# yanglei18/SGV3D

Hardware: AMD Instinct MI355X
Metric: camera frames/sec at 864x1536->BEV (higher is better)
Workload: dtype f32

## Files before the change

### include/sgv3d_hip.h

```cpp
#ifndef SGV3D_HIP_H
#define SGV3D_HIP_H

#include <stddef.h>
#include <stdint.h>

#ifdef __cplusplus
extern "C" {
#endif

#define SGV3D_OK 0
#define SGV3D_EINVAL (-1)
#define SGV3D_ELAUNCH (-2)
#define SGV3D_ENOSPACE (-3)

const char *sgv3d_last_error(void);
int sgv3d_abi_version(void);


int sgv3d_voxel_pooling_forward(int batch_size, int num_points, int num_channels,
                                int num_voxel_x, int num_voxel_y, int num_voxel_z,
                                const int32_t *geom_xyz, const float *input_features,
                                float *output_features, int32_t *pos_memo, void *stream);
int sgv3d_voxel_pooling_forward_fresh(int batch_size, int num_points, int num_channels,
                                      int num_voxel_x, int num_voxel_y, int num_voxel_z,
// ... 57 lines not shown
                              const float *prob,
                              const float *context,
                              const float *grad_output,
                              long long sb, long long sy, long long sx,
                              float *grad_prob,
                              float *grad_context,
                              void *workspace, size_t workspace_bytes, void *stream);


int sgv3d_calib_prep(int num_cams, const float *sensor2ego, const float *sensor2virtual,
                     const float *intrin, const float *ida, float *prep, void *stream);

int sgv3d_geometry_voxel_index(int num_cams, int cams_per_batch, int num_depth, int feat_h, int feat_w,
                               const float *frustum, const float *prep, const float *ref_h,
                               const float *bda, const float *voxel_coord ,
                               const float *voxel_size , int32_t *geom_xyz, float *geom_f,
                               void *stream);

int sgv3d_calib_changed(int n, const void *const *tensors , const int32_t *nbytes ,
                        void *copy, int force, int32_t *changed, void *stream);
int sgv3d_calib_prep_gated(int num_cams, const float *sensor2ego, const float *sensor2virtual, const float *intrin,
                           const float *ida, float *prep, const int32_t *run, void *stream);
int sgv3d_geometry_voxel_index_gated(int num_cams, int cams_per_batch, int num_depth, int feat_h, int feat_w,
                                     const float *frustum, const float *prep, const float *ref_h, const float *bda,
                                     const float *voxel_coord , const float *voxel_size , int32_t *geom_xyz,
                                     float *geom_f, const int32_t *run, void *stream);


int sgv3d_lift(int batch_size, int num_pixels, int num_depth, int num_channels,
               const float *height_context, float *prob, float *lifted, void *stream);
int sgv3d_lift_bf16(int batch_size, int num_pixels, int num_depth, int num_channels, const float *height_context,
                    float *prob, void *lifted_bf16, void *stream);


typedef struct sgv3d_conv_desc {
    int batch, in_h, in_w, cin;
    int out_h, out_w, cout;
    int kh, kw, stride, pad, dil;
    int x_ld, x_coff;
    int y_ld, y_coff;
    int res_ld;
    int relu;
    int mode;
    int deconv_ks;
    int k_pad, cout_pad;
    int tile;
    int x_nchw;
    int k_order;
    int split_k;
} sgv3d_conv_desc;

#define SGV3D_CONV_NORMAL 0
#define SGV3D_CONV_DECONV 1
#define SGV3D_CONV_NCHW_OUT 2
#define SGV3D_CONV_GROUP_PLANES 3

#define SGV3D_TILE_128x128 1
#define SGV3D_TILE_128x64 2
#define SGV3D_TILE_64x128 3
#define SGV3D_TILE_64x64 4
#define SGV3D_TILE_32x128 9
#define SGV3D_TILE_48x64 10
#define SGV3D_TILE_X3 64
#define SGV3D_TILE_MFIRST 16
#define SGV3D_TILE_OCC5 32
#define SGV3D_WINOGRAD_RESIDENT 6
#define SGV3D_WINOGRAD_HALF 8

int sgv3d_conv_winograd4_pack_weight(const float *w_src , int cout, int cin, int k_pad, int cout_pad,
                                     float *u_packed , void *stream);
int sgv3d_conv_winograd4_pack_weight_x3(const float *w_src, int cout, int cin, int cin_pad, int cout_pad, void *u3_packed,
                                        void *stream);

int sgv3d_conv_pack_weight_x3(const float *w_src, int cout, int cin, int kh, int kw, int cin_pad, int cout_pad, void *u3_packed,
                              void *stream);
int sgv3d_conv2d_x3_forward(const sgv3d_conv_desc *desc, const float *x, const void *u3_packed, const float *scale,
                            const float *bias, const float *residual, float *y, void *workspace, size_t workspace_bytes,
                            void *stream);
int sgv3d_conv2d_x3_shortcut_forward(const sgv3d_conv_desc *desc_a, const float *xa, const void *u3a, const float *scale_a,
                                     const float *bias_a, const sgv3d_conv_desc *desc_b, const float *xb, const void *u3b,
                                     const float *scale_b, const float *bias_b, float *y, void *stream);
int sgv3d_stem_pool_x3_forward(int batch, int h, int w, const float *x_nchw, const void *w_x3, size_t w_bytes, const float *scale,
                               const float *shift, float *y_nhwc, int y_ld, int variant, void *stream);
size_t sgv3d_conv2d_winograd4_workspace_bytes(const sgv3d_conv_desc *desc );
int sgv3d_conv2d_winograd4_forward(const sgv3d_conv_desc *desc , const float *x, const float *u_packed,
                                   const float *scale, const float *bias, const float *residual, float *y,
                                   void *workspace, size_t workspace_bytes, void *stream);

void sgv3d_conv_pack_geometry(int k, int n, int *k_pad, int *n_pad);

int sgv3d_conv_pack_weight(const float *w_src, int cout, int cin, int kh, int kw, int cin_pad,
                           int transposed, int k_order, float *w_packed, int k_pad, int cout_pad,
                           void *stream);

size_t sgv3d_conv2d_workspace_bytes(const sgv3d_conv_desc *desc );
int sgv3d_conv2d_forward(const sgv3d_conv_desc *desc , const float *x, const float *w_packed,
                         const float *scale, const float *bias, const float *residual,
                         const float *gate, float *y, void *workspace, size_t workspace_bytes,
                         void *stream);

int sgv3d_conv2d_forward_bf16(const sgv3d_conv_desc *desc , const float *x, const float *w_packed,
                              const float *scale, const float *bias, const float *residual,
                              const float *gate, float *y, void *workspace, size_t workspace_bytes,
                              void *stream);

int sgv3d_conv_weight_to_bf16(const float *w_packed, int k_pad, int cout_pad, void *w_packed_bf16, void *stream);
int sgv3d_conv2d_forward_bf16io(const sgv3d_conv_desc *desc , const void *x, const void *w_packed,
                                const float *scale, const float *bias, const void *residual, const float *gate,
                                void *y, void *workspace, size_t workspace_bytes, void *stream, int io_flags);

int sgv3d_conv2d_forward_f32x3(const sgv3d_conv_desc *desc , const float *x, const float *w_packed,
                               const float *scale, const float *bias, const float *residual,
                               const float *gate, float *y, void *workspace, size_t workspace_bytes,
                               void *stream);

size_t sgv3d_conv_winograd_weight_floats(int cout, int cin_pad);
int sgv3d_conv_winograd_pack_weight(const float *w_src, int cout, int cin, int cin_pad, float *w_packed,
                                    void *stream);
int sgv3d_conv2d_winograd_forward(const sgv3d_conv_desc *desc , const float *x, const float *w_wino,
                                  const float *scale, const float *bias, const float *residual,
                                  const float *gate, float *y, void *workspace, size_t workspace_bytes,
                                  void *stream);


int sgv3d_maxpool3x3s2(int batch, int in_h, int in_w, int channels, const float *x, float *y,
                       void *stream);

int sgv3d_maxpool3x3s2_bf16(int batch, int in_h, int in_w, int channels, const void *x, void *y, void *stream);
int sgv3d_nchw_to_nhwc(int batch, int channels, int h, int w, int c_pad, const float *x, float *y,
                       void *stream);
int sgv3d_nhwc_to_nchw(int batch, int channels, int h, int w, int ld, int coff, const float *x,
                       float *y, void *stream);

size_t sgv3d_global_avgpool_workspace_bytes(int batch, int channels);
int sgv3d_global_avgpool(int batch, int pixels, int channels, int x_ld, const float *x, float *y,
                         void *workspace, size_t workspace_bytes, void *stream);

int sgv3d_dense(int batch, int k, int n, const float *x, const float *w, const float *scale,
                const float *bias, int act, float *y, void *stream);
int sgv3d_dense_gated(int batch, int k, int n, const float *x, const float *w, const float *scale,
                      const float *bias, int act, float *y, const int32_t *run, void *stream);

int sgv3d_broadcast_channels(int batch, int pixels, int channels, int y_ld, int y_coff,
                             const float *v, float *y, void *stream);

int sgv3d_scale_channels(int batch, int pixels, int channels, const float *x, const float *gate,
                         float *y, void *stream);

int sgv3d_copy_channels(int batch, int pixels, int channels, int x_ld, int x_coff, const float *x,
                        float *y, void *stream);

int sgv3d_upsample_bilinear2x(int batch, int h, int w, int channels, const float *x, float *y, void *stream);

int sgv3d_add_mul_sigmoid(long long n, const float *a, const float *b, const float *c, float *y, void *stream);

int sgv3d_bsm_compose(int batch, int pixels, int num_depth, int context_channels, int semantic_channels,
                      int ld, const float *semantic_logits, int semantic_ld, float background_threshold,
                      float *height_context, void *stream);

int sgv3d_deform_conv3x3_forward(int batch, int h, int w, int channels, int groups, int out_per_group, const float *x,
                                 const float *offset, int off_ld, const float *const *w_packed, int k_pad, int cout_pad,
                                 float *y, int y_ld, int y_coff, void *stream);

size_t sgv3d_deform_conv3x3_bf16_weight_bytes(int channels, int groups, int out_per_group);
int sgv3d_deform_conv3x3_bf16_pack_weight(const float *weight, int channels, int groups, int out_per_group, void *w_packed,
                                          void *stream);
int sgv3d_deform_conv3x3_forward_bf16(int batch, int h, int w, int channels, int groups, int out_per_group, const void *x,
                                      int x_is_bf16, const float *offset, int off_ld, const void *w_packed, void *y,
                                      int y_is_bf16, int y_ld, int y_coff, void *stream);

// ... 555 lines not shown
```

### sgv3d_amd/_lib.py

```python
import ctypes
import os

_HERE = os.path.dirname(os.path.abspath(__file__))
LIB_PATH = os.path.join(_HERE, "csrc", "libsgv3d_hip.so")

c_int, c_void_p, c_size_t, c_ll = ctypes.c_int, ctypes.c_void_p, ctypes.c_size_t, ctypes.c_longlong


class ConvDesc(ctypes.Structure):
    _fields_ = [(n, c_int) for n in (
        "batch", "in_h", "in_w", "cin", "out_h", "out_w", "cout", "kh", "kw", "stride", "pad", "dil",
        "x_ld", "x_coff", "y_ld", "y_coff", "res_ld", "relu", "mode", "deconv_ks", "k_pad", "cout_pad",
        "tile", "x_nchw", "k_order", "split_k")]


class VitAttnDesc(ctypes.Structure):
    _fields_ = [(n, c_int) for n in ("batch", "height", "width", "heads", "head_dim", "win_h", "win_w")]


class SamAttnDesc(ctypes.Structure):
    _fields_ = [(n, c_int) for n in ("batch", "nq", "nk", "heads", "head_dim", "q_ld", "k_ld", "v_ld", "o_ld")] + [("scale", ctypes.c_float)]


CONV_NORMAL, CONV_DECONV, CONV_NCHW_OUT, CONV_GROUP_PLANES = 0, 1, 2, 3
# ... 1 lines not shown

_PROTOS = {
    "sgv3d_last_error": (ctypes.c_char_p, []),
    "sgv3d_abi_version": (c_int, []),
    "sgv3d_voxel_pooling_select_kernel": (c_int, [c_int]),
    "sgv3d_voxel_pooling_kernel_for": (c_int, [c_int] * 6),
    "sgv3d_voxel_pooling_forward": (c_int, [c_int] * 6 + [c_void_p] * 5),
    "sgv3d_voxel_pooling_forward_fresh": (c_int, [c_int] * 6 + [c_void_p] * 5),
    "sgv3d_voxel_pooling_forward_atomic": (c_int, [c_int] * 6 + [c_void_p] * 5),
    "sgv3d_voxel_pooling_cache_clear": (c_int, []),
    "sgv3d_voxel_pooling_cache_stats": (c_int, [ctypes.POINTER(ctypes.c_ulonglong)]),
    "sgv3d_voxel_plan_bytes": (c_size_t, [c_int] * 4),
    "sgv3d_voxel_plan_build": (c_int, [c_int] * 5 + [c_void_p, c_void_p, c_void_p, c_size_t, c_int, c_void_p]),
    "sgv3d_voxel_plan_init": (c_int, [c_int] * 4 + [c_void_p, c_size_t, c_void_p]),
    "sgv3d_voxel_plan_build_cached": (c_int, [c_int] * 5 + [c_void_p, c_void_p, c_size_t, c_int, c_void_p]),
    "sgv3d_voxel_plan_stats_offset": (c_size_t, [c_int] * 4),
    "sgv3d_voxel_pooling_workspace_bytes": (c_size_t, [c_int] * 3),
    "sgv3d_voxel_pooling_forward_planned": (c_int, [c_int] * 5 + [c_void_p] * 4 + [c_size_t, c_void_p]),
    "sgv3d_voxel_pooling_forward_planned_bf16": (c_int, [c_int] * 5 + [c_void_p] * 3 + [c_int, c_void_p, c_size_t, c_void_p]),
    "sgv3d_lift_splat_planned_bf16out": (c_int, [c_int] * 6 + [c_void_p] * 3 + [c_int, c_void_p, c_int, c_void_p, c_size_t, c_void_p]),
    "sgv3d_lift_splat_planned": (c_int, [c_int] * 6 + [c_void_p] * 5 + [c_size_t, c_void_p]),
    "sgv3d_voxel_pooling_backward": (c_int, [c_int] * 3 + [c_void_p, c_void_p, c_ll, c_ll, c_ll, c_ll, c_void_p, c_void_p]),
    "sgv3d_lift_splat_backward_workspace_bytes": (c_size_t, [c_int] * 4),
    "sgv3d_lift_splat_backward": (c_int, [c_int] * 7 + [c_void_p] * 4 + [c_ll] * 3 + [c_void_p] * 3 + [c_size_t, c_void_p]),
    "sgv3d_calib_prep": (c_int, [c_int] + [c_void_p] * 6),
    "sgv3d_calib_prep_gated": (c_int, [c_int] + [c_void_p] * 7),
    "sgv3d_calib_changed": (c_int, [c_int, ctypes.POINTER(c_void_p), ctypes.POINTER(c_int), c_void_p, c_int, c_void_p, c_void_p]),
    "sgv3d_geometry_voxel_index_gated": (c_int, [c_int] * 5 + [c_void_p] * 4 + [ctypes.POINTER(ctypes.c_float)] * 2 + [c_void_p] * 4),
    "sgv3d_dense_gated": (c_int, [c_int] * 3 + [c_void_p] * 4 + [c_int, c_void_p, c_void_p, c_void_p]),
    "sgv3d_geometry_voxel_index": (c_int, [c_int] * 5 + [c_void_p] * 4 + [ctypes.POINTER(ctypes.c_float)] * 2 + [c_void_p] * 3),
    "sgv3d_lift": (c_int, [c_int] * 4 + [c_void_p] * 4),
    "sgv3d_lift_bf16": (c_int, [c_int] * 4 + [c_void_p] * 4),
    "sgv3d_conv_pack_geometry": (None, [c_int, c_int, ctypes.POINTER(c_int), ctypes.POINTER(c_int)]),
    "sgv3d_conv_pack_weight": (c_int, [c_void_p] + [c_int] * 7 + [c_void_p, c_int, c_int, c_void_p]),
    "sgv3d_conv2d_workspace_bytes": (c_size_t, [ctypes.POINTER(ConvDesc)]),
    "sgv3d_conv2d_forward": (c_int, [ctypes.POINTER(ConvDesc)] + [c_void_p] * 8 + [c_size_t, c_void_p]),
    "sgv3d_conv2d_forward_bf16": (c_int, [ctypes.POINTER(ConvDesc)] + [c_void_p] * 8 + [c_size_t, c_void_p]),
    "sgv3d_conv2d_forward_bf16io": (c_int, [ctypes.POINTER(ConvDesc)] + [c_void_p] * 8 + [c_size_t, c_void_p, c_int]),
    "sgv3d_conv_weight_to_bf16": (c_int, [c_void_p, c_int, c_int, c_void_p, c_void_p]),
    "sgv3d_conv2d_forward_f32x3": (c_int, [ctypes.POINTER(ConvDesc)] + [c_void_p] * 8 + [c_size_t, c_void_p]),
    "sgv3d_centerhead_branches_workspace_bytes": (c_size_t, [c_int] * 4),
    "sgv3d_centerhead_branches_forward": (c_int, [c_int] * 6 + [c_void_p, c_int] + [c_void_p] * 3 + [c_int] + [c_void_p] * 5
                                          + [c_size_t, c_void_p]),
    "sgv3d_centerhead_bf16_weight_bytes": (c_size_t, [c_int]),
    "sgv3d_centerhead_bf16_pack_weight": (c_int, [c_void_p, c_int, c_int, c_void_p, c_void_p]),
    "sgv3d_centerhead_bf16_weight2_bytes": (c_size_t, [c_int]),
    "sgv3d_centerhead_bf16_pack_weight2": (c_int, [c_void_p, c_void_p, c_int, c_void_p, c_void_p]),
    "sgv3d_centerhead_f4_weight_floats": (c_size_t, [c_int]),
    "sgv3d_centerhead_f4_pack_weight": (c_int, [c_void_p, c_int, c_void_p, c_void_p]),
    "sgv3d_centerhead_branches_forward_f4": (c_int, [c_int] * 6 + [c_void_p, c_int] + [c_void_p] * 3 + [c_int] + [c_void_p] * 5
                                             + [c_size_t, c_void_p]),
    "sgv3d_conv3x3_f4res_weight_floats": (c_size_t, [c_int, c_int]),
    "sgv3d_conv3x3_f4res_pack_weight": (c_int, [c_void_p, c_int, c_int, c_int, c_void_p, c_void_p]),
    "sgv3d_conv3x3_f4res_forward": (c_int, [ctypes.POINTER(ConvDesc)] + [c_void_p] * 7),
    "sgv3d_centerhead_branches_forward_bf16": (c_int, [c_int] * 6 + [c_void_p, c_int] + [c_void_p] * 3 + [c_int] + [c_void_p] * 5),
    "sgv3d_centerhead_branches_forward_bf16x": (c_int, [c_int] * 6 + [c_void_p, c_int] + [c_void_p] * 3 + [c_int] + [c_void_p] * 5),
    "sgv3d_centerhead_bf16_select_plain": (None, [c_int]),
    "sgv3d_centerhead_bf16_debug_stamps": (None, [c_void_p]),
    "sgv3d_scale_channels_bf16": (c_int, [c_int] * 3 + [c_void_p] * 4),
    "sgv3d_global_avgpool_bf16": (c_int, [c_int] * 4 + [c_void_p] * 3 + [c_size_t, c_void_p]),
    "sgv3d_broadcast_channels_bf16": (c_int, [c_int] * 5 + [c_void_p] * 3),
    "sgv3d_upsample_bilinear2x_bf16": (c_int, [c_int] * 4 + [c_void_p] * 3),
    "sgv3d_add_mul_sigmoid_bf16": (c_int, [c_ll] + [c_void_p] * 5),
    "sgv3d_deform_im2col3x3_bf16": (c_int, [c_int] * 5 + [c_void_p] * 2 + [c_int, c_void_p, c_void_p]),
    "sgv3d_conv3x3_patch_bf16_weight_bytes": (c_size_t, [c_int, c_int]),
    "sgv3d_conv3x3_patch_bf16_debug_stamps": (None, [c_void_p]),
    "sgv3d_conv3x3_patch_bf16_pack_weight": (c_int, [c_void_p, c_int, c_int, c_void_p, c_void_p]),
    "sgv3d_conv3x3_patch_bf16_forward": (c_int, [c_int] * 11 + [c_void_p] * 6 + [c_int, c_int, c_void_p, c_size_t, c_void_p]),
    "sgv3d_conv_dw_bf16_weight_bytes": (c_size_t, [c_int] * 4),
    "sgv3d_conv_dw_bf16_pack_weight": (c_int, [c_void_p] + [c_int] * 5 + [c_void_p, c_void_p]),
    "sgv3d_conv_dw_bf16_forward": (c_int, [ctypes.POINTER(ConvDesc)] + [c_void_p] * 7),
    "sgv3d_conv_dw_bf16_workspace_bytes": (c_size_t, [ctypes.POINTER(ConvDesc)]),
    "sgv3d_conv_dw_bf16_forward_splitk": (c_int, [ctypes.POINTER(ConvDesc)] + [c_void_p] * 7 + [c_size_t, c_void_p]),
    "sgv3d_conv_dw_bf16_pair_forward": (c_int, [ctypes.POINTER(ConvDesc)] + [c_void_p] * 4 + [c_int] + [c_void_p] * 4 + [c_int, c_void_p, c_int, c_int, c_int, c_void_p]),
    "sgv3d_conv_winograd_weight_floats": (c_size_t, [c_int, c_int]),
    "sgv3d_conv_winograd_pack_weight": (c_int, [c_void_p, c_int, c_int, c_int, c_void_p, c_void_p]),
    "sgv3d_conv2d_winograd_forward": (c_int, [ctypes.POINTER(ConvDesc)] + [c_void_p] * 8 + [c_size_t, c_void_p]),
    "sgv3d_conv_winograd4_pack_weight": (c_int, [c_void_p, c_int, c_int, c_int, c_int, c_void_p, c_void_p]),
    "sgv3d_conv_winograd4_pack_weight_x3": (c_int, [c_void_p, c_int, c_int, c_int, c_int, c_void_p, c_void_p]),
    "sgv3d_conv_pack_weight_x3": (c_int, [c_void_p, c_int, c_int, c_int, c_int, c_int, c_int, c_void_p, c_void_p]),
    "sgv3d_conv2d_x3_forward": (c_int, [c_void_p] * 8 + [c_size_t, c_void_p]),
    "sgv3d_conv2d_x3_shortcut_forward": (c_int, [c_void_p] * 12),
    "sgv3d_stem_pool_x3_forward": (c_int, [c_int] * 3 + [c_void_p, c_void_p, c_size_t] + [c_void_p] * 3 + [c_int, c_int, c_void_p]),
    "sgv3d_conv2d_winograd4_workspace_bytes": (c_size_t, [ctypes.POINTER(ConvDesc)]),
    "sgv3d_conv2d_winograd4_forward": (c_int, [ctypes.POINTER(ConvDesc)] + [c_void_p] * 7 + [c_size_t, c_void_p]),
    "sgv3d_maxpool3x3s2": (c_int, [c_int] * 4 + [c_void_p] * 3),
    "sgv3d_maxpool3x3s2_bf16": (c_int, [c_int] * 4 + [c_void_p] * 3),
    "sgv3d_nchw_to_nhwc": (c_int, [c_int] * 5 + [c_void_p] * 3),
    "sgv3d_nhwc_to_nchw": (c_int, [c_int] * 6 + [c_void_p] * 3),
    "sgv3d_global_avgpool_workspace_bytes": (c_size_t, [c_int] * 2),
    "sgv3d_global_avgpool": (c_int, [c_int] * 4 + [c_void_p] * 3 + [c_size_t, c_void_p]),
    "sgv3d_dense": (c_int, [c_int] * 3 + [c_void_p] * 4 + [c_int, c_void_p, c_void_p]),
    "sgv3d_broadcast_channels": (c_int, [c_int] * 5 + [c_void_p] * 3),
    "sgv3d_scale_channels": (c_int, [c_int] * 3 + [c_void_p] * 4),
    "sgv3d_copy_channels": (c_int, [c_int] * 5 + [c_void_p] * 3),
    "sgv3d_upsample_bilinear2x": (c_int, [c_int] * 4 + [c_void_p] * 3),
    "sgv3d_add_mul_sigmoid": (c_int, [c_ll] + [c_void_p] * 5),
    "sgv3d_bsm_compose": (c_int, [c_int] * 6 + [c_void_p, c_int, ctypes.c_float, c_void_p, c_void_p]),
    "sgv3d_deform_im2col3x3": (c_int, [c_int] * 5 + [c_void_p, c_void_p, c_int, c_void_p, c_void_p]),
    "sgv3d_deform_conv3x3_forward": (c_int, [c_int] * 6 + [c_void_p, c_void_p, c_int, c_void_p, c_int, c_int, c_void_p, c_int, c_int,
                                                          c_void_p]),
    "sgv3d_deform_conv3x3_bf16_weight_bytes": (c_size_t, [c_int] * 3),
    "sgv3d_deform_conv3x3_bf16_pack_weight": (c_int, [c_void_p, c_int, c_int, c_int, c_void_p, c_void_p]),
    "sgv3d_deform_conv3x3_forward_bf16": (c_int, [c_int] * 6 + [c_void_p, c_int, c_void_p, c_int, c_void_p, c_void_p, c_int, c_int, c_int,
                                                               c_void_p]),
    "sgv3d_head_final_conv": (c_int, [c_int] * 6 + [c_void_p] * 6),
    "sgv3d_centerpoint_decode_workspace_bytes": (c_size_t, [c_int] * 3),
    "sgv3d_centerpoint_decode": (c_int, [c_int] * 5 + [c_void_p] * 6 + [c_ll] + [ctypes.c_float] * 6 +
                                 [ctypes.POINTER(ctypes.c_float), c_int, ctypes.c_float, c_int, c_void_p, c_size_t] +
                                 [c_void_p] * 6),
    "sgv3d_centerpoint_decode_tasks_workspace_bytes": (c_size_t, [c_int] * 4),
    "sgv3d_centerpoint_decode_tasks": (c_int, [c_int, c_int, ctypes.POINTER(ctypes.c_int32), c_int, c_int, c_int] +
                                       [ctypes.POINTER(c_void_p)] * 6 + [c_ll] + [ctypes.c_float] * 6 +
                                       [ctypes.POINTER(ctypes.c_float), c_int, ctypes.POINTER(ctypes.c_float), c_int, c_void_p,
                                        c_size_t] + [c_void_p] * 6),
    "sgv3d_centerpoint_merge_tasks": (c_int, [c_int] * 3 + [c_void_p] * 4 + [ctypes.POINTER(ctypes.c_int32)] + [c_void_p] * 5),
    "sgv3d_rotated_bev_iou_host": (c_int, [c_int] + [ctypes.POINTER(ctypes.c_float)] * 3),
    "sgv3d_rotate_nms_workspace_bytes": (c_size_t, [c_int] * 3),
    "sgv3d_rotate_nms": (c_int, [c_int] * 3 + [c_void_p] * 3 + [ctypes.c_float, ctypes.POINTER(ctypes.c_float), c_int, c_int,
                                                                ctypes.POINTER(ctypes.c_float), c_void_p, c_size_t, c_void_p, c_void_p]),
    "sgv3d_centerpoint_decode_tasks_rotate_workspace_bytes": (c_size_t, [c_int] * 4),
    "sgv3d_centerpoint_decode_tasks_rotate": (c_int, [c_int, c_int, ctypes.POINTER(ctypes.c_int32), c_int, c_int, c_int] +
                                              [ctypes.POINTER(c_void_p)] * 6 + [c_ll] + [ctypes.c_float] * 6 +
                                              [ctypes.POINTER(ctypes.c_float), c_int, ctypes.c_float, ctypes.POINTER(ctypes.c_float),
                                               c_int, c_int, ctypes.POINTER(ctypes.c_float), c_void_p, c_size_t] + [c_void_p] * 6),
    "sgv3d_centerhead_targets": (c_int, [c_int, c_int, c_void_p, c_void_p, c_int, ctypes.POINTER(ctypes.c_int32)] +
                                 [c_int] * 3 + [ctypes.c_float] * 5 + [ctypes.c_double, c_int, c_int] + [c_void_p] * 5),
    "sgv3d_conv2d_backward_weight_workspace_bytes": (c_size_t, [ctypes.POINTER(ConvDesc), c_int]),
    "sgv3d_conv2d_backward_weight": (c_int, [ctypes.POINTER(ConvDesc)] + [c_void_p] * 3 + [c_int, c_void_p, c_size_t, c_void_p]),
    "sgv3d_conv2d_backward_weight_bf16_workspace_bytes": (c_size_t, [ctypes.POINTER(ConvDesc), c_int]),
    "sgv3d_conv2d_backward_weight_bf16": (c_int, [ctypes.POINTER(ConvDesc)] + [c_void_p] * 3 + [c_int, c_void_p, c_size_t, c_void_p]),
    "sgv3d_conv2d_backward_weight_bf16_batched_workspace_bytes": (c_size_t, [ctypes.POINTER(ConvDesc), c_int, c_int]),
    "sgv3d_conv2d_backward_weight_bf16_batched": (c_int, [ctypes.POINTER(ConvDesc), c_void_p, ctypes.POINTER(c_void_p), ctypes.POINTER(c_void_p), c_int, c_int, c_void_p, c_size_t, c_void_p]),
    "sgv3d_conv2d_backward_weight_bf16_alltaps_workspace_bytes": (c_size_t, [ctypes.POINTER(ConvDesc), c_int, c_int]),
    "sgv3d_conv2d_backward_weight_bf16_alltaps": (c_int, [ctypes.POINTER(ConvDesc)] + [c_void_p] * 3 + [c_int, c_void_p, c_size_t, c_void_p]),
    "sgv3d_conv2d_backward_weight_bf16_tensors_workspace_bytes": (c_size_t, [ctypes.POINTER(ConvDesc), c_int]),
    "sgv3d_conv2d_backward_weight_bf16_tensors": (c_int, [ctypes.POINTER(ConvDesc)] + [c_void_p] * 3 + [c_int, c_void_p, c_size_t, c_void_p]),
    "sgv3d_conv2d_backward_weight_bf16_alltaps_tensors_workspace_bytes": (c_size_t, [ctypes.POINTER(ConvDesc), c_int]),
    "sgv3d_conv2d_backward_weight_bf16_alltaps_tensors": (c_int, [ctypes.POINTER(ConvDesc)] + [c_void_p] * 3 + [c_int, c_void_p, c_size_t, c_void_p]),
    "sgv3d_conv2d_backward_weight_bf16_alltaps_batched": (c_int, [ctypes.POINTER(ConvDesc), c_void_p, ctypes.POINTER(c_void_p), ctypes.POINTER(c_void_p), c_int, c_int, c_void_p, c_size_t, c_void_p]),
    "sgv3d_conv2d_backward_weight_thin_workspace_bytes": (c_size_t, [ctypes.POINTER(ConvDesc)]),
    "sgv3d_conv2d_backward_weight_batched_workspace_bytes": (c_size_t, [ctypes.POINTER(ConvDesc), c_int, c_int]),
    "sgv3d_conv2d_backward_weight_batched": (c_int, [ctypes.POINTER(ConvDesc), c_void_p, ctypes.POINTER(c_void_p), ctypes.POINTER(c_void_p), c_int, c_int, c_void_p, c_size_t, c_void_p]),
    "sgv3d_conv2d_backward_weight_thin": (c_int, [ctypes.POINTER(ConvDesc)] + [c_void_p] * 4 + [c_size_t, c_void_p]),
    "sgv3d_conv3x3_thin_forward_batched": (c_int, [ctypes.POINTER(ConvDesc), c_int, ctypes.POINTER(ctypes.c_int32)] + [ctypes.POINTER(c_void_p)] * 4 + [c_void_p]),
    "sgv3d_conv3x3_thin_backward_batched_workspace_bytes": (c_size_t, [ctypes.POINTER(ConvDesc), c_int, ctypes.POINTER(ctypes.c_int32)]),
    "sgv3d_conv3x3_thin_backward_batched": (c_int, [ctypes.POINTER(ConvDesc), c_int, ctypes.POINTER(ctypes.c_int32)] + [ctypes.POINTER(c_void_p)] * 6 + [c_void_p, c_size_t, c_void_p]),
    "sgv3d_weight_rot180_transpose": (c_int, [c_void_p] + [c_int] * 4 + [c_void_p, c_void_p]),
    "sgv3d_gather_pack_job_bytes": (c_int, []),
    "sgv3d_gather_pack_elements_per_block": (c_int, []),
    "sgv3d_gather_pack": (c_int, [c_void_p, c_int, c_int, c_void_p]),
    "sgv3d_zero_insert": (c_int, [c_int] * 7 + [c_void_p] * 3),
    "sgv3d_interleave_phases2": (c_int, [c_int] * 4 + [ctypes.POINTER(c_void_p)] + [ctypes.POINTER(ctypes.c_int32)] * 4 +
                                 [c_void_p, c_void_p]),
    "sgv3d_batchnorm_workspace_bytes": (c_size_t, [c_int]),
    "sgv3d_batchnorm_train_forward": (c_int, [c_ll, c_int] + [c_void_p] * 6 + [ctypes.c_float, ctypes.c_float, c_int] +
                                      [c_void_p] * 4 + [c_size_t, c_void_p]),
    "sgv3d_batchnorm_relu_train_backward_from_x": (c_int, [c_ll, c_int] + [c_void_p] * 9 + [c_void_p, c_size_t, c_void_p]),
    "sgv3d_batchnorm_train_backward": (c_int, [c_ll, c_int] + [c_void_p] * 6 + [c_int] + [c_void_p] * 5 + [c_size_t, c_void_p]),
    "sgv3d_batchnorm_train_forward_bf16": (c_int, [c_ll, c_int] + [c_void_p] * 6 + [ctypes.c_float, ctypes.c_float, c_int] +
                                           [c_void_p] * 4 + [c_size_t, c_void_p]),
    "sgv3d_batchnorm_relu_train_backward_from_x_bf16": (c_int, [c_ll, c_int] + [c_void_p] * 9 + [c_void_p, c_size_t, c_void_p]),
    "sgv3d_batchnorm_train_backward_bf16": (c_int, [c_ll, c_int] + [c_void_p] * 6 + [c_int] + [c_void_p] * 5 + [c_size_t, c_void_p]),
    "sgv3d_adamw_step": (c_int, [c_ll] + [c_void_p] * 4 + [c_int] + [ctypes.c_float] * 6 + [c_void_p] * 2),
    "sgv3d_adamw_step_dev": (c_int, [c_ll] + [c_void_p] * 5 + [ctypes.c_float] * 5 + [c_void_p] * 2),
    "sgv3d_adamw_set_hyper": (c_int, [c_void_p, c_int] + [ctypes.c_float] * 3 + [c_void_p]),
    "sgv3d_grad_sumsq_partials": (c_int, []),
    "sgv3d_grad_sumsq": (c_int, [c_ll, c_void_p, c_void_p, c_void_p]),
# ... 147 lines not shown
```

### sgv3d_amd/csrc/act_bf16.hip

```cpp
#include "common.hpp"

using namespace sgv3d;

namespace {

typedef __bf16 bf16x8 __attribute__((ext_vector_type(8)));
typedef __bf16 bf16x4 __attribute__((ext_vector_type(4)));
typedef float f32x4 __attribute__((ext_vector_type(4)));

constexpr int kBlock = 256;
constexpr int kAvgChunks = 32;

struct F8 {
    float v[8];
};

__device__ __forceinline__ F8 ld8(const __bf16 *p) {
    const bf16x8 q = *reinterpret_cast<const bf16x8 *>(p);
    F8 r;
#pragma unroll
    for (int i = 0; i < 8; ++i) r.v[i] = (float)q[i];
    return r;
}

__device__ __forceinline__ void st8(__bf16 *p, const F8 &r) {
    const f32x4 lo = {r.v[0], r.v[1], r.v[2], r.v[3]}, hi = {r.v[4], r.v[5], r.v[6], r.v[7]};
    const bf16x4 l4 = __builtin_convertvector(lo, bf16x4), h4 = __builtin_convertvector(hi, bf16x4);
    *reinterpret_cast<bf16x8 *>(p) = __builtin_shufflevector(l4, h4, 0, 1, 2, 3, 4, 5, 6, 7);
}

__global__ __launch_bounds__(kBlock) void scale_channels_bf16_kernel(long long total8, int P, int C8, const __bf16 *__restrict__ x,
                                                                     const float *__restrict__ gate, __bf16 *__restrict__ y) {
    const long long i = (long long)blockIdx.x * kBlock + threadIdx.x;
    if (i >= total8) return;
    const int c = (int)(i % C8);
    const long long b = i / ((long long)P * C8);
    F8 v = ld8(x + i * 8);
    const float *g = gate + (b * C8 + c) * 8;
#pragma unroll
    for (int k = 0; k < 8; ++k) v.v[k] *= g[k];
    st8(y + i * 8, v);
}

__global__ __launch_bounds__(kBlock) void global_avgpool_bf16_partial_kernel(int P, int C, int ld, const __bf16 *__restrict__ x,
                                                                             float *__restrict__ part) {
    __shared__ float red[4][64];
    const int b = blockIdx.z, chunk = blockIdx.y;
    const int c = blockIdx.x * 64 + (threadIdx.x & 63);
    const int g = threadIdx.x >> 6;
    const int per = (P + kAvgChunks - 1) / kAvgChunks;
    const int p0 = chunk * per, p1 = min(P, p0 + per);
    float s = 0.f;
    if (c < C)
        for (int p = p0 + g; p < p1; p += 4) s += (float)x[((long long)b * P + p) * ld + c];
    red[g][threadIdx.x & 63] = s;
    __syncthreads();
    if (g == 0 && c < C)
        part[((long long)b * kAvgChunks + chunk) * C + c] =
            (red[0][threadIdx.x] + red[1][threadIdx.x]) + (red[2][threadIdx.x] + red[3][threadIdx.x]);
}

__global__ __launch_bounds__(kBlock) void global_avgpool_bf16_final_kernel(int B, int P, int C, const float *__restrict__ part,
                                                                           float *__restrict__ y) {
    const long long i = (long long)blockIdx.x * kBlock + threadIdx.x;
    if (i >= (long long)B * C) return;
    const int b = (int)(i / C), c = (int)(i - (long long)b * C);
    float s = 0.f;
    for (int k = 0; k < kAvgChunks; ++k) s += part[((long long)b * kAvgChunks + k) * C + c];
    y[i] = s / (float)P;
}

__global__ __launch_bounds__(kBlock) void broadcast_channels_bf16_kernel(long long total8, int P, int C8, int ld, int coff,
                                                                         const float *__restrict__ v, __bf16 *__restrict__ y) {
    const long long i = (long long)blockIdx.x * kBlock + threadIdx.x;
    if (i >= total8) return;
    const int c = (int)(i % C8);
    const long long bp = i / C8;
    const long long b = bp / P;
    F8 r;
#pragma unroll
    for (int k = 0; k < 8; ++k) r.v[k] = v[(b * C8 + c) * 8 + k];
    st8(y + bp * ld + coff + c * 8, r);
}

__global__ __launch_bounds__(kBlock) void upsample_bilinear2x_bf16_kernel(int B, int H, int W, int C8, const __bf16 *__restrict__ x,
                                                                          __bf16 *__restrict__ y) {
    const long long total = (long long)B * 2 * H * 2 * W * C8;
    const long long i = (long long)blockIdx.x * kBlock + threadIdx.x;
    if (i >= total) return;
    const int c = (int)(i % C8);
    long long t = i / C8;
    const int ow = (int)(t % (2 * W));
    t /= (2 * W);
    const int oh = (int)(t % (2 * H));
    const int b = (int)(t / (2 * H));
    const float sh = fmaxf(0.5f * ((float)oh + 0.5f) - 0.5f, 0.f), sw = fmaxf(0.5f * ((float)ow + 0.5f) - 0.5f, 0.f);
    const int h1 = (int)sh, w1 = (int)sw;
    const int h1p = h1 < H - 1 ? 1 : 0, w1p = w1 < W - 1 ? 1 : 0;
    const float lh1 = sh - (float)h1, lw1 = sw - (float)w1;
    const float lh0 = 1.f - lh1, lw0 = 1.f - lw1;
    const __bf16 *p = x + (((long long)b * H * W) * C8 + c) * 8;
    const long long ps = (long long)C8 * 8;
    const F8 a = ld8(p + ((long long)h1 * W + w1) * ps), bq = ld8(p + ((long long)h1 * W + w1 + w1p) * ps);
    const F8 cq = ld8(p + ((long long)(h1 + h1p) * W + w1) * ps), d = ld8(p + ((long long)(h1 + h1p) * W + w1 + w1p) * ps);
    F8 o;
#pragma unroll
    for (int k = 0; k < 8; ++k) o.v[k] = lh0 * (lw0 * a.v[k] + lw1 * bq.v[k]) + lh1 * (lw0 * cq.v[k] + lw1 * d.v[k]);
    st8(y + i * 8, o);
}

__global__ __launch_bounds__(kBlock) void add_mul_sigmoid_bf16_kernel(long long n8, const __bf16 *__restrict__ a,
                                                                      const __bf16 *__restrict__ b, const __bf16 *__restrict__ c,
                                                                      __bf16 *__restrict__ y) {
    const long long i = (long long)blockIdx.x * kBlock + threadIdx.x;
    if (i >= n8) return;
    const F8 av = ld8(a + i * 8), bv = ld8(b + i * 8), cv = ld8(c + i * 8);
    F8 o;
#pragma unroll
    for (int k = 0; k < 8; ++k) o.v[k] = av.v[k] + bv.v[k] * (1.f / (1.f + expf(-cv.v[k])));
    st8(y + i * 8, o);
}

__global__ __launch_bounds__(kBlock) void deform_im2col3x3_bf16_kernel(int B, int H, int W, int C, int groups,
                                                                       const __bf16 *__restrict__ x, const float *__restrict__ off,
                                                                       int off_ld, __bf16 *__restrict__ col) {
    const int C8 = C >> 3;
    const long long total = (long long)B * H * W * 9 * C8;
    const long long i = (long long)blockIdx.x * kBlock + threadIdx.x;
    if (i >= total) return;
    const int c8 = (int)(i % C8);
    long long t = i / C8;
    const int tap = (int)(t % 9);
    t /= 9;
    const int w_ = (int)(t % W);
    const long long t2 = t / W;
    const int h_ = (int)(t2 % H);
    const int b = (int)(t2 / H);
    const int ky = tap / 3, kx = tap - ky * 3;
    const float oy = off[t * off_ld + 2 * tap], ox = off[t * off_ld + 2 * tap + 1];
    const float hf = (float)(h_ - 1 + ky) + oy;
    const float wf = (float)(w_ - 1 + kx) + ox;
    F8 val;
#pragma unroll
    for (int k = 0; k < 8; ++k) val.v[k] = 0.f;
    if (hf > -1.f && wf > -1.f && hf < (float)H && wf < (float)W) {
        const int h_low = (int)floorf(hf), w_low = (int)floorf(wf);
        const int h_high = h_low + 1, w_high = w_low + 1;
        const float lh = hf - (float)h_low, lw = wf - (float)w_low;
        const float hh = 1.f - lh, hw = 1.f - lw;
        const __bf16 *base = x + (long long)b * H * W * C + c8 * 8;
        const float w1 = hh * hw, w2 = hh * lw, w3 = lh * hw, w4 = lh * lw;
        F8 v1, v2, v3, v4;
#pragma unroll
        for (int k = 0; k < 8; ++k) v1.v[k] = v2.v[k] = v3.v[k] = v4.v[k] = 0.f;
        if (h_low >= 0 && w_low >= 0) v1 = ld8(base + ((long long)h_low * W + w_low) * C);
        if (h_low >= 0 && w_high <= W - 1) v2 = ld8(base + ((long long)h_low * W + w_high) * C);
        if (h_high <= H - 1 && w_low >= 0) v3 = ld8(base + ((long long)h_high * W + w_low) * C);
        if (h_high <= H - 1 && w_high <= W - 1) v4 = ld8(base + ((long long)h_high * W + w_high) * C);
#pragma unroll
        for (int k = 0; k < 8; ++k) val.v[k] = w1 * v1.v[k] + w2 * v2.v[k] + w3 * v3.v[k] + w4 * v4.v[k];
    }
    const int cpg = C / groups;
    const int c = c8 * 8;
    const int g = c / cpg, cg = c - g * cpg;
    st8(col + ((t * groups + g) * 9 + tap) * cpg + cg, val);
}

}

extern "C" int sgv3d_scale_channels_bf16(int batch, int pixels, int channels, const void *x, const float *gate, void *y, void *stream) {
    SGV3D_REQUIRE(batch > 0 && pixels > 0 && channels > 0 && (channels & 7) == 0, "scale_channels_bf16: channels must be a multiple of 8");
    SGV3D_REQUIRE(x && gate && y, "scale_channels_bf16: null pointer");
    const long long total8 = (long long)batch * pixels * (channels / 8);
    hipLaunchKernelGGL(scale_channels_bf16_kernel, dim3(cdiv(total8, kBlock)), dim3(kBlock), 0, as_stream(stream), total8, pixels,
                       channels / 8, static_cast<const __bf16 *>(x), gate, static_cast<__bf16 *>(y));
    return check_launch("scale_channels_bf16_kernel");
}

extern "C" int sgv3d_global_avgpool_bf16(int batch, int pixels, int channels, int x_ld, const void *x, float *y, void *workspace,
                                         size_t workspace_bytes, void *stream) {
    SGV3D_REQUIRE(batch > 0 && pixels > 0 && channels > 0 && x_ld >= channels, "global_avgpool_bf16: bad shape");
    SGV3D_REQUIRE(x && y && workspace, "global_avgpool_bf16: null pointer");
    if (workspace_bytes < sizeof(float) * (size_t)batch * kAvgChunks * channels)
        return fail(SGV3D_ENOSPACE, "global_avgpool_bf16: workspace too small (sgv3d_global_avgpool_workspace_bytes)");
    float *part = static_cast<float *>(workspace);
    hipLaunchKernelGGL(global_avgpool_bf16_partial_kernel, dim3(cdiv(channels, 64), kAvgChunks, batch), dim3(kBlock), 0,
                       as_stream(stream), pixels, channels, x_ld, static_cast<const __bf16 *>(x), part);
    hipLaunchKernelGGL(global_avgpool_bf16_final_kernel, dim3(cdiv((long long)batch * channels, kBlock)), dim3(kBlock), 0,
                       as_stream(stream), batch, pixels, channels, part, y);
    return check_launch("global_avgpool_bf16_kernel");
}

extern "C" int sgv3d_broadcast_channels_bf16(int batch, int pixels, int channels, int y_ld, int y_coff, const float *v, void *y,
                                             void *stream) {
    SGV3D_REQUIRE(batch > 0 && pixels > 0 && channels > 0 && y_ld >= y_coff + channels && y_coff >= 0, "broadcast_channels_bf16: bad shape");
    SGV3D_REQUIRE(((channels | y_ld | y_coff) & 7) == 0, "broadcast_channels_bf16: channels / y_ld / y_coff must be multiples of 8");
    SGV3D_REQUIRE(v && y, "broadcast_channels_bf16: null pointer");
    const long long total8 = (long long)batch * pixels * (channels / 8);
    hipLaunchKernelGGL(broadcast_channels_bf16_kernel, dim3(cdiv(total8, kBlock)), dim3(kBlock), 0, as_stream(stream), total8, pixels,
                       channels / 8, y_ld, y_coff, v, static_cast<__bf16 *>(y));
    return check_launch("broadcast_channels_bf16_kernel");
}

extern "C" int sgv3d_upsample_bilinear2x_bf16(int batch, int h, int w, int channels, const void *x, void *y, void *stream) {
    SGV3D_REQUIRE(batch > 0 && h > 0 && w > 0 && channels > 0 && (channels & 7) == 0, "upsample_bilinear2x_bf16: channels must be a multiple of 8");
    SGV3D_REQUIRE(x && y, "upsample_bilinear2x_bf16: null pointer");
    const long long total = (long long)batch * 4 * h * w * (channels / 8);
    hipLaunchKernelGGL(upsample_bilinear2x_bf16_kernel, dim3(cdiv(total, kBlock)), dim3(kBlock), 0, as_stream(stream), batch, h, w,
                       channels / 8, static_cast<const __bf16 *>(x), static_cast<__bf16 *>(y));
    return check_launch("upsample_bilinear2x_bf16_kernel");
}

extern "C" int sgv3d_add_mul_sigmoid_bf16(long long n, const void *a, const void *b, const void *c, void *y, void *stream) {
    SGV3D_REQUIRE(n > 0 && (n & 7) == 0, "add_mul_sigmoid_bf16: n must be a positive multiple of 8");
    SGV3D_REQUIRE(a && b && c && y, "add_mul_sigmoid_bf16: null pointer");
    hipLaunchKernelGGL(add_mul_sigmoid_bf16_kernel, dim3(cdiv(n / 8, kBlock)), dim3(kBlock), 0, as_stream(stream), n / 8,
                       static_cast<const __bf16 *>(a), static_cast<const __bf16 *>(b), static_cast<const __bf16 *>(c),
                       static_cast<__bf16 *>(y));
    return check_launch("add_mul_sigmoid_bf16_kernel");
}

extern "C" int sgv3d_deform_im2col3x3_bf16(int batch, int h, int w, int channels, int groups, const void *x, const float *offset,
                                           int off_ld, void *col, void *stream) {
    SGV3D_REQUIRE(batch > 0 && h > 0 && w > 0 && channels > 0 && groups > 0 && channels % groups == 0 &&
                      ((channels / groups) & 7) == 0 && off_ld >= 18,
                  "deform_im2col3x3_bf16: bad shape (channels per group must be a multiple of 8)");
    SGV3D_REQUIRE(x && offset && col, "deform_im2col3x3_bf16: null pointer");
    const long long total = (long long)batch * h * w * 9 * (channels / 8);
    hipLaunchKernelGGL(deform_im2col3x3_bf16_kernel, dim3(cdiv(total, kBlock)), dim3(kBlock), 0, as_stream(stream), batch, h, w,
                       channels, groups, static_cast<const __bf16 *>(x), offset, off_ld, static_cast<__bf16 *>(col));
    return check_launch("deform_im2col3x3_bf16_kernel");
}
```

### sgv3d_amd/csrc/conv_wino4.hip

```cpp
#include "conv_common.hpp"

using namespace sgv3d;

namespace {

struct f4 {
    float x, y, z, w;
};
__device__ __forceinline__ f4 ld4(const float *p) {
    const float4 v = *reinterpret_cast<const float4 *>(p);
    return {v.x, v.y, v.z, v.w};
}
__device__ __forceinline__ void st4(float *p, const f4 &v) { *reinterpret_cast<float4 *>(p) = make_float4(v.x, v.y, v.z, v.w); }
__device__ __forceinline__ f4 fma4(float s, const f4 &a, const f4 &b) {
    return {fmaf(s, a.x, b.x), fmaf(s, a.y, b.y), fmaf(s, a.z, b.z), fmaf(s, a.w, b.w)};
}
__device__ __forceinline__ f4 add4(const f4 &a, const f4 &b) { return {a.x + b.x, a.y + b.y, a.z + b.z, a.w + b.w}; }
__device__ __forceinline__ f4 sub4(const f4 &a, const f4 &b) { return {a.x - b.x, a.y - b.y, a.z - b.z, a.w - b.w}; }

__device__ __forceinline__ void wino4_bt(f4 &d0, f4 &d1, f4 &d2, f4 &d3, f4 &d4, f4 &d5) {
    const f4 a = fma4(-4.f, d2, d4), b = fma4(-4.f, d1, d3);
    const f4 c = sub4(d4, d2), e = sub4(d3, d1);
    const f4 t0 = fma4(4.f, d0, fma4(-5.f, d2, d4));
    const f4 t5 = fma4(4.f, d1, fma4(-5.f, d3, d5));
    d0 = t0;
    d1 = add4(a, b);
    d2 = sub4(a, b);
    d3 = fma4(2.f, e, c);
    d4 = fma4(-2.f, e, c);
    d5 = t5;
}

__device__ __forceinline__ void wino4_at(const f4 &m0, const f4 &m1, const f4 &m2, const f4 &m3, const f4 &m4, const f4 &m5,
                                         f4 &y0, f4 &y1, f4 &y2, f4 &y3) {
    const f4 p = add4(m1, m2), q = sub4(m1, m2), r = add4(m3, m4), s = sub4(m3, m4);
    y0 = add4(add4(m0, p), r);
    y1 = fma4(2.f, s, q);
    y2 = fma4(4.f, r, p);
    y3 = add4(fma4(8.f, s, q), m5);
}

constexpr int kTB = 256;

struct Wino4Args {
    const float *x, *scale, *bias, *res;
    float *v, *m, *y;
    int batch, h, w, cin, cout, x_ld, x_coff, y_ld, y_coff, res_ld, relu;
    int ty, tx;
    int dil;
    int rows;
    int c0, cn;
    int gw;
};

__device__ __forceinline__ void wino4_tile(const Wino4Args &a, int t, int &b, int &py, int &px, int &iy, int &ix) {
    const int per_phase = a.ty * a.tx, per_img = per_phase * a.dil * a.dil;
    b = t / per_img;
    int r = t - b * per_img;
    const int ph = r / per_phase;
    r -= ph * per_phase;
    py = ph / a.dil;
    px = ph - py * a.dil;
    iy = r / a.tx;
    ix = r - iy * a.tx;
}

__global__ __launch_bounds__(kTB) void wino4_input_kernel(const Wino4Args a) {
    const int cq = a.cin >> 2;
    const long long i = (long long)blockIdx.x * kTB + threadIdx.x;
    const long long ntile = (long long)a.batch * a.ty * a.tx * a.dil * a.dil;
    if (i >= ntile * cq) return;
    const int t = (int)(i / cq), c = (int)(i - (long long)t * cq) * 4;
    int b, py, px, iy, ix;
    wino4_tile(a, t, b, py, px, iy, ix);
    const int y0 = py + (4 * iy - 1) * a.dil, x0 = px + (4 * ix - 1) * a.dil;
    const float *xb = a.x + (size_t)b * a.h * a.w * a.x_ld + a.x_coff + c;
    f4 d[6][6];
#pragma unroll
    for (int rr = 0; rr < 6; ++rr) {
        const int yy = y0 + rr * a.dil;
        const bool rok = (unsigned)yy < (unsigned)a.h;
#pragma unroll
        for (int cc = 0; cc < 6; ++cc) {
            const int xx = x0 + cc * a.dil;
            d[rr][cc] = (rok && (unsigned)xx < (unsigned)a.w) ? ld4(xb + ((size_t)yy * a.w + xx) * a.x_ld) : f4{0.f, 0.f, 0.f, 0.f};
        }
    }
#pragma unroll
    for (int cc = 0; cc < 6; ++cc) wino4_bt(d[0][cc], d[1][cc], d[2][cc], d[3][cc], d[4][cc], d[5][cc]);
    float *vb = a.v + (size_t)t * a.cin + c;
    const size_t plane = (size_t)a.rows * a.cin;
#pragma unroll
    for (int rr = 0; rr < 6; ++rr) {
        wino4_bt(d[rr][0], d[rr][1], d[rr][2], d[rr][3], d[rr][4], d[rr][5]);
#pragma unroll
        for (int cc = 0; cc < 6; ++cc) st4(vb + (size_t)(rr * 6 + cc) * plane, d[rr][cc]);
    }
}

__global__ __launch_bounds__(kTB) void wino4_output_kernel(const Wino4Args a) {
    const int cq = a.cn >> 2;
    const long long i = (long long)blockIdx.x * kTB + threadIdx.x;
    const long long ntile = (long long)a.batch * a.ty * a.tx * a.dil * a.dil;
    if (i >= ntile * cq) return;
    const int t = (int)(i / cq), cl = (int)(i - (long long)t * cq) * 4;
    const int c = a.c0 + cl;
    int b, py, px, iy, ix;
    wino4_tile(a, t, b, py, px, iy, ix);
    const float *mb = a.m + (size_t)t * a.cn + cl;
    const size_t plane = (size_t)a.rows * a.cn;
    f4 rr_[4][6];
#pragma unroll
    for (int cc = 0; cc < 6; ++cc) {
        const f4 m0 = ld4(mb + (size_t)(0 * 6 + cc) * plane), m1 = ld4(mb + (size_t)(1 * 6 + cc) * plane),
                 m2 = ld4(mb + (size_t)(2 * 6 + cc) * plane), m3 = ld4(mb + (size_t)(3 * 6 + cc) * plane),
                 m4 = ld4(mb + (size_t)(4 * 6 + cc) * plane), m5 = ld4(mb + (size_t)(5 * 6 + cc) * plane);
        wino4_at(m0, m1, m2, m3, m4, m5, rr_[0][cc], rr_[1][cc], rr_[2][cc], rr_[3][cc]);
    }
    const f4 sc = a.scale ? ld4(a.scale + c) : f4{1.f, 1.f, 1.f, 1.f};
    const f4 sh = a.bias ? ld4(a.bias + c) : f4{0.f, 0.f, 0.f, 0.f};
    const float floor_ = a.relu ? 0.f : -__builtin_inff();
#pragma unroll
    for (int u = 0; u < 4; ++u) {
        f4 o[4];
        wino4_at(rr_[u][0], rr_[u][1], rr_[u][2], rr_[u][3], rr_[u][4], rr_[u][5], o[0], o[1], o[2], o[3]);
        const int yy = py + (4 * iy + u) * a.dil;
        if (yy >= a.h) continue;
#pragma unroll
        for (int v = 0; v < 4; ++v) {
            const int xx = px + (4 * ix + v) * a.dil;
            if (xx >= a.w) continue;
            const size_t pix = ((size_t)b * a.h + yy) * a.w + xx;
            f4 q = {fmaf(o[v].x, sc.x, sh.x), fmaf(o[v].y, sc.y, sh.y), fmaf(o[v].z, sc.z, sh.z), fmaf(o[v].w, sc.w, sh.w)};
            if (a.res) q = add4(q, ld4(a.res + pix * a.res_ld + c));
            q = {fmaxf(q.x, floor_), fmaxf(q.y, floor_), fmaxf(q.z, floor_), fmaxf(q.w, floor_)};
            if (a.gw > 0) {
                const int grp = c / a.gw;
                st4(a.y + ((size_t)grp * a.batch * a.h * a.w + pix) * a.gw + (c - grp * a.gw), q);
            } else {
                st4(a.y + pix * a.y_ld + a.y_coff + c, q);
            }
        }
    }
}

__global__ __launch_bounds__(256) void wino4_pack_weight_kernel(const float *__restrict__ w, int cout, int cin, int k_pad,
                                                                int cout_pad, float *__restrict__ u) {
    const long long i = (long long)blockIdx.x * 256 + threadIdx.x;
    if (i >= (long long)cout_pad * k_pad) return;
    const int co = (int)(i / k_pad), ci = (int)(i - (long long)co * k_pad);
    float g[3][3] = {{0.f, 0.f, 0.f}, {0.f, 0.f, 0.f}, {0.f, 0.f, 0.f}};
    if (co < cout && ci < cin) {
        const float *p = w + ((size_t)co * cin + ci) * 9;
#pragma unroll
        for (int a = 0; a < 3; ++a)
#pragma unroll
            for (int b = 0; b < 3; ++b) g[a][b] = p[a * 3 + b];
    }
    float t[6][3];
#pragma unroll
    for (int b = 0; b < 3; ++b) {
        const float s02 = g[0][b] + g[2][b];
        t[0][b] = 0.25f * g[0][b];
        t[1][b] = (-1.f / 6.f) * (s02 + g[1][b]);
        t[2][b] = (-1.f / 6.f) * (s02 - g[1][b]);
        t[3][b] = (1.f / 24.f) * g[0][b] + (1.f / 12.f) * g[1][b] + (1.f / 6.f) * g[2][b];
        t[4][b] = (1.f / 24.f) * g[0][b] - (1.f / 12.f) * g[1][b] + (1.f / 6.f) * g[2][b];
        t[5][b] = g[2][b];
    }
    const size_t block = (size_t)cout_pad * k_pad;
#pragma unroll
    for (int r = 0; r < 6; ++r) {
        const float s02 = t[r][0] + t[r][2];
        const float o[6] = {0.25f * t[r][0], (-1.f / 6.f) * (s02 + t[r][1]), (-1.f / 6.f) * (s02 - t[r][1]),
                            (1.f / 24.f) * t[r][0] + (1.f / 12.f) * t[r][1] + (1.f / 6.f) * t[r][2],
                            (1.f / 24.f) * t[r][0] - (1.f / 12.f) * t[r][1] + (1.f / 6.f) * t[r][2], t[r][2]};
#pragma unroll
        for (int c = 0; c < 6; ++c) u[(size_t)(r * 6 + c) * block + i] = o[c];
    }
}

typedef __bf16 bf16x4 __attribute__((ext_vector_type(4)));
typedef float f32x4v __attribute__((ext_vector_type(4)));

__device__ __forceinline__ void split3(const f4 &x, bf16x4 &hi, bf16x4 &mid, bf16x4 &lo) {
    const f32x4v v = {x.x, x.y, x.z, x.w};
    hi = __builtin_convertvector(v, bf16x4);
    const f32x4v r1 = v - __builtin_convertvector(hi, f32x4v);
    mid = __builtin_convertvector(r1, bf16x4);
    const f32x4v r2 = r1 - __builtin_convertvector(mid, f32x4v);
    lo = __builtin_convertvector(r2, bf16x4);
}

__global__ __launch_bounds__(kTB) void wino4_input_x3_kernel(const Wino4Args a) {
    const int cq = a.cin >> 2;
    const long long i = (long long)blockIdx.x * kTB + threadIdx.x;
    const long long ntile = (long long)a.batch * a.ty * a.tx * a.dil * a.dil;
    if (i >= ntile * cq) return;
    const int t = (int)(i / cq), c = (int)(i - (long long)t * cq) * 4;
    int b, py, px, iy, ix;
    wino4_tile(a, t, b, py, px, iy, ix);
    const int y0 = py + (4 * iy - 1) * a.dil, x0 = px + (4 * ix - 1) * a.dil;
    const float *xb = a.x + (size_t)b * a.h * a.w * a.x_ld + a.x_coff + c;
    f4 d[6][6];
#pragma unroll
    for (int rr = 0; rr < 6; ++rr) {
        const int yy = y0 + rr * a.dil;
        const bool rok = (unsigned)yy < (unsigned)a.h;
#pragma unroll
        for (int cc = 0; cc < 6; ++cc) {
            const int xx = x0 + cc * a.dil;
            d[rr][cc] = (rok && (unsigned)xx < (unsigned)a.w) ? ld4(xb + ((size_t)yy * a.w + xx) * a.x_ld) : f4{0.f, 0.f, 0.f, 0.f};
        }
    }
#pragma unroll
    for (int cc = 0; cc < 6; ++cc) wino4_bt(d[0][cc], d[1][cc], d[2][cc], d[3][cc], d[4][cc], d[5][cc]);
    __bf16 *vb = reinterpret_cast<__bf16 *>(a.v) + ((size_t)t * (a.cin >> 5) + (c >> 5)) * 96 + (c & 31);
    const size_t plane = (size_t)a.rows * (a.cin >> 5) * 96;
#pragma unroll
    for (int rr = 0; rr < 6; ++rr) {
        wino4_bt(d[rr][0], d[rr][1], d[rr][2], d[rr][3], d[rr][4], d[rr][5]);
#pragma unroll
        for (int cc = 0; cc < 6; ++cc) {
            bf16x4 hi, mid, lo;
            split3(d[rr][cc], hi, mid, lo);
            __bf16 *o = vb + (size_t)(rr * 6 + cc) * plane;
            *reinterpret_cast<bf16x4 *>(o) = hi;
            *reinterpret_cast<bf16x4 *>(o + 32) = mid;
            *reinterpret_cast<bf16x4 *>(o + 64) = lo;
        }
    }
}

__global__ __launch_bounds__(256) void wino4_pack_weight_x3_kernel(const float *__restrict__ w, int cout, int cin, int k_pad,
                                                                   int cout_pad, __bf16 *__restrict__ u) {
    const long long i = (long long)blockIdx.x * 256 + threadIdx.x;
    if (i >= (long long)cout_pad * k_pad) return;
    const int co = (int)(i / k_pad), ci = (int)(i - (long long)co * k_pad);
    float g[3][3] = {{0.f, 0.f, 0.f}, {0.f, 0.f, 0.f}, {0.f, 0.f, 0.f}};
    if (co < cout && ci < cin) {
        const float *p = w + ((size_t)co * cin + ci) * 9;
#pragma unroll
        for (int a = 0; a < 3; ++a)
#pragma unroll
            for (int b = 0; b < 3; ++b) g[a][b] = p[a * 3 + b];
    }
    float t[6][3];
#pragma unroll
    for (int b = 0; b < 3; ++b) {
        const float s02 = g[0][b] + g[2][b];
        t[0][b] = 0.25f * g[0][b];
        t[1][b] = (-1.f / 6.f) * (s02 + g[1][b]);
        t[2][b] = (-1.f / 6.f) * (s02 - g[1][b]);
        t[3][b] = (1.f / 24.f) * g[0][b] + (1.f / 12.f) * g[1][b] + (1.f / 6.f) * g[2][b];
        t[4][b] = (1.f / 24.f) * g[0][b] - (1.f / 12.f) * g[1][b] + (1.f / 6.f) * g[2][b];
        t[5][b] = g[2][b];
    }
    const size_t block = (size_t)cout_pad * k_pad * 3;
    __bf16 *ub = u + (((size_t)(co >> 4) * (k_pad >> 5) + (ci >> 5)) * 3) * 512 + ((((ci & 31) >> 3) * 16 + (co & 15)) * 8 + (ci & 7));
#pragma unroll
    for (int r = 0; r < 6; ++r) {
        const float s02 = t[r][0] + t[r][2];
        const float o[6] = {0.25f * t[r][0], (-1.f / 6.f) * (s02 + t[r][1]), (-1.f / 6.f) * (s02 - t[r][1]),
                            (1.f / 24.f) * t[r][0] + (1.f / 12.f) * t[r][1] + (1.f / 6.f) * t[r][2],
                            (1.f / 24.f) * t[r][0] - (1.f / 12.f) * t[r][1] + (1.f / 6.f) * t[r][2], t[r][2]};
#pragma unroll
        for (int c = 0; c < 6; ++c) {
            const float v = o[c];
            const __bf16 hi = (__bf16)v;
            const float r1 = v - (float)hi;
            const __bf16 mid = (__bf16)r1;
            const __bf16 lo = (__bf16)(r1 - (float)mid);
            __bf16 *q = ub + (size_t)(r * 6 + c) * block;
            q[0] = hi;
            q[512] = mid;
            q[1024] = lo;
        }
    }
}

void wino4_geom(const sgv3d_conv_desc *d, int &ty, int &tx, long long &tiles, int &rows) {
    const int dil = d->dil;
    ty = cdiv(cdiv(d->out_h, dil), 4);
    tx = cdiv(cdiv(d->out_w, dil), 4);
    tiles = (long long)d->batch * dil * dil * ty * tx;
    const int g = (d->tile & SGV3D_TILE_X3) ? gemm_x3_tile_rows(d->tile & 15)
                  : (d->tile & ~SGV3D_TILE_OCC5) == SGV3D_TILE_32x128 ? 32 : d->tile == SGV3D_TILE_48x64 ? 48 : 64;
    rows = (int)((tiles + g - 1) / g * g);
}

int wino4_chunk(const sgv3d_conv_desc *d, int rows) {
    const long long per_channel = 36LL * rows * 4;
    long long cn = (160LL << 20) / per_channel / 128 * 128;
    if (cn < 128) cn = 128;
    return cn >= d->cout ? d->cout : (int)cn;
}

}

extern "C" int sgv3d_conv_winograd4_pack_weight(const float *w_src, int cout, int cin, int k_pad, int cout_pad, float *u_packed,
                                                void *stream) {
    SGV3D_REQUIRE(w_src && u_packed && cout > 0 && cin > 0 && k_pad >= cin && k_pad % 32 == 0 && cout_pad >= cout,
                  "conv_winograd4_pack_weight: bad arguments (cout=%d cin=%d k_pad=%d cout_pad=%d)", cout, cin, k_pad, cout_pad);
    const long long total = (long long)cout_pad * k_pad;
    hipLaunchKernelGGL(wino4_pack_weight_kernel, dim3(cdiv(total, 256)), dim3(256), 0, as_stream(stream), w_src, cout, cin, k_pad,
                       cout_pad, u_packed);
    return check_launch("wino4_pack_weight_kernel");
}

extern "C" int sgv3d_conv_winograd4_pack_weight_x3(const float *w_src, int cout, int cin, int cin_pad, int cout_pad, void *u3_packed,
                                                   void *stream) {
    SGV3D_REQUIRE(w_src && u3_packed && cout > 0 && cin > 0 && cin_pad >= cin && cin_pad % 32 == 0 && cout_pad >= cout && cout_pad % 32 == 0,
                  "conv_winograd4_pack_weight_x3: bad arguments (cout=%d cin=%d cin_pad=%d cout_pad=%d)", cout, cin, cin_pad, cout_pad);
    const long long total = (long long)cout_pad * cin_pad;
    hipLaunchKernelGGL(wino4_pack_weight_x3_kernel, dim3(cdiv(total, 256)), dim3(256), 0, as_stream(stream), w_src, cout, cin, cin_pad,
                       cout_pad, static_cast<__bf16 *>(u3_packed));
    return check_launch("wino4_pack_weight_x3_kernel");
}

extern "C" size_t sgv3d_conv2d_winograd4_workspace_bytes(const sgv3d_conv_desc *d) {
    if (!d || d->batch <= 0 || d->out_h <= 0 || d->out_w <= 0 || d->cin <= 0 || d->cout <= 0 || d->dil <= 0) return 0;
    int ty, tx, rows;
    long long tiles;
    wino4_geom(d, ty, tx, tiles, rows);
    if (d->tile & SGV3D_TILE_X3)
        return 36 * (size_t)rows * (6 * (size_t)d->cin + sizeof(float) * (size_t)wino4_chunk(d, rows));
    return sizeof(float) * 36 * (size_t)rows * ((size_t)d->cin + (size_t)wino4_chunk(d, rows));
}

extern "C" int sgv3d_conv2d_winograd4_forward(const sgv3d_conv_desc *d, const float *x, const float *u_packed,
                                              const float *scale, const float *bias, const float *residual, float *y,
                                              void *workspace, size_t workspace_bytes, void *stream) {
    SGV3D_REQUIRE(d && x && u_packed && y && workspace, "conv2d_winograd4_forward: null pointer");
    SGV3D_REQUIRE(d->kh == 3 && d->kw == 3 && d->stride == 1 && d->dil >= 1 && d->pad == d->dil,
                  "conv2d_winograd4_forward: only 3x3 / stride 1 / pad == dilation");
    SGV3D_REQUIRE(d->batch > 0 && d->in_h > 0 && d->in_w > 0 && d->cin > 0 && d->cout > 0 && d->out_h == d->in_h && d->out_w == d->in_w,
                  "conv2d_winograd4_forward: bad sizes");
    const bool planes = d->mode == SGV3D_CONV_GROUP_PLANES;
    SGV3D_REQUIRE(d->mode == SGV3D_CONV_NORMAL || planes, "conv2d_winograd4_forward: NHWC or GROUP_PLANES output only");
    SGV3D_REQUIRE(!planes || (d->deconv_ks > 0 && d->deconv_ks % 4 == 0 && d->cout % d->deconv_ks == 0 && residual == nullptr),
                  "conv2d_winograd4_forward: GROUP_PLANES needs deconv_ks = group width (a multiple of 4) dividing cout, no residual");
    SGV3D_REQUIRE(d->cin % 4 == 0 && d->cout % 4 == 0 && (d->x_ld & 3) == 0 && (d->x_coff & 3) == 0 &&
                      (planes || ((d->y_ld & 3) == 0 && (d->y_coff & 3) == 0)) && (residual == nullptr || (d->res_ld & 3) == 0),
                  "conv2d_winograd4_forward: channel counts, leading dimensions and offsets must be multiples of 4");
    SGV3D_REQUIRE(((reinterpret_cast<uintptr_t>(x) | reinterpret_cast<uintptr_t>(y) | reinterpret_cast<uintptr_t>(residual) |
                    reinterpret_cast<uintptr_t>(scale) | reinterpret_cast<uintptr_t>(bias) | reinterpret_cast<uintptr_t>(u_packed) |
                    reinterpret_cast<uintptr_t>(workspace)) & 15) == 0,
                  "conv2d_winograd4_forward: pointers must be 16-B aligned");
    SGV3D_REQUIRE(d->x_ld >= d->x_coff + d->cin && (planes || d->y_ld >= d->y_coff + d->cout) && (residual == nullptr || d->res_ld >= d->cout),
                  "conv2d_winograd4_forward: leading dimension too small");
    const size_t need = sgv3d_conv2d_winograd4_workspace_bytes(d);
    if (workspace_bytes < need) return fail(SGV3D_ENOSPACE, "conv2d_winograd4_forward: workspace has %zu bytes, needs %zu", workspace_bytes, need);
    Wino4Args a;
    a.x = x; a.scale = scale; a.bias = bias; a.res = residual; a.y = y;
    a.batch = d->batch; a.h = d->in_h; a.w = d->in_w; a.cin = d->cin; a.cout = d->cout;
    a.x_ld = d->x_ld; a.x_coff = d->x_coff; a.y_ld = d->y_ld; a.y_coff = d->y_coff; a.res_ld = d->res_ld; a.relu = d->relu;
    long long tiles;
    wino4_geom(d, a.ty, a.tx, tiles, a.rows);
    a.dil = d->dil;
    SGV3D_REQUIRE(tiles < 0x7fffffffLL / 64, "conv2d_winograd4_forward: too many tiles");
    const bool x3 = (d->tile & SGV3D_TILE_X3) != 0;
    a.v = static_cast<float *>(workspace);
    a.m = x3 ? reinterpret_cast<float *>(static_cast<unsigned char *>(workspace) + (size_t)36 * a.rows * d->cin * 6)
             : a.v + (size_t)36 * a.rows * d->cin;
    hipStream_t st = as_stream(stream);
    a.gw = planes ? d->deconv_ks : 0;
    a.c0 = 0; a.cn = d->cout;
    if (x3) {
        SGV3D_REQUIRE(d->cin % 32 == 0 && d->cout_pad % 32 == 0 && d->cout_pad >= d->cout,
                      "conv2d_winograd4_forward: SGV3D_TILE_X3 needs cin %% 32 == 0 and cout_pad (a multiple of 32) of the x3 weights");
        SGV3D_REQUIRE((d->tile & 15) < 10, "conv2d_winograd4_forward: unknown SGV3D_TILE_X3 variant %d", d->tile & 15);
        hipLaunchKernelGGL(wino4_input_x3_kernel, dim3(cdiv(tiles * (d->cin / 4), kTB)), dim3(kTB), 0, st, a);
        const int chunk3 = wino4_chunk(d, a.rows);
        for (int c0 = 0; c0 < d->cout; c0 += chunk3) {
            a.c0 = c0;
            a.cn = d->cout - c0 < chunk3 ? d->cout - c0 : chunk3;
            if (int rc = conv_gemm_grouped_x3(a.v, static_cast<const unsigned char *>(static_cast<const void *>(u_packed)) + (size_t)c0 * d->cin * 6,
                                              a.m, a.rows, d->cin, a.cn, d->cout_pad - c0, d->tile & 15, st, (size_t)d->cout_pad * d->cin * 6)) return rc;
            hipLaunchKernelGGL(wino4_output_kernel, dim3(cdiv(tiles * (a.cn / 4), kTB)), dim3(kTB), 0, st, a);
        }
        return check_launch("conv2d_winograd4_forward(x3)");
    }
    hipLaunchKernelGGL(wino4_input_kernel, dim3(cdiv(tiles * (d->cin / 4), kTB)), dim3(kTB), 0, st, a);
    int tile = (d->tile == SGV3D_TILE_64x128 || d->tile == SGV3D_TILE_32x128 || d->tile == SGV3D_TILE_48x64) ? d->tile
               : (d->tile & SGV3D_TILE_OCC5) ? (SGV3D_TILE_64x64 | SGV3D_TILE_OCC5) : SGV3D_TILE_64x64;
    if (tile == SGV3D_TILE_32x128 && (d->k_order != 1 || d->cin < 128)) tile = SGV3D_TILE_64x64;
    SGV3D_REQUIRE(tile != SGV3D_TILE_48x64 || (d->k_order == 1 && d->cin % 32 == 0),
                  "conv2d_winograd4_forward: SGV3D_TILE_48x64 needs channel-chunk-major weights (cin %% 32 == 0)");
    const int chunk = wino4_chunk(d, a.rows);
    for (int c0 = 0; c0 < d->cout; c0 += chunk) {
        a.c0 = c0;
        a.cn = d->cout - c0 < chunk ? d->cout - c0 : chunk;
        if (tile == SGV3D_TILE_48x64) {
            if (int rc = conv_gemm_grouped16(a.v, u_packed + (size_t)c0 * d->k_pad, a.m, a.rows, 36, d->cin, a.cn, d->k_pad,
                                             d->cout_pad, st)) return rc;
        } else if (int rc = conv_gemm_grouped(a.v, u_packed + (size_t)c0 * d->k_pad, a.m, a.rows, 36, d->cin, a.cn, d->k_pad,
                                              d->cout_pad, d->k_order, tile, st)) return rc;
        hipLaunchKernelGGL(wino4_output_kernel, dim3(cdiv(tiles * (a.cn / 4), kTB)), dim3(kTB), 0, st, a);
    }
    return check_launch("conv2d_winograd4_forward");
}
```

### sgv3d_amd/csrc/misc_layers.hip

```cpp
#include "common.hpp"

using namespace sgv3d;

namespace {

constexpr int kBlock = 256;

__device__ __forceinline__ float max_nan(float m, float v) { return (v > m || v != v) ? v : m; }

__global__ __launch_bounds__(kBlock) void maxpool3x3s2_kernel(int B, int H, int W, int C4, int OH, int OW,
                                                              const float4 *__restrict__ x, float4 *__restrict__ y) {
    const long long i = (long long)blockIdx.x * kBlock + threadIdx.x;
    const long long total = (long long)B * OH * OW * C4;
    if (i >= total) return;
    const int c = (int)(i % C4);
    long long t = i / C4;
    const int ow = (int)(t % OW);
    t /= OW;
    const int oh = (int)(t % OH);
    const int b = (int)(t / OH);
    float4 m = make_float4(-INFINITY, -INFINITY, -INFINITY, -INFINITY);
#pragma unroll
    for (int dy = 0; dy < 3; ++dy) {
        const int ih = oh * 2 - 1 + dy;
        if ((unsigned)ih >= (unsigned)H) continue;
#pragma unroll
        for (int dx = 0; dx < 3; ++dx) {
            const int iw = ow * 2 - 1 + dx;
            if ((unsigned)iw >= (unsigned)W) continue;
            const float4 v = x[((long long)(b * H + ih) * W + iw) * C4 + c];
            m.x = max_nan(m.x, v.x); m.y = max_nan(m.y, v.y); m.z = max_nan(m.z, v.z); m.w = max_nan(m.w, v.w);
        }
    }
    y[i] = m;
}

typedef __bf16 mp_bf16x8 __attribute__((ext_vector_type(8)));
__global__ __launch_bounds__(kBlock) void maxpool3x3s2_bf16_kernel(int B, int H, int W, int C8, int OH, int OW,
                                                                   const mp_bf16x8 *__restrict__ x, mp_bf16x8 *__restrict__ y) {
    const long long i = (long long)blockIdx.x * kBlock + threadIdx.x;
    const long long total = (long long)B * OH * OW * C8;
    if (i >= total) return;
    const int c = (int)(i % C8);
    long long t = i / C8;
    const int ow = (int)(t % OW);
    t /= OW;
    const int oh = (int)(t % OH);
    const int b = (int)(t / OH);
    float m[8];
#pragma unroll
    for (int j = 0; j < 8; ++j) m[j] = -INFINITY;
#pragma unroll
    for (int dy = 0; dy < 3; ++dy) {
        const int ih = oh * 2 - 1 + dy;
        if ((unsigned)ih >= (unsigned)H) continue;
#pragma unroll
        for (int dx = 0; dx < 3; ++dx) {
            const int iw = ow * 2 - 1 + dx;
            if ((unsigned)iw >= (unsigned)W) continue;
            const mp_bf16x8 v = x[((long long)(b * H + ih) * W + iw) * C8 + c];
#pragma unroll
            for (int j = 0; j < 8; ++j) m[j] = max_nan(m[j], (float)v[j]);
        }
    }
    mp_bf16x8 o;
#pragma unroll
    for (int j = 0; j < 8; ++j) o[j] = (__bf16)m[j];
    y[i] = o;
}

__global__ __launch_bounds__(kBlock) void nchw_to_nhwc_kernel(int B, int C, long long HW, int Cp,
                                                              const float *__restrict__ x, float *__restrict__ y) {
    const long long i = (long long)blockIdx.x * kBlock + threadIdx.x;
    if (i >= (long long)B * HW) return;
    const long long b = i / HW, p = i - b * HW;
    const float *src = x + b * C * HW + p;
    float *dst = y + i * Cp;
    for (int c = 0; c < Cp; ++c) dst[c] = c < C ? src[(long long)c * HW] : 0.f;
}

__global__ __launch_bounds__(kBlock) void nhwc_to_nchw_kernel(int C, long long HW, int ld, int coff,
                                                              const float *__restrict__ x, float *__restrict__ y) {
    __shared__ float tile[32][33];
    const int b = blockIdx.z;
    const long long p0 = (long long)blockIdx.x * 32;
    const int c0 = blockIdx.y * 32;
    const int tx = threadIdx.x & 31, ty = threadIdx.x >> 5;
    for (int r = ty; r < 32; r += 8) {
        const long long p = p0 + r;
        const int c = c0 + tx;
        tile[r][tx] = (p < HW && c < C) ? x[((long long)b * HW + p) * ld + coff + c] : 0.f;
    }
    __syncthreads();
    for (int r = ty; r < 32; r += 8) {
        const int c = c0 + r;
        const long long p = p0 + tx;
        if (c < C && p < HW) y[((long long)b * C + c) * HW + p] = tile[tx][r];
    }
}

constexpr int kAvgChunks = 32;

__global__ __launch_bounds__(kBlock) void global_avgpool_partial_kernel(int P, int C, int ld,
                                                                        const float *__restrict__ x,
                                                                        float *__restrict__ part) {
    __shared__ float red[4][64];
    const int b = blockIdx.z, chunk = blockIdx.y;
    const int c = blockIdx.x * 64 + (threadIdx.x & 63);
    const int g = threadIdx.x >> 6;
    const int per = (P + kAvgChunks - 1) / kAvgChunks;
    const int p0 = chunk * per, p1 = min(P, p0 + per);
    float s = 0.f;
    if (c < C)
        for (int p = p0 + g; p < p1; p += 4) s += x[((long long)b * P + p) * ld + c];
    red[g][threadIdx.x & 63] = s;
    __syncthreads();
    if (g == 0 && c < C)
        part[((long long)b * kAvgChunks + chunk) * C + c] =
            (red[0][threadIdx.x] + red[1][threadIdx.x]) + (red[2][threadIdx.x] + red[3][threadIdx.x]);
}

__global__ __launch_bounds__(kBlock) void global_avgpool_final_kernel(int B, int P, int C,
                                                                      const float *__restrict__ part,
                                                                      float *__restrict__ y) {
    const long long i = (long long)blockIdx.x * kBlock + threadIdx.x;
    if (i >= (long long)B * C) return;
    const int b = (int)(i / C), c = (int)(i - (long long)b * C);
    float s = 0.f;
    for (int k = 0; k < kAvgChunks; ++k) s += part[((long long)b * kAvgChunks + k) * C + c];
    y[i] = s / (float)P;
}

__global__ __launch_bounds__(kBlock) void dense_kernel(int B, int K, int N, const float *__restrict__ x,
                                                       const float *__restrict__ w, const float *__restrict__ scale,
                                                       const float *__restrict__ bias, int act, float *__restrict__ y,
                                                       const int *__restrict__ run) {
    if (run && *run == 0) return;
    const int wave = blockIdx.x * (kBlock / 64) + (threadIdx.x >> 6);
    const int lane = threadIdx.x & 63;
    if (wave >= B * N) return;
    const int b = wave / N, n = wave - b * N;
    const float *xr = x + (long long)b * K;
    const float *wr = w + (long long)n * K;
    float s = 0.f;
    for (int k = lane; k < K; k += 64) s += wr[k] * xr[k];
#pragma unroll
    for (int o = 32; o > 0; o >>= 1) s += __shfl_xor(s, o, 64);
    if (lane == 0) {
        float v = s * (scale ? scale[n] : 1.f) + (bias ? bias[n] : 0.f);
        if (act == 1) v = fmaxf(v, 0.f);
        else if (act == 2) v = 1.f / (1.f + expf(-v));
        y[(long long)b * N + n] = v;
    }
}

__global__ __launch_bounds__(kBlock) void broadcast_channels_kernel(long long total, int P, int C, int ld, int coff,
                                                                    const float *__restrict__ v, float *__restrict__ y) {
    const long long i = (long long)blockIdx.x * kBlock + threadIdx.x;
    if (i >= total) return;
    const int c = (int)(i % C);
    const long long bp = i / C;
    const long long b = bp / P;
    y[bp * ld + coff + c] = v[b * C + c];
}

__global__ __launch_bounds__(kBlock) void scale_channels_kernel(long long total4, int P, int C4,
                                                                const float4 *__restrict__ x,
                                                                const float4 *__restrict__ gate,
                                                                float4 *__restrict__ y) {
    const long long i = (long long)blockIdx.x * kBlock + threadIdx.x;
    if (i >= total4) return;
    const int c = (int)(i % C4);
    const long long b = i / ((long long)P * C4);
    const float4 v = x[i], g = gate[b * C4 + c];
    y[i] = make_float4(v.x * g.x, v.y * g.y, v.z * g.z, v.w * g.w);
}

__global__ __launch_bounds__(kBlock) void copy_channels_kernel(long long total, int C, int ld, int coff,
                                                               const float *__restrict__ x, float *__restrict__ y) {
    const long long i = (long long)blockIdx.x * kBlock + threadIdx.x;
    if (i >= total) return;
    const long long bp = i / C;
    const int c = (int)(i - bp * C);
    y[i] = x[bp * ld + coff + c];
}

__global__ __launch_bounds__(kBlock) void upsample_bilinear2x_kernel(int B, int H, int W, int C4,
                                                                     const float4 *__restrict__ x, float4 *__restrict__ y) {
    const long long total = (long long)B * 2 * H * 2 * W * C4;
    const long long i = (long long)blockIdx.x * kBlock + threadIdx.x;
    if (i >= total) return;
    const int c = (int)(i % C4);
    long long t = i / C4;
    const int ow = (int)(t % (2 * W));
    t /= (2 * W);
    const int oh = (int)(t % (2 * H));
    const int b = (int)(t / (2 * H));
    const float sh = fmaxf(0.5f * ((float)oh + 0.5f) - 0.5f, 0.f), sw = fmaxf(0.5f * ((float)ow + 0.5f) - 0.5f, 0.f);
    const int h1 = (int)sh, w1 = (int)sw;
    const int h1p = h1 < H - 1 ? 1 : 0, w1p = w1 < W - 1 ? 1 : 0;
    const float lh1 = sh - (float)h1, lw1 = sw - (float)w1;
    const float lh0 = 1.f - lh1, lw0 = 1.f - lw1;
    const float4 *p = x + ((long long)b * H * W) * C4 + c;
    const float4 a = p[((long long)h1 * W + w1) * C4], bq = p[((long long)h1 * W + w1 + w1p) * C4];
    const float4 cq = p[((long long)(h1 + h1p) * W + w1) * C4], d = p[((long long)(h1 + h1p) * W + w1 + w1p) * C4];
    float4 o;
    o.x = lh0 * (lw0 * a.x + lw1 * bq.x) + lh1 * (lw0 * cq.x + lw1 * d.x);
    o.y = lh0 * (lw0 * a.y + lw1 * bq.y) + lh1 * (lw0 * cq.y + lw1 * d.y);
    o.z = lh0 * (lw0 * a.z + lw1 * bq.z) + lh1 * (lw0 * cq.z + lw1 * d.z);
    o.w = lh0 * (lw0 * a.w + lw1 * bq.w) + lh1 * (lw0 * cq.w + lw1 * d.w);
    y[i] = o;
}

// ... 177 lines not shown
#pragma unroll
                        for (int ky = 0; ky < 3; ++ky) {
                            const float4 wv = *reinterpret_cast<const float4 *>(wts + (o * 9 + ky * 3 + kx) * hc + c0 + q * 4);
#pragma unroll
                            for (int r = 0; r < kHfRpt; ++r)
                                acc[o][r] += p[r + ky].x * wv.x + p[r + ky].y * wv.y + p[r + ky].z * wv.z + p[r + ky].w * wv.w;
                        }
                    }
                }
            }
        }
    }
#undef SGV3D_HF_LOAD
    const int x = tx0 + tx;
    if (x < W) {
#pragma unroll
        for (int o = 0; o < kHfMaxOut; ++o) {
            if (o < ck) {
                const float bv = bias[first + o];
#pragma unroll
                for (int r = 0; r < kHfRpt; ++r) {
                    const int y = ty0 + tq * kHfRpt + r;
                    if (y < H) out[((long long)(b * total_out + first + o) * H + y) * W + x] = acc[o][r] + bv;
                }
            }
        }
    }
}

}

extern "C" int sgv3d_maxpool3x3s2(int batch, int in_h, int in_w, int channels, const float *x, float *y, void *stream) {
    SGV3D_REQUIRE(batch > 0 && in_h > 0 && in_w > 0 && channels > 0 && (channels & 3) == 0, "maxpool3x3s2: bad shape");
    SGV3D_REQUIRE(x && y, "maxpool3x3s2: null pointer");
    const int oh = (in_h - 1) / 2 + 1, ow = (in_w - 1) / 2 + 1;
    const long long total = (long long)batch * oh * ow * (channels / 4);
    hipLaunchKernelGGL(maxpool3x3s2_kernel, dim3(cdiv(total, kBlock)), dim3(kBlock), 0, as_stream(stream), batch, in_h,
                       in_w, channels / 4, oh, ow, reinterpret_cast<const float4 *>(x), reinterpret_cast<float4 *>(y));
    return check_launch("maxpool3x3s2_kernel");
}

extern "C" int sgv3d_maxpool3x3s2_bf16(int batch, int in_h, int in_w, int channels, const void *x, void *y, void *stream) {
    SGV3D_REQUIRE(batch > 0 && in_h > 0 && in_w > 0 && channels > 0 && channels % 8 == 0, "maxpool3x3s2_bf16: channels must be a multiple of 8");
    SGV3D_REQUIRE(x && y && (reinterpret_cast<uintptr_t>(x) & 15) == 0 && (reinterpret_cast<uintptr_t>(y) & 15) == 0,
                  "maxpool3x3s2_bf16: null or unaligned pointer");
    const int oh = (in_h - 1) / 2 + 1, ow = (in_w - 1) / 2 + 1;
    const long long total = (long long)batch * oh * ow * (channels / 8);
    hipLaunchKernelGGL(maxpool3x3s2_bf16_kernel, dim3(cdiv(total, kBlock)), dim3(kBlock), 0, as_stream(stream), batch, in_h,
                       in_w, channels / 8, oh, ow, static_cast<const mp_bf16x8 *>(x), static_cast<mp_bf16x8 *>(y));
    return check_launch("maxpool3x3s2_bf16_kernel");
}

extern "C" int sgv3d_nchw_to_nhwc(int batch, int channels, int h, int w, int c_pad, const float *x, float *y, void *stream) {
    SGV3D_REQUIRE(batch > 0 && channels > 0 && h > 0 && w > 0 && c_pad >= channels, "nchw_to_nhwc: bad shape");
    SGV3D_REQUIRE(x && y, "nchw_to_nhwc: null pointer");
    const long long hw = (long long)h * w;
    hipLaunchKernelGGL(nchw_to_nhwc_kernel, dim3(cdiv(batch * hw, kBlock)), dim3(kBlock), 0, as_stream(stream), batch,
                       channels, hw, c_pad, x, y);
    return check_launch("nchw_to_nhwc_kernel");
}

extern "C" int sgv3d_nhwc_to_nchw(int batch, int channels, int h, int w, int ld, int coff, const float *x, float *y,
                                  void *stream) {
    SGV3D_REQUIRE(batch > 0 && channels > 0 && h > 0 && w > 0 && ld >= coff + channels && coff >= 0, "nhwc_to_nchw: bad shape");
    SGV3D_REQUIRE(x && y, "nhwc_to_nchw: null pointer");
    const long long hw = (long long)h * w;
    dim3 grid(cdiv(hw, 32), cdiv(channels, 32), batch);
    hipLaunchKernelGGL(nhwc_to_nchw_kernel, grid, dim3(kBlock), 0, as_stream(stream), channels, hw, ld, coff, x, y);
    return check_launch("nhwc_to_nchw_kernel");
}

extern "C" size_t sgv3d_global_avgpool_workspace_bytes(int batch, int channels) {
    if (batch <= 0 || channels <= 0) return 0;
    return sizeof(float) * (size_t)batch * kAvgChunks * channels;
}

extern "C" int sgv3d_global_avgpool(int batch, int pixels, int channels, int x_ld, const float *x, float *y,
                                    void *workspace, size_t workspace_bytes, void *stream) {
    SGV3D_REQUIRE(batch > 0 && pixels > 0 && channels > 0 && x_ld >= channels, "global_avgpool: bad shape");
    SGV3D_REQUIRE(x && y && workspace, "global_avgpool: null pointer");
    if (workspace_bytes < sgv3d_global_avgpool_workspace_bytes(batch, channels))
        return fail(SGV3D_ENOSPACE, "global_avgpool: workspace too small");
    float *part = static_cast<float *>(workspace);
    hipLaunchKernelGGL(global_avgpool_partial_kernel, dim3(cdiv(channels, 64), kAvgChunks, batch), dim3(kBlock), 0,
                       as_stream(stream), pixels, channels, x_ld, x, part);
    hipLaunchKernelGGL(global_avgpool_final_kernel, dim3(cdiv((long long)batch * channels, kBlock)), dim3(kBlock), 0,
                       as_stream(stream), batch, pixels, channels, part, y);
    return check_launch("global_avgpool_kernel");
}

extern "C" int sgv3d_dense_gated(int batch, int k, int n, const float *x, const float *w, const float *scale,
                                 const float *bias, int act, float *y, const int32_t *run, void *stream) {
    SGV3D_REQUIRE(batch > 0 && k > 0 && n > 0 && act >= 0 && act <= 2, "dense: bad shape/act");
    SGV3D_REQUIRE(x && w && y, "dense: null pointer");
    hipLaunchKernelGGL(dense_kernel, dim3(cdiv((long long)batch * n, kBlock / 64)), dim3(kBlock), 0, as_stream(stream),
                       batch, k, n, x, w, scale, bias, act, y, run);
    return check_launch("dense_kernel");
}

extern "C" int sgv3d_dense(int batch, int k, int n, const float *x, const float *w, const float *scale,
                           const float *bias, int act, float *y, void *stream) {
    return sgv3d_dense_gated(batch, k, n, x, w, scale, bias, act, y, nullptr, stream);
}

extern "C" int sgv3d_broadcast_channels(int batch, int pixels, int channels, int y_ld, int y_coff, const float *v,
                                        float *y, void *stream) {
    SGV3D_REQUIRE(batch > 0 && pixels > 0 && channels > 0 && y_ld >= y_coff + channels && y_coff >= 0, "broadcast_channels: bad shape");
    SGV3D_REQUIRE(v && y, "broadcast_channels: null pointer");
    const long long total = (long long)batch * pixels * channels;
    hipLaunchKernelGGL(broadcast_channels_kernel, dim3(cdiv(total, kBlock)), dim3(kBlock), 0, as_stream(stream), total,
                       pixels, channels, y_ld, y_coff, v, y);
    return check_launch("broadcast_channels_kernel");
}

extern "C" int sgv3d_scale_channels(int batch, int pixels, int channels, const float *x, const float *gate, float *y,
                                    void *stream) {
    SGV3D_REQUIRE(batch > 0 && pixels > 0 && channels > 0 && (channels & 3) == 0, "scale_channels: bad shape");
    SGV3D_REQUIRE(x && gate && y, "scale_channels: null pointer");
    const long long total4 = (long long)batch * pixels * (channels / 4);
    hipLaunchKernelGGL(scale_channels_kernel, dim3(cdiv(total4, kBlock)), dim3(kBlock), 0, as_stream(stream), total4,
                       pixels, channels / 4, reinterpret_cast<const float4 *>(x), reinterpret_cast<const float4 *>(gate),
                       reinterpret_cast<float4 *>(y));
    return check_launch("scale_channels_kernel");
}

extern "C" int sgv3d_copy_channels(int batch, int pixels, int channels, int x_ld, int x_coff, const float *x, float *y,
                                   void *stream) {
    SGV3D_REQUIRE(batch > 0 && pixels > 0 && channels > 0 && x_coff >= 0 && x_ld >= x_coff + channels, "copy_channels: bad shape");
    SGV3D_REQUIRE(x && y, "copy_channels: null pointer");
    const long long total = (long long)batch * pixels * channels;
    hipLaunchKernelGGL(copy_channels_kernel, dim3(cdiv(total, kBlock)), dim3(kBlock), 0, as_stream(stream), total, channels,
                       x_ld, x_coff, x, y);
    return check_launch("copy_channels_kernel");
}

extern "C" int sgv3d_upsample_bilinear2x(int batch, int h, int w, int channels, const float *x, float *y, void *stream) {
    SGV3D_REQUIRE(batch > 0 && h > 0 && w > 0 && channels > 0, "upsample_bilinear2x: bad shape");
    SGV3D_REQUIRE(x && y, "upsample_bilinear2x: null pointer");
    if (channels & 3) {
        const long long n = (long long)batch * 4 * h * w * channels;
        hipLaunchKernelGGL(upsample2x_scalar_kernel, dim3(cdiv(n, kBlock)), dim3(kBlock), 0, as_stream(stream), batch, h, w,
                           channels, x, y);
        return check_launch("upsample2x_scalar_kernel");
    }
    const long long total = (long long)batch * 4 * h * w * (channels / 4);
    hipLaunchKernelGGL(upsample_bilinear2x_kernel, dim3(cdiv(total, kBlock)), dim3(kBlock), 0, as_stream(stream), batch, h, w,
                       channels / 4, reinterpret_cast<const float4 *>(x), reinterpret_cast<float4 *>(y));
    return check_launch("upsample_bilinear2x_kernel");
}

extern "C" int sgv3d_add_mul_sigmoid(long long n, const float *a, const float *b, const float *c, float *y, void *stream) {
    SGV3D_REQUIRE(n > 0 && (n & 3) == 0, "add_mul_sigmoid: n must be a positive multiple of 4");
    SGV3D_REQUIRE(a && b && c && y, "add_mul_sigmoid: null pointer");
    hipLaunchKernelGGL(add_mul_sigmoid_kernel, dim3(cdiv(n / 4, kBlock)), dim3(kBlock), 0, as_stream(stream), n / 4,
                       reinterpret_cast<const float4 *>(a), reinterpret_cast<const float4 *>(b),
                       reinterpret_cast<const float4 *>(c), reinterpret_cast<float4 *>(y));
    return check_launch("add_mul_sigmoid_kernel");
}

extern "C" int sgv3d_bsm_compose(int batch, int pixels, int num_depth, int context_channels, int semantic_channels,
                                 int ld, const float *semantic_logits, int semantic_ld, float background_threshold,
                                 float *height_context, void *stream) {
    SGV3D_REQUIRE(batch > 0 && pixels > 0 && num_depth > 0 && context_channels > 0 && semantic_channels > 0 &&
                      ld >= num_depth + context_channels + semantic_channels && semantic_ld >= semantic_channels,
                  "bsm_compose: bad shape");
    SGV3D_REQUIRE(semantic_logits && height_context, "bsm_compose: null pointer");
    const long long px = (long long)batch * pixels;
    hipLaunchKernelGGL(bsm_compose_kernel, dim3(cdiv(px, kBlock / 32)), dim3(kBlock), 0, as_stream(stream), px, num_depth,
                       context_channels, semantic_channels, ld, semantic_logits, semantic_ld, background_threshold,
                       height_context);
// ... 35 lines not shown
```

### sgv3d_amd/hip_ops.py

```python
import ctypes
from collections import namedtuple
from functools import partialmethod

import torch

from . import _lib, conv_tiles, pack_cache
from ._lib import ConvDesc, CONV_NORMAL, CONV_DECONV, CONV_NCHW_OUT, CONV_GROUP_PLANES
from .conv_tiles import (TILE_WINO, TILE_WINO_RES, TILE_PATCH, TILE_WINO_HALF, TILE_WINO4, TILE_WINO4_WIDE, TILE_WINO4_NARROW,
                         TILE_WINO4_OCC, TILE_WINO4_G48, TILE_F4RES)


def _st(t):
    return _lib.stream_handle(t.device)


PROFILE = None
AUTOTUNE = not __import__("os").environ.get("SGV3D_NO_AUTOTUNE")
DETERMINISTIC = __import__("os").environ.get("SGV3D_DETERMINISTIC", "0") not in ("", "0")


def deterministic():
    return DETERMINISTIC or torch.are_deterministic_algorithms_enabled()
PROFILE_DETAIL = False
import os as _os
# ... 30 lines not shown
    path = path or _tune_db_path()
    if path and os.path.exists(path):
        with open(path) as f:
            loaded = {k: tuple(v) for k, v in json.load(f).items()}
        TUNE_DB.update(loaded)
        _COMMITTED_SIGS.difference_update(loaded)
    return len(TUNE_DB)


def save_tune_db(path=None):
    import json
    path = path or _tune_db_path()
    if path:
        with open(path, "w") as f:
            json.dump({k: list(v) for k, v in TUNE_DB.items()}, f, indent=0, sort_keys=True)


def load_default_tune_dbs():
    import glob
    import os
    if os.environ.get("SGV3D_NO_TUNE_DB"):
        return 0
    root = os.path.join(os.path.dirname(os.path.dirname(os.path.abspath(__file__))), "tune")
    skip = {x for x in os.environ.get("SGV3D_TUNE_SKIP", "").split(",") if x}
    n = 0
    for f in sorted(glob.glob(os.path.join(root, "gfx950_*.json"))):
        if os.path.basename(f) in skip:
            continue
        with open(f) as fh:
            sigs = list(__import__("json").load(fh))
        n += load_tune_db(f) and 1
        _COMMITTED_SIGS.update(sigs)
    return n


_ARCH_IS_GFX950 = {}


def _is_gfx950(device):
    idx = torch.device(device).index or 0
    if idx not in _ARCH_IS_GFX950:
        _ARCH_IS_GFX950[idx] = "gfx950" in str(getattr(torch.cuda.get_device_properties(idx), "gcnArchName", ""))
    return _ARCH_IS_GFX950[idx]


def tune_lookup(sig, device):
    if not AUTOTUNE or sig not in TUNE_DB or (sig in _COMMITTED_SIGS and not _is_gfx950(device)):
        return None
    return TUNE_DB[sig]


def tune_may_measure():
    return AUTOTUNE and not deterministic() and not torch.cuda.is_current_stream_capturing()


def tune_record(sig, entry):
    TUNE_DB[sig] = entry
    _COMMITTED_SIGS.discard(sig)


def tune_best_of(sig, device, baseline, candidates):
    baseline()
    t0 = time_callable(baseline, device)
    best, t1 = None, None
    for key, fn in candidates:
        fn()
        dt = time_callable(fn, device)
        if TUNE_VERBOSE:
            print(f"[tune] {sig}: {key}: {dt * 1e3 / TUNE_ROUNDS:.1f} us (baseline {t0 * 1e3 / TUNE_ROUNDS:.1f} us)", flush=True)
        if t1 is None or dt < t1:
            best, t1 = key, dt
    return t0, best, t1


load_default_tune_dbs()
load_tune_db()
TILES = conv_tiles.TILES
TILE_NAMES = {t: T.label for t, T in TILES.items()}
MFIRST = _os.environ.get("SGV3D_MFIRST", "1") != "0"
WINO4_X3_TILES = conv_tiles.family("wino4_x3")
X3_TILE_ROWS = {t: TILES[t].bm for t in WINO4_X3_TILES}
X3_TILE_COLS = {t: TILES[t].bn for t in WINO4_X3_TILES}
WINO4_TILES = conv_tiles.family("wino4", "wino4_x3")
WINO4_G48 = _os.environ.get("SGV3D_WINO4_G48", "1") != "0"
WINO4_X3 = _os.environ.get("SGV3D_WINO4_X3", "1") != "0"
PW_X3 = _os.environ.get("SGV3D_PW_X3", "1") != "0"
PW_X3_TILES = conv_tiles.family("pw_x3")
PW_X3_DIMS = {t: (TILES[t].bm, TILES[t].bn) for t in PW_X3_TILES}


def _pw_x3_tiles(gemm_m, gemm_n, nkt=None, mfirst=True, skip=()):
    out = ()
    for t in PW_X3_TILES:
        bm, bn = PW_X3_DIMS[t]
        wgs = -(-gemm_m // bm) * -(-gemm_n // bn)
        if (bm, bn) in skip or (bn == 256 and gemm_n < 256) or (TILES[t].mfirst and not (mfirst and MFIRST and gemm_n > bn)):
            continue
        if (wgs >= 96 or (SPLIT_K and nkt is not None and nkt >= 16)) and (bn >= 128 or gemm_n <= 64 or wgs < 1024):
            out += (t,)
    return out


def _split_factors(policy, nk, wgs):
    if not SPLIT_K:
        return ()
    pol = conv_tiles.SPLIT_POLICY[policy]
    return tuple(s for s in conv_tiles.SPLITS if nk // s >= pol["min_k"] and wgs < pol["max_wgs"] and wgs * s <= pol["max_total"])


F4RES = _os.environ.get("SGV3D_F4RES", "1") != "0"
OCC5_TILES = conv_tiles.select("igemm", occ5=True) + conv_tiles.select("igemm", occ5=True, mfirst=True)
OCC5 = _os.environ.get("SGV3D_OCC5", "1") != "0"
WINO4 = _os.environ.get("SGV3D_WINO4", "1") != "0"
WINO4_MIN_CHANNELS = 128
WINO_HALF = _os.environ.get("SGV3D_WINO_HALF", "1") != "0"
PATCH_BF16 = _os.environ.get("SGV3D_PATCH_BF16", "1") != "0"
DW_TILES = conv_tiles.family("dw_bf16")
DW_DEEP_TILES = conv_tiles.select("dw_bf16", deep=True)
DW_DEEP = _os.environ.get("SGV3D_DW_DEEP", "1") != "0"
DW_NARROW = _os.environ.get("SGV3D_DW_NARROW", "1") != "0"
DW_DEEP_MAX_WGS = int(_os.environ.get("SGV3D_DW_DEEP_MAX_WGS", "768"))
DW_BF16 = _os.environ.get("SGV3D_DW_BF16", "1") != "0"
DW_SPLIT_K = _os.environ.get("SGV3D_DW_SPLITK", "1") != "0"


class prof:
    __slots__ = ("name", "flops", "nbytes", "extra", "e0")

    def __init__(self, name, flops=0.0, nbytes=0.0, extra=None):
        self.name, self.flops, self.nbytes, self.extra, self.e0 = name, flops, nbytes, extra, None

    def __enter__(self):
        if PROFILE is not None:
            self.e0 = torch.cuda.Event(enable_timing=True)
            self.e0.record()
        return self

    def __exit__(self, *exc):
        if self.e0 is not None:
            e1 = torch.cuda.Event(enable_timing=True)
            e1.record()
            PROFILE.append((self.name, self.flops, self.e0, e1, self.nbytes, self.extra))
            self.e0 = None
        return False


def heuristic_tile(M, N):
    best, best_cost = 1, None
    for t, pen in zip(conv_tiles.select("igemm"), (1.0, 1.06, 1.06, 1.18)):
        bm, bn = TILES[t].bm, TILES[t].bn
        tiles = -(-M // bm) * -(-N // bn)
        cost = -(-tiles // 256) * bm * bn * pen
        if best_cost is None or cost < best_cost:
            best, best_cost = t, cost
    return best


def pack_geometry(k, n):
    kp, np_ = ctypes.c_int(), ctypes.c_int()
    _lib.load().sgv3d_conv_pack_geometry(int(k), int(n), ctypes.byref(kp), ctypes.byref(np_))
    return kp.value, np_.value


def fold_bn(bn, conv_bias=None):
    with torch.no_grad():
        inv = torch.rsqrt(bn.running_var.float() + bn.eps)
# ... 305 lines not shown
                raise _lib.SGV3DError(f"conv output buffer {got} does not match {want}")
        y_ld = int(out.shape[1] if nchw_out else out.shape[-1])
        if group_planes:
            y_ld, y_coff = self.cout, 0
        d = ConvDesc()
        d.batch, d.in_h, d.in_w, d.cin = B, H, W, self.cin
        d.out_h, d.out_w, d.cout = oh, ow, self.cout
        d.kh, d.kw, d.stride, d.pad, d.dil = self.kh, self.kw, self.stride, self.pad, self.dil
        d.x_ld, d.x_coff, d.y_ld, d.y_coff = x_ld, int(x_coff), y_ld, int(y_coff)
        d.res_ld = int(residual.shape[-1]) if residual is not None else 0
        d.relu = 1 if self.relu else 0
        d.mode = CONV_DECONV if self.transposed else (CONV_NCHW_OUT if nchw_out else CONV_NORMAL)
        d.deconv_ks = self.ks
        if group_planes:
            d.mode, d.deconv_ks = CONV_GROUP_PLANES, int(group_planes)
        d.k_pad, d.cout_pad = self.k_pad, self.cout_pad
        d.x_nchw = 0
        d.k_order = self.k_order
        lib = _lib.load()
        gemm_m = B * (H * W if self.transposed else oh * ow)
        gemm_n = self.cout * (self.ks * self.ks if self.transposed else 1)
        nkt = self.k_pad // 32
        t = int(self.tile if tile is None else tile)
        sk = int(split_k) if split_k else 0
        if t == 0 or sk == 0:
            key = (B, H, W, t, sk, MFMA_BF16, MFMA_F32X3, d.mode, residual is not None, gate is not None, io)
            choice = self._tile_cache.get(key)
            if choice is None:
                sig = (f"{self.cout}x{self.cin}k{self.kh}x{self.kw}s{self.stride}p{self.pad}d{self.dil}"
                       f"ks{self.ks}|{B}x{H}x{W}|m{d.mode}r{int(residual is not None)}g{int(gate is not None)}|{t}.{sk}"
                       + ("|bf16" if MFMA_BF16 else "|f32x3" if MFMA_F32X3 is True else "|x3auto" if MFMA_F32X3 else "")
                       + (f"|io{io}" if io else "") + f"|ts{TUNE_STREAMS}")
                choice = self._db_choice(sig, d, x, gate, gemm_m, gemm_n, nkt, t, sk, io)
                if choice is not None:
                    self._tile_cache[key] = choice
                    TUNE_STATS["from_db"] += 1
                elif tune_may_measure():
                    TUNE_STATS["measured"] += 1
                    choice = self._autotune(lib, d, x, residual, gate, out, gemm_m, gemm_n, nkt, t, sk, io)
                    self._tile_cache[key] = choice
                    tune_record(sig, choice)
                else:
                    choice = self._rule(t, sk, d, gemm_m, gemm_n, gate)
            t, sk = choice
        d.tile, d.split_k = t, sk
        name, flops, nbytes, extra = self._profile_record(TILES[t], sk, x, out, residual, gemm_m, io)
        with torch.cuda.device(x.device), prof(name, flops, nbytes, extra):
            rc = self._launch(lib, d, x, residual, gate, out, io)
        _lib.check(rc, "sgv3d_conv2d_forward")
        return out

    def _profile_record(self, T, sk, x, out, residual, gemm_m, io):
        B, H, W, _ = (int(s) for s in x.shape)
        ks2 = self.ks * self.ks if self.transposed else 1
        real_n = self.cout_real * ks2
        flops = 2.0 * gemm_m * real_n * (self.cin_real * self.kh * self.kw)
        plain = T.family == "igemm"
        x3 = plain and (T.x3 or (MFMA_F32X3 is True and not (T.mfirst or T.occ5)))
        name = (("conv_igemm_bf16_" if MFMA_BF16 else "conv_igemm_f32x3_" if x3 else "conv_igemm_") if plain else "conv_") + T.label
        pw1 = self.kh == 1 and self.kw == 1 and self.stride == 1 and self.pad == 0
        if plain and self.k_order == 0:
            name += "_tapmajor"
        elif plain and not MFMA_BF16 and not x3:
            if pw1 and not self.transposed and (T.occ5 or self.cin >= 128) and (T.occ5 or T.bm == 64):
                name += "_pw"
            if T.occ5:
                name += "_occ5"
        nbytes = (float(x.element_size()) * B * H * W * self.cin_real
                  + (2.0 if MFMA_BF16 else 4.0) * self.cout_real * self.cin_real * self.kh * self.kw * ks2
                  + float(out.element_size()) * gemm_m * real_n
                  + (float(residual.element_size()) * gemm_m * real_n if residual is not None else 0.0))
        if PROFILE_DETAIL:
            name += (f"|{B}x{H}x{W}x{self.cin}->{self.cout} k{self.kh if not self.transposed else -self.ks} "
                     f"s{self.stride} d{self.dil} splitk{sk}" + (" mfirst" if plain and T.mfirst else "") + (" occ5" if T.occ5 else ""))
        if io:
            name = name.replace("conv_igemm_bf16_", "conv_igemm_bf16io_")
        extra = None
        if PROFILE is not None and not MFMA_BF16 and not x3 and T.symbol:
            b = lambda v: "true" if v else "false"
            symbol = T.symbol.format(chunk=b(self.k_order != 0), pw=b(name.endswith(("_pw", "_pw_occ5"))),
                                     kmode=2 if self.k_order == 0 else 0 if pw1 else 1)
            if T.flops == "wino4":
                oh, ow = self.out_hw(H, W)
                dil = max(1, self.dil)
                tiles = B * dil * dil * -(-(-(-oh // dil)) // 4) * -(-(-(-ow // dil)) // 4)
                mfma = 2.0 * 36 * (-(-tiles // T.bm) * T.bm) * self.cin * self.cout
            elif T.flops == "direct_k32":
                mfma = 2.0 * gemm_m * self.cout * _up32(self.cin * self.kh * self.kw)
            else:
                mfma = 2.0 * gemm_m * self.cout * self.cin * self.kh * self.kw * ks2
            extra = {"symbol": symbol, "mfma_flops": mfma}
            if T.x3:
                extra["bf16_mfma_flops"] = 6 * mfma
        return name, flops, nbytes, extra

    def _rule(self, t, sk, d, gemm_m, gemm_n, gate=None):
        if t == 0 and self.wino_ok and WINOGRAD and not MFMA_BF16 and d.out_h * d.out_w * d.batch >= 1024:
            wgs = d.batch * -(-d.out_h // 16) * -(-d.out_w // 16) * -(-gemm_n // 64)
            split = 1
            if not sk and SPLIT_K:
                for cand in (2, 3, 4, 6, 8):
                    if wgs * cand <= 512 and self.cin // 8 // cand >= 4:
                        split = cand
            return TILE_WINO, sk or split
        if t == 0 and self._patch_eligible(d, gate) and d.out_h * d.out_w * d.batch >= 4096:
            wgs = d.batch * -(-d.out_h // 16) * -(-d.out_w // 32) * -(-gemm_n // 64)
            split = 1
            if not sk and SPLIT_K:
                for cand in (2, 3, 4, 6, 8):
                    if wgs * cand <= 512 and self.cin // 32 // cand >= 2:
                        split = cand
            return TILE_PATCH, sk or split
        return (t or heuristic_tile(gemm_m, gemm_n)), (sk or 1)

    def _patch_eligible(self, d, gate=None):
        return (MFMA_BF16 and not MFMA_F32X3 and PATCH_BF16 and self.patch_ok and d.mode == CONV_NORMAL and gate is None
                and d.x_ld % 8 == 0 and d.x_coff % 8 == 0 and d.y_ld % 8 == 0 and d.y_coff % 8 == 0
                and (d.res_ld % 8 == 0))

    def _launch(self, lib, d, x, residual, gate, out, io=0):
        T = TILES[d.tile]
        ws, nws = None, 0
        if d.split_k > 1 and T.family != "dw_bf16":
            nws = lib.sgv3d_conv2d_workspace_bytes(ctypes.byref(d))
            ws = torch.empty(nws, dtype=torch.uint8, device=x.device)
        tail = (_lib.ptr(self.scale), _lib.ptr(self.shift), _lib.ptr(residual))
        return getattr(self, "_launch_" + T.entry)(lib, T, d, x, tail, gate, out, io, ws, nws)

    @staticmethod
    def _abi(d, T, k_pad=None, cout_pad=None):
        a = ConvDesc.from_buffer_copy(d)
        if T.abi is not None:
            a.tile = T.abi
        if k_pad is not None:
            a.k_pad, a.cout_pad = k_pad, cout_pad
        return ctypes.byref(a)

    def _launch_conv2d(self, lib, T, d, x, tail, gate, out, io, ws, nws):
        x3 = T.x3 or (MFMA_F32X3 is True)
        if T.occ5 and (MFMA_BF16 or x3 or io or self.k_order != 1):
            raise _lib.SGV3DError("the five-per-CU 64x64 tile is f32 only and needs channel-chunk-major weights (cin % 32 == 0)")
        if io:
            return lib.sgv3d_conv2d_forward_bf16io(self._abi(d, T), x.data_ptr(), self._bf16_weights().data_ptr(), *tail, _lib.ptr(gate),
                                                   out.data_ptr(), _lib.ptr(ws), nws, _st(x), int(io))
        fwd = (lib.sgv3d_conv2d_forward_bf16 if MFMA_BF16 else
               lib.sgv3d_conv2d_forward_f32x3 if x3 else lib.sgv3d_conv2d_forward)
        return fwd(self._abi(d, T), x.data_ptr(), self.w.data_ptr(), *tail, _lib.ptr(gate), out.data_ptr(), _lib.ptr(ws), nws, _st(x))

    def _launch_winograd(self, lib, T, d, x, tail, gate, out, io, ws, nws):
        if not self.wino_ok:
            raise _lib.SGV3DError("this layer has no Winograd weights (needs 3x3 / stride 1 / pad 1 / cin % 8 == 0)")
        return lib.sgv3d_conv2d_winograd_forward(self._abi(d, T), x.data_ptr(), self.w_wino.data_ptr(), *tail, _lib.ptr(gate),
                                                 out.data_ptr(), _lib.ptr(ws), nws, _st(x))

    def _launch_winograd4(self, lib, T, d, x, tail, gate, out, io, ws, nws):
        if not self.wino4_ok(d, gate) or d.split_k > 1:
            raise _lib.SGV3DError("F(4x4) Winograd covers f32 3x3 / stride 1 / pad 1 layers with cin % 32 == 0, cout % 4 == 0, "
                                  "NHWC output, no gate, no split-K")
        u = self._form(T.form)
        a = self._abi(d, T, self.cin, self.wino4_x3_cout_pad) if T.x3 else self._abi(d, T, *self.wino4_geom)
        nws4 = lib.sgv3d_conv2d_winograd4_workspace_bytes(a)
        ws4 = torch.empty(nws4, dtype=torch.uint8, device=x.device)
        return lib.sgv3d_conv2d_winograd4_forward(a, x.data_ptr(), u.data_ptr(), *tail, out.data_ptr(), ws4.data_ptr(), nws4, _st(x))

    def _launch_f4res(self, lib, T, d, x, tail, gate, out, io, ws, nws):
        if not self.f4res_ok(d, gate, io) or d.split_k > 1 or x.dtype != torch.float32:
            raise _lib.SGV3DError("the resident F(4x4) kernel covers f32 3x3 / stride 1 / pad 1 layers with 64 input channels "
                                  "(cout % 64 == 0) or 64 output channels (cin % 64 == 0), NHWC output, no gate, no split-K")
# ... 29 lines not shown
        global _TUNE_SIDE_STREAMS
        cur = torch.cuda.current_stream(x.device)
        if len(_TUNE_SIDE_STREAMS) < TUNE_STREAMS:
            _TUNE_SIDE_STREAMS = [torch.cuda.Stream(device=x.device) for _ in range(TUNE_STREAMS)]
        best = None
        rounds = rounds or TUNE_ROUNDS
        for _ in range(TUNE_REPEATS):
            e0 = torch.cuda.Event(enable_timing=True)
            e1 = torch.cuda.Event(enable_timing=True)
            e0.record(cur)
            for s in _TUNE_SIDE_STREAMS[:TUNE_STREAMS]:
                s.wait_event(e0)
                with torch.cuda.stream(s):
                    for _r in range(rounds):
                        self._launch(lib, d, x, residual, gate, out, io)
                cur.wait_stream(s)
            e1.record(cur)
            e1.synchronize()
            dt = e0.elapsed_time(e1)
            best = dt if best is None else min(best, dt)
        return best

    def _candidates(self, d, gate, gemm_m, gemm_n, nkt, fixed_tile, fixed_split, io=0):
        sel = conv_tiles.select
        mfirst = lambda t: MFIRST and d.mode in (CONV_NORMAL, CONV_NCHW_OUT) and gemm_n > TILES[t].bn
        tiles = sel("igemm") + tuple(t for t in sel("igemm", mfirst=True) if mfirst(t))
        if OCC5 and self.k_order == 1 and not MFMA_BF16 and not MFMA_F32X3 and io == 0:
            tiles += sel("igemm", occ5=True) + tuple(t for t in sel("igemm", occ5=True, mfirst=True) if mfirst(t))
        if MFMA_F32X3 == "auto" and not MFMA_BF16:
            tiles += sel("igemm", x3=True)
        if self.wino_ok and WINOGRAD and not MFMA_BF16:
            tiles += (TILE_WINO,)
            if WINO_HALF:
                tiles += (TILE_WINO_HALF,)
            if self.cin <= 96 and self.cout >= 128:
                tiles += (TILE_WINO_RES,)

        if self.wino4_ok(d, gate):
            tiles += ((TILE_WINO4, TILE_WINO4_WIDE) + ((TILE_WINO4_NARROW,) if self.cin >= 128 else ()) + ((TILE_WINO4_OCC,) if OCC5 else ())
                      + ((TILE_WINO4_G48,) if WINO4_G48 and self.k_order == 1 else ()))
            if WINO4_X3 and not MFMA_F32X3:
                tiles += self._x3_tiles(d)
        if self.f4res_ok(d, gate, io):
            tiles += (TILE_F4RES,)
        if self.pw_x3_ok(d, gate, io):
            tiles += _pw_x3_tiles(gemm_m, gemm_n, nkt)
        if self._patch_eligible(d, gate):
            tiles += (TILE_PATCH,)
        if self._dw_eligible(d, gate, io):
            dw = lambda bm, bn, deep=False: (conv_tiles.by_shape("dw_bf16", bm, bn, deep),)
            deep = self.kh * self.kw * self.cin >= 512
            tiles += (dw(64, 256) + (dw(128, 256) if deep else ()) if gemm_n > 128 else
                      dw(128, 128) + (dw(256, 128) if deep else ()) if gemm_n > 64 else dw(128, 128) + dw(256, 64))
            if DW_DEEP and self.kh * self.kw * self.cin >= 256:
                if gemm_n > 128 and -(-gemm_m // 64) * -(-gemm_n // 256) <= DW_DEEP_MAX_WGS:
                    tiles += dw(64, 256, True)
                    if DW_NARROW and -(-gemm_m // 64) * -(-gemm_n // 256) <= 384:
                        tiles += dw(64, 128) + dw(64, 128, True)
                elif 64 < gemm_n <= 128 and -(-gemm_m // 128) * -(-gemm_n // 128) <= DW_DEEP_MAX_WGS:
                    tiles += dw(128, 128, True)
        if fixed_tile:
            tiles = (fixed_tile,)
        cands = []
        for t in tiles:
            T = TILES[t]
            wgs = -(-gemm_m // T.bm) * -(-gemm_n // T.bn)
            nk = nkt
            if T.spatial:
                th, tw, kc = T.spatial
                nk = self.cin // kc
                wgs = d.batch * -(-d.out_h // th) * -(-d.out_w // tw) * -(-gemm_n // T.bn)
            if T.family == "dw_bf16":
                nk = -(-(self.kh * self.kw * (self.cin // 32)) // 2)
            if T.split is None or (T.family == "dw_bf16" and (d.mode != CONV_NORMAL or not DW_SPLIT_K)):
                splits = (1,)
            elif fixed_split:
                splits = (fixed_split,)
            else:
                splits = (1,) + _split_factors(T.split, nk, wgs)
            cands.append((t, splits))
        return cands

    def _x3_tiles(self, d):
        dil = max(1, int(d.dil))
        tiles = d.batch * dil * dil * -(-(-(-d.out_h // dil)) // 4) * -(-(-(-d.out_w // dil)) // 4)
        waste = {r: (-(-tiles // r) * r - tiles) / tiles for r in sorted(set(X3_TILE_ROWS.values()))}
        best = min(waste.values())
        ms = [r for r in waste if waste[r] <= max(best, 0.10) and (r <= 64 or tiles >= r)]
        idle = lambda c: -(-self.cout // c) * c - self.cout
        cols = [128] + ([160] if idle(160) < idle(128) else [])
        return tuple(conv_tiles.by_shape("wino4_x3", r, c) for c in cols for r in ms)

    def _db_choice(self, sig, d, x, gate, gemm_m, gemm_n, nkt, fixed_tile, fixed_split, io=0):
        choice = tune_lookup(sig, x.device)
        if choice is None:
            return None
        t, sk = int(choice[0]), int(choice[1])
        for ct, splits in self._candidates(d, gate, gemm_m, gemm_n, nkt, fixed_tile, fixed_split, io):
            if ct == t and sk in splits:
                return (t, sk)
        del TUNE_DB[sig]
        _COMMITTED_SIGS.discard(sig)
        return None

    def _autotune(self, lib, d, x, residual, gate, out, gemm_m, gemm_n, nkt, fixed_tile, fixed_split, io=0):
        cands = self._candidates(d, gate, gemm_m, gemm_n, nkt, fixed_tile, fixed_split, io)
        best, best_t = (cands[0][0], fixed_split or 1), None
        with torch.cuda.device(x.device):
            for t, splits in cands:
                for sk in splits:
                    d.tile, d.split_k = t, sk
                    _lib.check(self._launch(lib, d, x, residual, gate, out, io), "sgv3d_conv2d_forward")
                    if TUNE_STREAMS > 1:
                        dt = self._time_under_load(lib, d, x, residual, gate, out, io=io)
                    else:
                        nrep = max(4, TUNE_ROUNDS * TUNE_REPEATS // 2)
                        evs = [torch.cuda.Event(enable_timing=True) for _ in range(nrep + 1)]
                        evs[0].record()
                        for r in range(nrep):
                            self._launch(lib, d, x, residual, gate, out, io)
                            evs[r + 1].record()
                        evs[-1].synchronize()
                        dt = min(evs[r].elapsed_time(evs[r + 1]) for r in range(nrep))
                    if TUNE_VERBOSE:
                        print(f"[tune] {self.cout}x{self.cin}k{self.kh} {d.batch}x{d.in_h}x{d.in_w}: tile {t} split {sk}: {dt * 1e3:.1f} us", flush=True)
                    if best_t is None or dt < best_t:
                        best, best_t = (t, sk), dt
        return best


PAIR_BF16 = _os.environ.get("SGV3D_PAIR_BF16", "1") != "0"


PARALLEL_BRANCHES = _os.environ.get("SGV3D_PARALLEL_BRANCHES", "0") == "1"
_BRANCH_POOL = {}
_BRANCH_TOP = {}


_OWNED_STREAMS = {}


def distinct_stream(device, avoid=()):
    dev = torch.device(device)
    key = dev.index if dev.index is not None else torch.cuda.current_device()
    taken = _OWNED_STREAMS.setdefault(key, set())
    banned = {st.cuda_stream for st in avoid if st is not None} | {torch.cuda.current_stream(dev).cuda_stream} | taken
    for _ in range(64):
        st = torch.cuda.Stream(device=dev)
        if st.cuda_stream not in banned:
            if len(taken) < 24:
                taken.add(st.cuda_stream)
            return st
    return torch.cuda.Stream(device=dev)


def release_stream(st):
    for taken in _OWNED_STREAMS.values():
        taken.discard(st.cuda_stream)


def run_parallel(device, thunks):
    thunks = list(thunks)
    if len(thunks) <= 1 or not PARALLEL_BRANCHES or not torch.cuda.is_current_stream_capturing():
        return [t() for t in thunks]
    dev = torch.device(device)
    key = dev.index if dev.index is not None else torch.cuda.current_device()
    pool = _BRANCH_POOL.setdefault(key, [])
    top = _BRANCH_TOP.get(key, 0)
    if top > 0:
        return [t() for t in thunks]
    need = top + len(thunks) - 1
    while len(pool) < need:
        pool.append(distinct_stream(dev, pool))
    mine = pool[top:need]
    _BRANCH_TOP[key] = need
    cur = torch.cuda.current_stream(dev)
    results = [None] * len(thunks)
    try:
        for st, (i, t) in zip(mine, list(enumerate(thunks))[1:]):
            st.wait_stream(cur)
            with torch.cuda.stream(st):
                results[i] = t()
        results[0] = thunks[0]()
    finally:
        for st in mine:
            cur.wait_stream(st)
        _BRANCH_TOP[key] = top
    return results


_GRAPH_SPLIT_HOOK = None


def graph_split_point(tag):
    if _GRAPH_SPLIT_HOOK is not None:
        _GRAPH_SPLIT_HOOK(tag)


def switch_state():
    g = globals()
    return tuple(g.get(k) for k in ("AUTOTUNE", "SPLIT_K", "WINOGRAD", "FUSED_HEAD", "HEAD_PATH", "MFMA_BF16", "BF16_ACTIVATIONS",
                                    "MFMA_F32X3", "MFIRST", "WINO4", "WINO_HALF", "PATCH_BF16", "DW_BF16", "DW_DEEP", "DW_NARROW",
                                    "DW_SPLIT_K", "DW_DEEP_MAX_WGS", "PAIR_BF16", "TUNE_STREAMS", "PARALLEL_BRANCHES", "F4RES", "OCC5", "WINO4_G48", "DCN_FUSED", "WINO4_X3", "PW_X3",
                                    "DCN_FUSED_BF16", "DCN_FUSED_TRAIN", "TRAIN_BF16_STORAGE", "SHORTCUT_X3", "DECONV_X3", "VIT_BF16", "STEM_FUSED"))


def conv_pair_eligible(a, b, x, residual=None):
    return (MFMA_BF16 and not MFMA_F32X3 and DW_BF16 and PAIR_BF16 and x.dtype == torch.bfloat16 and not a.transposed and not b.transposed
            and a.cout == 256 and a.cin % 32 == 0 and int(x.shape[-1]) % 8 == 0 and b.cin == 256 and b.kh == 1 and b.kw == 1
            and b.stride == 1 and b.pad == 0 and b.cout % 256 == 0 and (residual is None or residual.dtype == torch.bfloat16))


def conv_pair_bf16(a, b, x, residual=None, out=None):
    B, H, W, x_ld = (int(v) for v in x.shape)
    oh, ow = a.out_hw(H, W)
    if out is None:
        out = torch.empty(B, oh, ow, b.cout, dtype=torch.bfloat16, device=x.device)
    d = ConvDesc()
    d.batch, d.in_h, d.in_w, d.cin = B, H, W, a.cin
    d.out_h, d.out_w, d.cout = oh, ow, a.cout
    d.kh, d.kw, d.stride, d.pad, d.dil = a.kh, a.kw, a.stride, a.pad, a.dil
    d.x_ld, d.x_coff, d.y_ld, d.y_coff = x_ld, 0, a.cout, 0
    d.relu, d.mode, d.split_k = (1 if a.relu else 0), CONV_NORMAL, 1
    flops = 2.0 * B * oh * ow * (a.cout_real * a.cin_real * a.kh * a.kw + b.cout_real * b.cin_real)
    name = "conv_dw_bf16_pair"
    if PROFILE_DETAIL:
        name += f"|{B}x{H}x{W}x{a.cin}->{a.cout} k{a.kh} s{a.stride} d{a.dil} ->{b.cout} k1"
    with torch.cuda.device(x.device), prof(name, flops):
        rc = _lib.load().sgv3d_conv_dw_bf16_pair_forward(
            ctypes.byref(d), x.data_ptr(), a._dw_weights().data_ptr(), _lib.ptr(a.scale), _lib.ptr(a.shift), b.cout,
            b._dw_weights().data_ptr(), _lib.ptr(b.scale), _lib.ptr(b.shift), _lib.ptr(residual),
            int(residual.shape[-1]) if residual is not None else 0, out.data_ptr(), int(out.shape[-1]), 0, 1 if b.relu else 0, _st(x))
    _lib.check(rc, "sgv3d_conv_dw_bf16_pair_forward")
    return out


def conv_pair_choice(a, b, x, residual=None):
    if not conv_pair_eligible(a, b, x, residual):
        return False
    B, H, W, _ = (int(v) for v in x.shape)
    sig = (f"pair|{a.cout}x{a.cin}k{a.kh}x{a.kw}s{a.stride}p{a.pad}d{a.dil}->{b.cout}|{B}x{H}x{W}|r{int(residual is not None)}|bf16|ts{TUNE_STREAMS}")
    hit = tune_lookup(sig, x.device)
    if hit is not None:
        return bool(hit[0])
    if not tune_may_measure():
        return True
    act = torch.bfloat16
    two = lambda: b(a(x, out_dtype=act), residual=residual, out_dtype=act)
    one = lambda: conv_pair_bf16(a, b, x, residual)
    two(); one()
    t2 = time_callable(two, x.device)
    t1 = time_callable(one, x.device)
    tune_record(sig, [1 if t1 < t2 else 0, 0])
    return t1 < t2


SHORTCUT_X3 = _os.environ.get("SGV3D_SHORTCUT_X3", "1") != "0"


def conv_shortcut_eligible(c3, ds, mid, x):
    if not (SHORTCUT_X3 and PW_X3 and not MFMA_BF16 and not MFMA_F32X3):
        return False
    if c3.transposed or ds.transposed or mid.dtype != torch.float32 or x.dtype != torch.float32:
        return False
    one = lambda c: c.kh == 1 and c.kw == 1 and c.pad == 0 and c.cin % 32 == 0
    if not (one(c3) and one(ds) and c3.stride == 1 and ds.stride in (1, 2) and not ds.relu and c3.cout == ds.cout and c3.cout % 4 == 0):
        return False
    B, H, W, x_ld = (int(v) for v in x.shape)
    return (tuple(int(v) for v in mid.shape[:3]) == (B,) + ds.out_hw(H, W) and int(mid.shape[-1]) % 4 == 0 and x_ld % 4 == 0
            and int(mid.shape[-1]) >= c3.cin and x_ld >= ds.cin)


def _shortcut_rule_tile(gemm_m, gemm_n):
    plain = {PW_X3_DIMS[t]: t for t in PW_X3_TILES if not TILES[t].mfirst}
    for bm in (128, 64):
        if -(-gemm_m // bm) * -(-gemm_n // 128) >= 512:
            return plain[bm, 128]
    return plain[32, 128]


def _shortcut_tiles(gemm_m, gemm_n):
    return _pw_x3_tiles(gemm_m, gemm_n, skip=((128, 64),)) or (_shortcut_rule_tile(gemm_m, gemm_n),)


def conv_shortcut_x3(c3, ds, mid, x, out=None, tile=None):
    B, H, W, x_ld = (int(v) for v in x.shape)
    oh, ow = ds.out_hw(H, W)
    assert mid.is_contiguous() and x.is_contiguous() and tuple(int(v) for v in mid.shape[:3]) == (B, oh, ow)
    if out is None:
        out = torch.empty(B, oh, ow, c3.cout, dtype=torch.float32, device=x.device)
    gemm_m = B * oh * ow
    T = TILES[int(tile or _shortcut_rule_tile(gemm_m, c3.cout))]
    if T.family != "pw_x3":
        raise _lib.SGV3DError(f"conv_shortcut_x3: tile {T.id} is not a tile of the f32x3 pointwise kernel")
    da, db = ConvDesc(), ConvDesc()
    for d, c, (h, w), ld in ((da, c3, (oh, ow), int(mid.shape[-1])), (db, ds, (H, W), x_ld)):
        d.batch, d.in_h, d.in_w, d.cin = B, h, w, c.cin
        d.out_h, d.out_w, d.cout = oh, ow, c.cout
        d.kh, d.kw, d.stride, d.pad, d.dil = 1, 1, c.stride, 0, 1
        d.x_ld, d.x_coff, d.y_ld, d.y_coff, d.res_ld = ld, 0, int(out.shape[-1]), 0, 0
        d.relu, d.mode, d.split_k, d.tile = (1 if c.relu else 0), CONV_NORMAL, 1, T.abi
        d.k_pad, d.k_order = c.k_pad, c.k_order
    ua, ub = c3._form(T.form), ds._form(T.form)
    da.cout_pad, db.cout_pad = c3.pw_x3_cout_pad, ds.pw_x3_cout_pad
    flops = 2.0 * gemm_m * (c3.cout_real * c3.cin_real + ds.cout_real * ds.cin_real)
    nbytes = 4.0 * (gemm_m * c3.cin_real + B * H * W * ds.cin_real + c3.cout_real * c3.cin_real + ds.cout_real * ds.cin_real
                    + gemm_m * c3.cout_real)
    name, extra = "conv_pw_x3_shortcut", None
    if PROFILE_DETAIL:
        name += f"|{B}x{oh}x{ow}x{c3.cin}->{c3.cout} k1 s1 + {B}x{H}x{W}x{ds.cin}->{ds.cout} k1 s{ds.stride}"
    if PROFILE is not None:
        mfma = 2.0 * gemm_m * c3.cout * (c3.cin + ds.cin)
        extra = {"symbol": f"conv_pw_x3_kernel<{T.bm // 16}, {T.bn // 32}, 3>", "mfma_flops": mfma, "bf16_mfma_flops": 6 * mfma}
    with torch.cuda.device(x.device), prof(name, flops, nbytes, extra):
        rc = _lib.load().sgv3d_conv2d_x3_shortcut_forward(
            ctypes.byref(da), mid.data_ptr(), ua.data_ptr(), _lib.ptr(c3.scale), _lib.ptr(c3.shift),
            ctypes.byref(db), x.data_ptr(), ub.data_ptr(), _lib.ptr(ds.scale), _lib.ptr(ds.shift), out.data_ptr(), _st(x))
    _lib.check(rc, "sgv3d_conv2d_x3_shortcut_forward")
    return out


def conv_shortcut_signature(c3, ds, x):
    B, H, W, _ = (int(v) for v in x.shape)
    return f"pair|shortcut|{c3.cout}x{c3.cin}+{ds.cin}s{ds.stride}|{B}x{H}x{W}|r{int(c3.relu)}|ts{TUNE_STREAMS}"


def conv_shortcut_choice(c3, ds, mid, x):
    if not conv_shortcut_eligible(c3, ds, mid, x):
        return 0
    gemm_m, gemm_n = int(mid.shape[0]) * int(mid.shape[1]) * int(mid.shape[2]), c3.cout
    rule = _shortcut_rule_tile(gemm_m, gemm_n)
    sig = conv_shortcut_signature(c3, ds, x)
    hit = tune_lookup(sig, x.device)
    if hit is not None:
        on, t = (int(v) for v in hit)
        if not on:
            return 0
        return t if t in PW_X3_TILES else rule
    if not tune_may_measure():
        return rule
    TUNE_STATS["measured"] += 1
    out = torch.empty(tuple(mid.shape[:3]) + (c3.cout,), dtype=torch.float32, device=x.device)
    t2, best, t1 = tune_best_of(sig, x.device, lambda: c3(mid, out, residual=ds(x)),
                                [(t, lambda t=t: conv_shortcut_x3(c3, ds, mid, x, out, tile=t)) for t in _shortcut_tiles(gemm_m, gemm_n)])
    on = t1 < t2
    tune_record(sig, [1, best] if on else [0, 0])
    return best if on else 0

DECONV_X3 = _os.environ.get("SGV3D_DECONV_X3", "1") != "0"


def deconv_x3_eligible(conv, x, out=None, y_coff=0):
    if not (DECONV_X3 and PW_X3 and not MFMA_BF16 and not MFMA_F32X3):
        return False
    if not conv.transposed or conv.ks < 1 or conv.cin % 32 or conv.cout % 4 or x.dtype != torch.float32 or x.dim() != 4:
        return False
    x_ld = int(x.shape[-1])
    if x_ld % 4 or x_ld < conv.cin or int(y_coff) % 4 or int(y_coff) < 0:
        return False
    if out is not None:
        B, H, W, _ = (int(v) for v in x.shape)
        return (out.dtype == torch.float32 and out.dim() == 4 and tuple(int(v) for v in out.shape[:3]) == (B,) + conv.out_hw(H, W)
                and int(out.shape[-1]) % 4 == 0 and int(out.shape[-1]) >= int(y_coff) + conv.cout)
    return True


def _deconv_x3_rule(gemm_m, gemm_n):
    return _shortcut_rule_tile(gemm_m, gemm_n), 1


def _deconv_x3_candidates(gemm_m, gemm_n, nkt):
    wgs = lambda t: -(-gemm_m // TILES[t].bm) * -(-gemm_n // TILES[t].bn)
    out = tuple((t, (1,) + _split_factors("igemm", nkt, wgs(t))) for t in _pw_x3_tiles(gemm_m, gemm_n, nkt, mfirst=False))
    return out or ((_shortcut_rule_tile(gemm_m, gemm_n), (1,)),)


def deconv_x3(conv, x, out=None, y_coff=0, tile=None, split_k=None):
    B, H, W, x_ld = (int(v) for v in x.shape)
    oh, ow = conv.out_hw(H, W)
    assert x.is_contiguous() and conv.transposed
    if out is None:
        out = torch.empty(B, oh, ow, conv.cout, dtype=torch.float32, device=x.device)
    assert out.is_contiguous() and out.dtype == torch.float32 and tuple(int(v) for v in out.shape[:3]) == (B, oh, ow)
    gemm_m, gemm_n = B * H * W, conv.ks * conv.ks * conv.cout
    rule_t, rule_s = _deconv_x3_rule(gemm_m, gemm_n)
    T = TILES[int(tile or rule_t)]
    sk = int(split_k or rule_s)
    if T.family != "pw_x3":
        raise _lib.SGV3DError(f"deconv_x3: tile {T.id} is not a tile of the f32x3 pointwise kernel")
    u = conv._form("w_pw_x3_deconv")
    d = ConvDesc()
    d.batch, d.in_h, d.in_w, d.cin = B, H, W, conv.cin
    d.out_h, d.out_w, d.cout = oh, ow, conv.cout
    d.kh, d.kw, d.stride, d.pad, d.dil = 1, 1, 1, 0, 1
    d.x_ld, d.x_coff, d.y_ld, d.y_coff, d.res_ld = x_ld, 0, int(out.shape[-1]), int(y_coff), 0
    d.relu, d.mode, d.deconv_ks, d.split_k, d.tile = (1 if conv.relu else 0), CONV_DECONV, conv.ks, sk, T.abi
    d.k_pad, d.cout_pad, d.k_order = conv.cin, conv.pw_x3_deconv_cout_pad, 1
    ws, nws = None, 0
    if sk > 1:
        nws = 4 * sk * gemm_m * gemm_n
        ws = torch.empty(nws, dtype=torch.uint8, device=x.device)
    real_n = conv.cout_real * conv.ks * conv.ks
    flops = 2.0 * gemm_m * real_n * conv.cin_real
    nbytes = 4.0 * (gemm_m * conv.cin_real + real_n * conv.cin_real + gemm_m * real_n)
    name, extra = "conv_pw_x3_deconv", None
    if PROFILE_DETAIL:
        name += f"|{B}x{H}x{W}x{conv.cin}->{conv.cout} k{-conv.ks} s1 d1 splitk{sk}"
    if PROFILE is not None:
        mfma = 2.0 * gemm_m * gemm_n * conv.cin
        extra = {"symbol": f"conv_pw_x3_kernel<{T.bm // 16}, {T.bn // 32}, 4>", "mfma_flops": mfma, "bf16_mfma_flops": 6 * mfma}
    with torch.cuda.device(x.device), prof(name, flops, nbytes, extra):
        rc = _lib.load().sgv3d_conv2d_x3_forward(ctypes.byref(d), x.data_ptr(), u.data_ptr(), _lib.ptr(conv.scale), _lib.ptr(conv.shift),
                                                 None, out.data_ptr(), _lib.ptr(ws), nws, _st(x))
    _lib.check(rc, "sgv3d_conv2d_x3_forward")
    return out


def deconv_x3_signature(conv, x):
    B, H, W, _ = (int(v) for v in x.shape)
    return f"pair|deconv|{conv.cout}x{conv.cin}ks{conv.ks}|{B}x{H}x{W}|r{int(conv.relu)}|ts{TUNE_STREAMS}"


def deconv_x3_choice(conv, x, out=None, y_coff=0):
    if not deconv_x3_eligible(conv, x, out, y_coff):
        return None
    B, H, W, _ = (int(v) for v in x.shape)
    gemm_m, gemm_n, nkt = B * H * W, conv.ks * conv.ks * conv.cout, conv.cin // 32
    rule = _deconv_x3_rule(gemm_m, gemm_n)
    sig = deconv_x3_signature(conv, x)
    hit = tune_lookup(sig, x.device)
# ... 504 lines not shown
```

### sgv3d_amd/layers/backbones/lss_fpn.py

```python
import ctypes

import numpy as np
import torch
from torch import nn

from ... import _lib, hip_ops
from ...hip_ops import PackedConv, fold_bn
from ...calibration import CalibrationCache
from ...ops.voxel_pooling import VoxelPlan
from ..blocks import BasicBlock, HipModule, build_backbone, build_neck, conv_bn

import os as _os

CACHE_CAMERA_GATES = _os.environ.get("SGV3D_CACHE_CAMERA_GATES", "1") != "0"
GATED_CALIBRATION = _os.environ.get("SGV3D_GATED_CALIBRATION", "1") != "0"
FOLD_ASPP_POOL = _os.environ.get("SGV3D_FOLD_ASPP_POOL", "1") != "0"
FUSE_LIFT_SPLAT = _os.environ.get("SGV3D_FUSE_LIFT_SPLAT", "1") != "0"

__all__ = ['LSSFPN']


class _ASPPModule(HipModule):

    def __init__(self, inplanes, planes, kernel_size, padding, dilation, BatchNorm):
        super().__init__()
        self.atrous_conv = nn.Conv2d(inplanes, planes, kernel_size=kernel_size, stride=1, padding=padding,
                                     dilation=dilation, bias=False)
        self.bn = BatchNorm(planes)
        self.relu = nn.ReLU()
        torch.nn.init.kaiming_normal_(self.atrous_conv.weight)

    def hip_compile(self, device):
        return conv_bn(self.atrous_conv, self.bn, True, device)


class ASPP(HipModule):

    def __init__(self, inplanes, mid_channels=256, BatchNorm=nn.BatchNorm2d):
        super().__init__()
        dilations = [1, 6, 12, 18]
        self.aspp1 = _ASPPModule(inplanes, mid_channels, 1, padding=0, dilation=dilations[0], BatchNorm=BatchNorm)
        self.aspp2 = _ASPPModule(inplanes, mid_channels, 3, padding=dilations[1], dilation=dilations[1], BatchNorm=BatchNorm)
        self.aspp3 = _ASPPModule(inplanes, mid_channels, 3, padding=dilations[2], dilation=dilations[2], BatchNorm=BatchNorm)
        self.aspp4 = _ASPPModule(inplanes, mid_channels, 3, padding=dilations[3], dilation=dilations[3], BatchNorm=BatchNorm)
        self.global_avg_pool = nn.Sequential(
            nn.AdaptiveAvgPool2d((1, 1)),
            nn.Conv2d(inplanes, mid_channels, 1, stride=1, bias=False),
            BatchNorm(mid_channels),
            nn.ReLU(),
        )
        self.conv1 = nn.Conv2d(int(mid_channels * 5), mid_channels, 1, bias=False)
        self.bn1 = BatchNorm(mid_channels)
        self.relu = nn.ReLU()
        self.dropout = nn.Dropout(0.5)
        self.mid_channels = mid_channels
        for m in (self.global_avg_pool[1], self.conv1):
            torch.nn.init.kaiming_normal_(m.weight)

    def hip_compile(self, device):
        gscale, gshift = fold_bn(self.global_avg_pool[2])
        mid = self.mid_channels
        s = dict(
            gap_w=self.global_avg_pool[1].weight.detach().reshape(mid, -1).to(device).float().contiguous(),
            gap_scale=gscale.to(device), gap_shift=gshift.to(device),
            conv1=conv_bn(self.conv1, self.bn1, True, device))
        w1 = self.conv1.weight.detach()
        scale1, shift1 = fold_bn(self.bn1)
        s['conv1_head'] = PackedConv(w1[:, :4 * mid].contiguous(), scale=scale1, shift=shift1, relu=True, device=device)
        s['conv1_tail_w'] = w1[:, 4 * mid:].reshape(mid, mid).to(device).float().contiguous()
        s['bn1_scale'], s['bn1_shift'] = scale1.to(device).float().contiguous(), shift1.to(device).float().contiguous()
        return s

    def hip_forward(self, x):
        s = self.hip_state(x.device)
        B, H, W, _ = x.shape
        mid = self.mid_channels
        fold = FOLD_ASPP_POOL and B == 1 and x.dtype == torch.float32 and not hip_ops.MFMA_BF16
        cat = torch.empty(B, H, W, (4 if fold else 5) * mid, dtype=x.dtype, device=x.device)
        folded = [None]

        def pooled_branch():
            pooled = hip_ops.global_avgpool(x)
            x5 = hip_ops.dense(pooled, s['gap_w'], s['gap_scale'], s['gap_shift'], hip_ops.ACT_RELU)
            if fold:
                folded[0] = hip_ops.dense(x5, s['conv1_tail_w'], s['bn1_scale'], s['bn1_shift'], hip_ops.ACT_NONE)
            else:
                hip_ops.broadcast_channels(x5, cat, y_coff=4 * mid)

        def conv_branches():
            for i, m in enumerate((self.aspp1, self.aspp2, self.aspp3, self.aspp4)):
                m.hip_state(x.device)(x, cat, y_coff=i * mid)
        hip_ops.run_parallel(x.device, (conv_branches, pooled_branch))
        if fold:
            return s['conv1_head'](cat, shift=folded[0].view(-1), out_dtype=x.dtype)
        return s['conv1'](cat, out_dtype=x.dtype)


class Mlp(nn.Module):

    def __init__(self, in_features, hidden_features=None, out_features=None, act_layer=nn.ReLU, drop=0.0):
        super().__init__()
        out_features = out_features or in_features
        hidden_features = hidden_features or in_features
        self.fc1 = nn.Linear(in_features, hidden_features)
        self.act = act_layer()
        self.drop1 = nn.Dropout(drop)
        self.fc2 = nn.Linear(hidden_features, out_features)
        self.drop2 = nn.Dropout(drop)


class SELayer(nn.Module):

    def __init__(self, channels, act_layer=nn.ReLU, gate_layer=nn.Sigmoid):
        super().__init__()
        self.conv_reduce = nn.Conv2d(channels, channels, 1, bias=True)
        self.act1 = act_layer()
        self.conv_expand = nn.Conv2d(channels, channels, 1, bias=True)
        self.gate = gate_layer()


class DCN(HipModule):

    def __init__(self, in_channels, out_channels, kernel_size=3, padding=1, groups=1, deform_groups=1,
                 stride=1, dilation=1, im2col_step=32, **unused):
        super().__init__()
        assert kernel_size == 3 and padding == 1 and stride == 1 and dilation == 1 and deform_groups == 1
        assert in_channels % groups == 0 and out_channels % groups == 0
        self.in_channels, self.out_channels, self.groups = in_channels, out_channels, groups
        self.weight = nn.Parameter(torch.empty(out_channels, in_channels // groups, 3, 3))
        nn.init.kaiming_uniform_(self.weight, nonlinearity='relu')
        self.conv_offset = nn.Conv2d(in_channels, deform_groups * 2 * 9, kernel_size=3, stride=1, padding=1, bias=True)
        nn.init.zeros_(self.conv_offset.weight)
        nn.init.zeros_(self.conv_offset.bias)

    def hip_compile(self, device):
        g = self.groups
        opg, cpg = self.out_channels // g, self.in_channels // g
        convs = []
        for gi in range(g):
            wg = self.weight.detach()[gi * opg:(gi + 1) * opg]
            wg = wg.permute(0, 2, 3, 1).reshape(opg, 9 * cpg, 1, 1).contiguous()
            convs.append(PackedConv(wg, device=device))
        dcn_bf16 = None
        if hip_ops.deform_conv3x3_bf16_covers(self.in_channels, g, self.out_channels):
            dcn_bf16 = hip_ops.PackedDeformBf16(self.weight, g, device=device)
        return dict(offset=conv_bn(self.conv_offset, None, False, device), convs=convs, opg=opg, cpg=cpg, dcn_bf16=dcn_bf16)

    def hip_forward(self, x):
        s = self.hip_state(x.device)
        B, H, W, C = x.shape
        offset = s['offset'](x)
        if hip_ops.deform_conv3x3_eligible(x, s['convs']):
            return hip_ops.deform_conv3x3(x, offset, s['convs'])
        if s['dcn_bf16'] is not None and hip_ops.deform_conv3x3_bf16_eligible(x, self.groups, self.out_channels):
            return hip_ops.deform_conv3x3_bf16(x, offset, s['dcn_bf16'])
        col = hip_ops.deform_im2col3x3(x, offset, self.groups)
        out = torch.empty(B, H, W, self.out_channels, dtype=x.dtype, device=x.device)
        for gi, conv in enumerate(s['convs']):
            conv(col, out, x_coff=gi * 9 * s['cpg'], y_coff=gi * s['opg'])
        return out


class HeightNet(HipModule):

    def __init__(self, in_channels, mid_channels, context_channels, height_channels):
        super().__init__()
        self.reduce_conv = nn.Sequential(
            nn.Conv2d(in_channels, mid_channels, kernel_size=3, stride=1, padding=1),
            nn.BatchNorm2d(mid_channels),
            nn.ReLU(inplace=True),
        )
        self.context_conv = nn.Conv2d(mid_channels, context_channels, kernel_size=1, stride=1, padding=0)
        self.bn = nn.BatchNorm1d(27)
        self.height_mlp = Mlp(27, mid_channels, mid_channels)
# ... 315 lines not shown
```

Before: 293.1.

## Batch dilated ASPP Winograd F(4x4) convs into one multi-layer launch with packed dilation lattice

Adds a multi-layer Winograd F(4x4) path that runs the three dilated ASPP 3x3 convs on a shared input in combined launches, with block ranges selecting each layer's arguments. It also changes dilated tiling from per-phase tiles to a packed lattice that stacks dilation phases along each axis, which can reduce padded tiles. The global avgpool is moved into a shared header and its reduction is split into more chunks with a parallel final stage. The multi path is autotuned against running the convs separately, so the gain depends on tuning, and the lattice code adds index arithmetic to every tile.

```diff
diff --git a/include/sgv3d_hip.h b/include/sgv3d_hip.h
--- a/include/sgv3d_hip.h
+++ b/include/sgv3d_hip.h
@@ -163,10 +163,16 @@
                                      const float *scale_b, const float *bias_b, float *y, void *stream);
 int sgv3d_stem_pool_x3_forward(int batch, int h, int w, const float *x_nchw, const void *w_x3, size_t w_bytes, const float *scale,
                                const float *shift, float *y_nhwc, int y_ld, int variant, void *stream);
+int sgv3d_wino4_lattice_axis(int n, int dil, int tile, int k0, int count, int *tiles, int *stacked, int *pixels);
 size_t sgv3d_conv2d_winograd4_workspace_bytes(const sgv3d_conv_desc *desc );
 int sgv3d_conv2d_winograd4_forward(const sgv3d_conv_desc *desc , const float *x, const float *u_packed,
                                    const float *scale, const float *bias, const float *residual, float *y,
                                    void *workspace, size_t workspace_bytes, void *stream);
+
+size_t sgv3d_conv2d_winograd4_multi_workspace_bytes(int n, const sgv3d_conv_desc *descs );
+int sgv3d_conv2d_winograd4_forward_multi(int n, const sgv3d_conv_desc *descs , const float *x, const void *const *u_packed,
+                                         const float *const *scale, const float *const *bias, float *const *y, void *workspace,
+                                         size_t workspace_bytes, void *stream);
 
 void sgv3d_conv_pack_geometry(int k, int n, int *k_pad, int *n_pad);
 
diff --git a/sgv3d_amd/_lib.py b/sgv3d_amd/_lib.py
--- a/sgv3d_amd/_lib.py
+++ b/sgv3d_amd/_lib.py
@@ -107,8 +107,11 @@
     "sgv3d_conv2d_x3_forward": (c_int, [c_void_p] * 8 + [c_size_t, c_void_p]),
     "sgv3d_conv2d_x3_shortcut_forward": (c_int, [c_void_p] * 12),
     "sgv3d_stem_pool_x3_forward": (c_int, [c_int] * 3 + [c_void_p, c_void_p, c_size_t] + [c_void_p] * 3 + [c_int, c_int, c_void_p]),
+    "sgv3d_wino4_lattice_axis": (c_int, [c_int] * 5 + [c_void_p] * 3),
     "sgv3d_conv2d_winograd4_workspace_bytes": (c_size_t, [ctypes.POINTER(ConvDesc)]),
     "sgv3d_conv2d_winograd4_forward": (c_int, [ctypes.POINTER(ConvDesc)] + [c_void_p] * 7 + [c_size_t, c_void_p]),
+    "sgv3d_conv2d_winograd4_multi_workspace_bytes": (c_size_t, [c_int, c_void_p]),
+    "sgv3d_conv2d_winograd4_forward_multi": (c_int, [c_int] + [c_void_p] * 7 + [c_size_t, c_void_p]),
     "sgv3d_maxpool3x3s2": (c_int, [c_int] * 4 + [c_void_p] * 3),
     "sgv3d_maxpool3x3s2_bf16": (c_int, [c_int] * 4 + [c_void_p] * 3),
     "sgv3d_nchw_to_nhwc": (c_int, [c_int] * 5 + [c_void_p] * 3),
diff --git a/sgv3d_amd/csrc/act_bf16.hip b/sgv3d_amd/csrc/act_bf16.hip
--- a/sgv3d_amd/csrc/act_bf16.hip
+++ b/sgv3d_amd/csrc/act_bf16.hip
@@ -1,4 +1,5 @@
 #include "common.hpp"
+#include "avgpool.hpp"
 
 using namespace sgv3d;
 
@@ -9,7 +10,6 @@
 typedef float f32x4 __attribute__((ext_vector_type(4)));
 
 constexpr int kBlock = 256;
-constexpr int kAvgChunks = 32;
 
 struct F8 {
     float v[8];
@@ -42,32 +42,14 @@
     st8(y + i * 8, v);
 }
 
-__global__ __launch_bounds__(kBlock) void global_avgpool_bf16_partial_kernel(int P, int C, int ld, const __bf16 *__restrict__ x,
-                                                                             float *__restrict__ part) {
-    __shared__ float red[4][64];
-    const int b = blockIdx.z, chunk = blockIdx.y;
-    const int c = blockIdx.x * 64 + (threadIdx.x & 63);
-    const int g = threadIdx.x >> 6;
-    const int per = (P + kAvgChunks - 1) / kAvgChunks;
-    const int p0 = chunk * per, p1 = min(P, p0 + per);
-    float s = 0.f;
-    if (c < C)
-        for (int p = p0 + g; p < p1; p += 4) s += (float)x[((long long)b * P + p) * ld + c];
-    red[g][threadIdx.x & 63] = s;
-    __syncthreads();
-    if (g == 0 && c < C)
-        part[((long long)b * kAvgChunks + chunk) * C + c] =
-            (red[0][threadIdx.x] + red[1][threadIdx.x]) + (red[2][threadIdx.x] + red[3][threadIdx.x]);
-}
-
-__global__ __launch_bounds__(kBlock) void global_avgpool_bf16_final_kernel(int B, int P, int C, const float *__restrict__ part,
-                                                                           float *__restrict__ y) {
-    const long long i = (long long)blockIdx.x * kBlock + threadIdx.x;
-    if (i >= (long long)B * C) return;
-    const int b = (int)(i / C), c = (int)(i - (long long)b * C);
-    float s = 0.f;
-    for (int k = 0; k < kAvgChunks; ++k) s += part[((long long)b * kAvgChunks + k) * C + c];
-    y[i] = s / (float)P;
+__global__ __launch_bounds__(kAvgBlock) void global_avgpool_bf16_partial_kernel(int P, int C, int ld, const __bf16 *__restrict__ x,
+                                                                                float *__restrict__ part) {
+    avgpool_partial_scalar(P, C, ld, x, part);
+}
+
+__global__ __launch_bounds__(kAvgBlock) void global_avgpool_bf16_final_kernel(int P, int C, const float *__restrict__ part,
+                                                                              float *__restrict__ y) {
+    avgpool_final(P, C, part, y);
 }
 
 __global__ __launch_bounds__(kBlock) void broadcast_channels_bf16_kernel(long long total8, int P, int C8, int ld, int coff,
@@ -184,10 +166,10 @@
     if (workspace_bytes < sizeof(float) * (size_t)batch * kAvgChunks * channels)
         return fail(SGV3D_ENOSPACE, "global_avgpool_bf16: workspace too small (sgv3d_global_avgpool_workspace_bytes)");
     float *part = static_cast<float *>(workspace);
-    hipLaunchKernelGGL(global_avgpool_bf16_partial_kernel, dim3(cdiv(channels, 64), kAvgChunks, batch), dim3(kBlock), 0,
+    hipLaunchKernelGGL(global_avgpool_bf16_partial_kernel, dim3(cdiv(channels, 64), kAvgChunks, batch), dim3(kAvgBlock), 0,
                        as_stream(stream), pixels, channels, x_ld, static_cast<const __bf16 *>(x), part);
-    hipLaunchKernelGGL(global_avgpool_bf16_final_kernel, dim3(cdiv((long long)batch * channels, kBlock)), dim3(kBlock), 0,
-                       as_stream(stream), batch, pixels, channels, part, y);
+    hipLaunchKernelGGL(global_avgpool_bf16_final_kernel, dim3(cdiv(channels, 32), batch), dim3(kAvgBlock), 0, as_stream(stream), pixels,
+                       channels, part, y);
     return check_launch("global_avgpool_bf16_kernel");
 }
 
diff --git a/sgv3d_amd/csrc/avgpool.hpp b/sgv3d_amd/csrc/avgpool.hpp
--- /dev/null
+++ b/sgv3d_amd/csrc/avgpool.hpp
@@ -0,0 +1,54 @@
+#pragma once
+#include "common.hpp"
+
+namespace sgv3d {
+
+constexpr int kAvgBlock = 256;
+constexpr int kAvgChunks = 128;
+constexpr int kAvgFinalLanes = 8;
+static_assert(kAvgChunks % kAvgFinalLanes == 0 && kAvgBlock == 32 * kAvgFinalLanes, "final stage: 32 channels x 8 lanes");
+
+__device__ __forceinline__ void avgpool_chunk(int P, int chunk, int &p0, int &p1) {
+    const int per = (P + kAvgChunks - 1) / kAvgChunks;
+    p0 = chunk * per;
+    p1 = min(P, p0 + per);
+}
+
+template <typename T>
+__device__ __forceinline__ void avgpool_partial_scalar(int P, int C, int ld, const T *__restrict__ x, float *__restrict__ part) {
+    __shared__ float red[4][64];
+    const int b = blockIdx.z, chunk = blockIdx.y;
+    const int c = blockIdx.x * 64 + (threadIdx.x & 63);
+    const int g = threadIdx.x >> 6;
+    int p0, p1;
+    avgpool_chunk(P, chunk, p0, p1);
+    float s = 0.f;
+    if (c < C)
+        for (int p = p0 + g; p < p1; p += 4) s += (float)x[((long long)b * P + p) * ld + c];
+    red[g][threadIdx.x & 63] = s;
+    __syncthreads();
+    if (g == 0 && c < C)
+        part[((long long)b * kAvgChunks + chunk) * C + c] =
+            (red[0][threadIdx.x] + red[1][threadIdx.x]) + (red[2][threadIdx.x] + red[3][threadIdx.x]);
+}
+
+__device__ __forceinline__ void avgpool_final(int P, int C, const float *__restrict__ part, float *__restrict__ y) {
+    __shared__ float red[kAvgFinalLanes][32];
+    constexpr int kPer = kAvgChunks / kAvgFinalLanes;
+    const int b = blockIdx.y, c = blockIdx.x * 32 + (threadIdx.x & 31), k = threadIdx.x >> 5;
+    float s = 0.f;
+    if (c < C) {
+        const float *p = part + ((long long)b * kAvgChunks + k * kPer) * C + c;
+#pragma unroll
+        for (int j = 0; j < kPer; ++j) s += p[(long long)j * C];
+    }
+    red[k][threadIdx.x & 31] = s;
+    __syncthreads();
+    if (k == 0 && c < C) {
+        const int t = threadIdx.x;
+        const float s01 = red[0][t] + red[1][t], s23 = red[2][t] + red[3][t], s45 = red[4][t] + red[5][t], s67 = red[6][t] + red[7][t];
+        y[(long long)b * C + c] = ((s01 + s23) + (s45 + s67)) / (float)P;
+    }
+}
+
+}
diff --git a/sgv3d_amd/csrc/conv_wino4.hip b/sgv3d_amd/csrc/conv_wino4.hip
--- a/sgv3d_amd/csrc/conv_wino4.hip
+++ b/sgv3d_amd/csrc/conv_wino4.hip
@@ -42,49 +42,108 @@
 
 constexpr int kTB = 256;
 
+struct Wino4Axis {
+    int n, dil;
+    int tiles;
+    int per_phase;
+};
+
+__host__ __device__ inline Wino4Axis wino4_axis(int n, int dil) {
+    const int split = dil * (((n + dil - 1) / dil + 3) / 4), stacked = (n + dil - 1 + 3) / 4;
+    Wino4Axis a;
+    a.n = n;
+    a.dil = dil;
+    a.tiles = stacked < split ? stacked : split;
+    a.per_phase = stacked < split ? 0 : split / dil;
+    return a;
+}
+
+template <int N>
+__host__ __device__ __forceinline__ void wino4_axis_pixels(const Wino4Axis &ax, int t, int k0, int (&pix)[N]) {
+    if (ax.per_phase) {
+        const int p = t / ax.per_phase, e0 = 4 * (t - p * ax.per_phase) + k0;
+#pragma unroll
+        for (int k = 0; k < N; ++k) {
+            const int e = e0 + k, c = p + e * ax.dil;
+            pix[k] = (e >= 0 && c < ax.n) ? c : -1;
+        }
+        return;
+    }
+    const int q = ax.n / ax.dil, r = ax.n - q * ax.dil, head = r * (q + 2);
+    const int v = 4 * t + k0;
+    int p = -1, i = 0, len = 0;
+    if (v >= 0) {
+        if (v < head) {
+            p = v / (q + 2);
+            i = v - p * (q + 2);
+        } else {
+            const int u = (v - head) / (q + 1);
+            p = r + u;
+            i = v - head - u * (q + 1);
+        }
+        len = q + (p < r ? 1 : 0);
+    }
+#pragma unroll
+    for (int k = 0; k < N; ++k) {
+        pix[k] = ((unsigned)p < (unsigned)ax.dil && i < len) ? p + i * ax.dil : -1;
+        if (++i > len) {
+            ++p;
+            i = 0;
+            len = q + (p < r ? 1 : 0);
+        }
+    }
+}
+
+template <bool kDilated, int N>
+__device__ __forceinline__ void wino4_pixels(const Wino4Axis &ax, int t, int k0, int (&pix)[N]) {
+    if constexpr (kDilated) {
+        wino4_axis_pixels(ax, t, k0, pix);
+    } else {
+#pragma unroll
+        for (int k = 0; k < N; ++k) {
+            const int c = 4 * t + k0 + k;
+            pix[k] = (unsigned)c < (unsigned)ax.n ? c : -1;
+        }
+    }
+}
+
 struct Wino4Args {
     const float *x, *scale, *bias, *res;
     float *v, *m, *y;
     int batch, h, w, cin, cout, x_ld, x_coff, y_ld, y_coff, res_ld, relu;
-    int ty, tx;
-    int dil;
+    Wino4Axis ay, ax;
     int rows;
     int c0, cn;
     int gw;
 };
 
-__device__ __forceinline__ void wino4_tile(const Wino4Args &a, int t, int &b, int &py, int &px, int &iy, int &ix) {
-    const int per_phase = a.ty * a.tx, per_img = per_phase * a.dil * a.dil;
+__device__ __forceinline__ void wino4_tile(const Wino4Args &a, int t, int &b, int &ty, int &tx) {
+    const int per_img = a.ay.tiles * a.ax.tiles;
     b = t / per_img;
-    int r = t - b * per_img;
-    const int ph = r / per_phase;
-    r -= ph * per_phase;
-    py = ph / a.dil;
-    px = ph - py * a.dil;
-    iy = r / a.tx;
-    ix = r - iy * a.tx;
-}
-
+    const int r = t - b * per_img;
+    ty = r / a.ax.tiles;
+    tx = r - ty * a.ax.tiles;
+}
+
+template <bool kDilated>
 __global__ __launch_bounds__(kTB) void wino4_input_kernel(const Wino4Args a) {
     const int cq = a.cin >> 2;
     const long long i = (long long)blockIdx.x * kTB + threadIdx.x;
-    const long long ntile = (long long)a.batch * a.ty * a.tx * a.dil * a.dil;
+    const long long ntile = (long long)a.batch * a.ay.tiles * a.ax.tiles;
     if (i >= ntile * cq) return;
     const int t = (int)(i / cq), c = (int)(i - (long long)t * cq) * 4;
-    int b, py, px, iy, ix;
-    wino4_tile(a, t, b, py, px, iy, ix);
-    const int y0 = py + (4 * iy - 1) * a.dil, x0 = px + (4 * ix - 1) * a.dil;
+    int b, ty, tx;
+    wino4_tile(a, t, b, ty, tx);
+    int yy[6], xx[6];
+    wino4_pixels<kDilated>(a.ay, ty, -1, yy);
+    wino4_pixels<kDilated>(a.ax, tx, -1, xx);
     const float *xb = a.x + (size_t)b * a.h * a.w * a.x_ld + a.x_coff + c;
     f4 d[6][6];
 #pragma unroll
     for (int rr = 0; rr < 6; ++rr) {
-        const int yy = y0 + rr * a.dil;
-        const bool rok = (unsigned)yy < (unsigned)a.h;
-#pragma unroll
-        for (int cc = 0; cc < 6; ++cc) {
-            const int xx = x0 + cc * a.dil;
-            d[rr][cc] = (rok && (unsigned)xx < (unsigned)a.w) ? ld4(xb + ((size_t)yy * a.w + xx) * a.x_ld) : f4{0.f, 0.f, 0.f, 0.f};
-        }
+#pragma unroll
+        for (int cc = 0; cc < 6; ++cc)
+            d[rr][cc] = (yy[rr] >= 0 && xx[cc] >= 0) ? ld4(xb + ((size_t)yy[rr] * a.w + xx[cc]) * a.x_ld) : f4{0.f, 0.f, 0.f, 0.f};
     }
 #pragma unroll
     for (int cc = 0; cc < 6; ++cc) wino4_bt(d[0][cc], d[1][cc], d[2][cc], d[3][cc], d[4][cc], d[5][cc]);
@@ -98,15 +157,15 @@
     }
 }
 
-__global__ __launch_bounds__(kTB) void wino4_output_kernel(const Wino4Args a) {
+template <bool kDilated>
+__device__ __forceinline__ void wino4_output_body(const Wino4Args &a, const long long i) {
     const int cq = a.cn >> 2;
-    const long long i = (long long)blockIdx.x * kTB + threadIdx.x;
-    const long long ntile = (long long)a.batch * a.ty * a.tx * a.dil * a.dil;
+    const long long ntile = (long long)a.batch * a.ay.tiles * a.ax.tiles;
     if (i >= ntile * cq) return;
     const int t = (int)(i / cq), cl = (int)(i - (long long)t * cq) * 4;
     const int c = a.c0 + cl;
-    int b, py, px, iy, ix;
-    wino4_tile(a, t, b, py, px, iy, ix);
+    int b, ty, tx;
+    wino4_tile(a, t, b, ty, tx);
     const float *mb = a.m + (size_t)t * a.cn + cl;
     const size_t plane = (size_t)a.rows * a.cn;
     f4 rr_[4][6];
@@ -117,6 +176,9 @@
                  m4 = ld4(mb + (size_t)(4 * 6 + cc) * plane), m5 = ld4(mb + (size_t)(5 * 6 + cc) * plane);
         wino4_at(m0, m1, m2, m3, m4, m5, rr_[0][cc], rr_[1][cc], rr_[2][cc], rr_[3][cc]);
     }
+    int yy[4], xx[4];
+    wino4_pixels<kDilated>(a.ay, ty, 0, yy);
+    wino4_pixels<kDilated>(a.ax, tx, 0, xx);
     const f4 sc = a.scale ? ld4(a.scale + c) : f4{1.f, 1.f, 1.f, 1.f};
     const f4 sh = a.bias ? ld4(a.bias + c) : f4{0.f, 0.f, 0.f, 0.f};
     const float floor_ = a.relu ? 0.f : -__builtin_inff();
@@ -124,13 +186,11 @@
     for (int u = 0; u < 4; ++u) {
         f4 o[4];
         wino4_at(rr_[u][0], rr_[u][1], rr_[u][2], rr_[u][3], rr_[u][4], rr_[u][5], o[0], o[1], o[2], o[3]);
-        const int yy = py + (4 * iy + u) * a.dil;
-        if (yy >= a.h) continue;
+        if (yy[u] < 0) continue;
 #pragma unroll
         for (int v = 0; v < 4; ++v) {
-            const int xx = px + (4 * ix + v) * a.dil;
-            if (xx >= a.w) continue;
-            const size_t pix = ((size_t)b * a.h + yy) * a.w + xx;
+            if (xx[v] < 0) continue;
+            const size_t pix = ((size_t)b * a.h + yy[u]) * a.w + xx[v];
             f4 q = {fmaf(o[v].x, sc.x, sh.x), fmaf(o[v].y, sc.y, sh.y), fmaf(o[v].z, sc.z, sh.z), fmaf(o[v].w, sc.w, sh.w)};
             if (a.res) q = add4(q, ld4(a.res + pix * a.res_ld + c));
             q = {fmaxf(q.x, floor_), fmaxf(q.y, floor_), fmaxf(q.z, floor_), fmaxf(q.w, floor_)};
@@ -144,6 +204,30 @@
     }
 }
 
+template <bool kDilated>
+__global__ __launch_bounds__(kTB) void wino4_output_kernel(const Wino4Args a) {
+    wino4_output_body<kDilated>(a, (long long)blockIdx.x * kTB + threadIdx.x);
+}
+
+constexpr int kWino4Multi = 4;
+struct Wino4MultiArgs {
+    Wino4Args a[kWino4Multi];
+    int first[kWino4Multi + 1];
+    int n;
+};
+
+__device__ __forceinline__ int wino4_multi_layer(const Wino4MultiArgs &m) {
+    int l = 0;
+#pragma unroll
+    for (int k = 1; k < kWino4Multi; ++k) l += (k < m.n && (int)blockIdx.x >= m.first[k]) ? 1 : 0;
+    return l;
+}
+
+__global__ __launch_bounds__(kTB) void wino4_output_multi_kernel(const Wino4MultiArgs m) {
+    const int l = wino4_multi_layer(m);
+    wino4_output_body<true>(m.a[l], (long long)((int)blockIdx.x - m.first[l]) * kTB + threadIdx.x);
+}
+
 __global__ __launch_bounds__(256) void wino4_pack_weight_kernel(const float *__restrict__ w, int cout, int cin, int k_pad,
                                                                 int cout_pad, float *__restrict__ u) {
     const long long i = (long long)blockIdx.x * 256 + threadIdx.x;
@@ -192,26 +276,24 @@
     lo = __builtin_convertvector(r2, bf16x4);
 }
 
-__global__ __launch_bounds__(kTB) void wino4_input_x3_kernel(const Wino4Args a) {
+template <bool kDilated>
+__device__ __forceinline__ void wino4_input_x3_body(const Wino4Args &a, const long long i) {
     const int cq = a.cin >> 2;
-    const long long i = (long long)blockIdx.x * kTB + threadIdx.x;
-    const long long ntile = (long long)a.batch * a.ty * a.tx * a.dil * a.dil;
+    const long long ntile = (long long)a.batch * a.ay.tiles * a.ax.tiles;
     if (i >= ntile * cq) return;
     const int t = (int)(i / cq), c = (int)(i - (long long)t * cq) * 4;
-    int b, py, px, iy, ix;
-    wino4_tile(a, t, b, py, px, iy, ix);
-    const int y0 = py + (4 * iy - 1) * a.dil, x0 = px + (4 * ix - 1) * a.dil;
+    int b, ty, tx;
+    wino4_tile(a, t, b, ty, tx);
+    int yy[6], xx[6];
+    wino4_pixels<kDilated>(a.ay, ty, -1, yy);
+    wino4_pixels<kDilated>(a.ax, tx, -1, xx);
     const float *xb = a.x + (size_t)b * a.h * a.w * a.x_ld + a.x_coff + c;
     f4 d[6][6];
 #pragma unroll
     for (int rr = 0; rr < 6; ++rr) {
-        const int yy = y0 + rr * a.dil;
-        const bool rok = (unsigned)yy < (unsigned)a.h;
-#pragma unroll
-        for (int cc = 0; cc < 6; ++cc) {
-            const int xx = x0 + cc * a.dil;
-            d[rr][cc] = (rok && (unsigned)xx < (unsigned)a.w) ? ld4(xb + ((size_t)yy * a.w + xx) * a.x_ld) : f4{0.f, 0.f, 0.f, 0.f};
-        }
+#pragma unroll
+        for (int cc = 0; cc < 6; ++cc)
+            d[rr][cc] = (yy[rr] >= 0 && xx[cc] >= 0) ? ld4(xb + ((size_t)yy[rr] * a.w + xx[cc]) * a.x_ld) : f4{0.f, 0.f, 0.f, 0.f};
     }
 #pragma unroll
     for (int cc = 0; cc < 6; ++cc) wino4_bt(d[0][cc], d[1][cc], d[2][cc], d[3][cc], d[4][cc], d[5][cc]);
@@ -230,6 +312,24 @@
             *reinterpret_cast<bf16x4 *>(o + 64) = lo;
         }
     }
+}
+
+template <bool kDilated>
+__global__ __launch_bounds__(kTB) void wino4_input_x3_kernel(const Wino4Args a) {
+    wino4_input_x3_body<kDilated>(a, (long long)blockIdx.x * kTB + threadIdx.x);
+}
+
+__global__ __launch_bounds__(kTB) void wino4_input_x3_multi_kernel(const Wino4MultiArgs m) {
+    const int l = wino4_multi_layer(m);
+    wino4_input_x3_body<true>(m.a[l], (long long)((int)blockIdx.x - m.first[l]) * kTB + threadIdx.x);
+}
+
+__device__ __forceinline__ void split3_rounded(float v, __bf16 &hi, __bf16 &mid, __bf16 &lo) {
+#pragma clang fp contract(off)
+    hi = (__bf16)v;
+    const float r1 = v - (float)hi;
+    mid = (__bf16)r1;
+    lo = (__bf16)(r1 - (float)mid);
 }
 
 __global__ __launch_bounds__(256) void wino4_pack_weight_x3_kernel(const float *__restrict__ w, int cout, int cin, int k_pad,
@@ -266,11 +366,8 @@
                             (1.f / 24.f) * t[r][0] - (1.f / 12.f) * t[r][1] + (1.f / 6.f) * t[r][2], t[r][2]};
 #pragma unroll
         for (int c = 0; c < 6; ++c) {
-            const float v = o[c];
-            const __bf16 hi = (__bf16)v;
-            const float r1 = v - (float)hi;
-            const __bf16 mid = (__bf16)r1;
-            const __bf16 lo = (__bf16)(r1 - (float)mid);
+            __bf16 hi, mid, lo;
+            split3_rounded(o[c], hi, mid, lo);
             __bf16 *q = ub + (size_t)(r * 6 + c) * block;
             q[0] = hi;
             q[512] = mid;
@@ -279,11 +376,10 @@
     }
 }
 
-void wino4_geom(const sgv3d_conv_desc *d, int &ty, int &tx, long long &tiles, int &rows) {
-    const int dil = d->dil;
-    ty = cdiv(cdiv(d->out_h, dil), 4);
-    tx = cdiv(cdiv(d->out_w, dil), 4);
-    tiles = (long long)d->batch * dil * dil * ty * tx;
+void wino4_geom(const sgv3d_conv_desc *d, Wino4Axis &ay, Wino4Axis &ax, long long &tiles, int &rows) {
+    ay = wino4_axis(d->out_h, d->dil);
+    ax = wino4_axis(d->out_w, d->dil);
+    tiles = (long long)d->batch * ay.tiles * ax.tiles;
     const int g = (d->tile & SGV3D_TILE_X3) ? gemm_x3_tile_rows(d->tile & 15)
                   : (d->tile & ~SGV3D_TILE_OCC5) == SGV3D_TILE_32x128 ? 32 : d->tile == SGV3D_TILE_48x64 ? 48 : 64;
     rows = (int)((tiles + g - 1) / g * g);
@@ -318,11 +414,27 @@
     return check_launch("wino4_pack_weight_x3_kernel");
 }
 
+extern "C" int sgv3d_wino4_lattice_axis(int n, int dil, int tile, int k0, int count, int *tiles, int *stacked, int *pixels) {
+    SGV3D_REQUIRE(n > 0 && dil > 0, "wino4_lattice_axis: bad axis (n=%d dil=%d)", n, dil);
+    const Wino4Axis ax = wino4_axis(n, dil);
+    if (tiles) *tiles = ax.tiles;
+    if (stacked) *stacked = ax.per_phase == 0;
+    if (pixels) {
+        SGV3D_REQUIRE(tile >= 0 && tile < ax.tiles && (k0 == -1 || k0 == 0) && count >= 1 && count <= 6,
+                      "wino4_lattice_axis: bad tile / element range (tile=%d k0=%d count=%d)", tile, k0, count);
+        int pix[6];
+        wino4_axis_pixels(ax, tile, k0, pix);
+        for (int k = 0; k < count; ++k) pixels[k] = pix[k];
+    }
+    return SGV3D_OK;
+}
+
 extern "C" size_t sgv3d_conv2d_winograd4_workspace_bytes(const sgv3d_conv_desc *d) {
     if (!d || d->batch <= 0 || d->out_h <= 0 || d->out_w <= 0 || d->cin <= 0 || d->cout <= 0 || d->dil <= 0) return 0;
-    int ty, tx, rows;
+    Wino4Axis ay, ax;
+    int rows;
     long long tiles;
-    wino4_geom(d, ty, tx, tiles, rows);
+    wino4_geom(d, ay, ax, tiles, rows);
     if (d->tile & SGV3D_TILE_X3)
         return 36 * (size_t)rows * (6 * (size_t)d->cin + sizeof(float) * (size_t)wino4_chunk(d, rows));
     return sizeof(float) * 36 * (size_t)rows * ((size_t)d->cin + (size_t)wino4_chunk(d, rows));
@@ -356,8 +468,7 @@
     a.batch = d->batch; a.h = d->in_h; a.w = d->in_w; a.cin = d->cin; a.cout = d->cout;
     a.x_ld = d->x_ld; a.x_coff = d->x_coff; a.y_ld = d->y_ld; a.y_coff = d->y_coff; a.res_ld = d->res_ld; a.relu = d->relu;
     long long tiles;
-    wino4_geom(d, a.ty, a.tx, tiles, a.rows);
-    a.dil = d->dil;
+    wino4_geom(d, a.ay, a.ax, tiles, a.rows);
     SGV3D_REQUIRE(tiles < 0x7fffffffLL / 64, "conv2d_winograd4_forward: too many tiles");
     const bool x3 = (d->tile & SGV3D_TILE_X3) != 0;
     a.v = static_cast<float *>(workspace);
@@ -370,18 +481,21 @@
         SGV3D_REQUIRE(d->cin % 32 == 0 && d->cout_pad % 32 == 0 && d->cout_pad >= d->cout,
                       "conv2d_winograd4_forward: SGV3D_TILE_X3 needs cin %% 32 == 0 and cout_pad (a multiple of 32) of the x3 weights");
         SGV3D_REQUIRE((d->tile & 15) < 10, "conv2d_winograd4_forward: unknown SGV3D_TILE_X3 variant %d", d->tile & 15);
-        hipLaunchKernelGGL(wino4_input_x3_kernel, dim3(cdiv(tiles * (d->cin / 4), kTB)), dim3(kTB), 0, st, a);
+        if (d->dil > 1) hipLaunchKernelGGL(wino4_input_x3_kernel<true>, dim3(cdiv(tiles * (d->cin / 4), kTB)), dim3(kTB), 0, st, a);
+        else hipLaunchKernelGGL(wino4_input_x3_kernel<false>, dim3(cdiv(tiles * (d->cin / 4), kTB)), dim3(kTB), 0, st, a);
         const int chunk3 = wino4_chunk(d, a.rows);
         for (int c0 = 0; c0 < d->cout; c0 += chunk3) {
             a.c0 = c0;
             a.cn = d->cout - c0 < chunk3 ? d->cout - c0 : chunk3;
             if (int rc = conv_gemm_grouped_x3(a.v, static_cast<const unsigned char *>(static_cast<const void *>(u_packed)) + (size_t)c0 * d->cin * 6,
                                               a.m, a.rows, d->cin, a.cn, d->cout_pad - c0, d->tile & 15, st, (size_t)d->cout_pad * d->cin * 6)) return rc;
-            hipLaunchKernelGGL(wino4_output_kernel, dim3(cdiv(tiles * (a.cn / 4), kTB)), dim3(kTB), 0, st, a);
+            if (d->dil > 1) hipLaunchKernelGGL(wino4_output_kernel<true>, dim3(cdiv(tiles * (a.cn / 4), kTB)), dim3(kTB), 0, st, a);
+            else hipLaunchKernelGGL(wino4_output_kernel<false>, dim3(cdiv(tiles * (a.cn / 4), kTB)), dim3(kTB), 0, st, a);
         }
         return check_launch("conv2d_winograd4_forward(x3)");
     }
-    hipLaunchKernelGGL(wino4_input_kernel, dim3(cdiv(tiles * (d->cin / 4), kTB)), dim3(kTB), 0, st, a);
+    if (d->dil > 1) hipLaunchKernelGGL(wino4_input_kernel<true>, dim3(cdiv(tiles * (d->cin / 4), kTB)), dim3(kTB), 0, st, a);
+    else hipLaunchKernelGGL(wino4_input_kernel<false>, dim3(cdiv(tiles * (d->cin / 4), kTB)), dim3(kTB), 0, st, a);
     int tile = (d->tile == SGV3D_TILE_64x128 || d->tile == SGV3D_TILE_32x128 || d->tile == SGV3D_TILE_48x64) ? d->tile
                : (d->tile & SGV3D_TILE_OCC5) ? (SGV3D_TILE_64x64 | SGV3D_TILE_OCC5) : SGV3D_TILE_64x64;
     if (tile == SGV3D_TILE_32x128 && (d->k_order != 1 || d->cin < 128)) tile = SGV3D_TILE_64x64;
@@ -396,7 +510,93 @@
                                              d->cout_pad, st)) return rc;
         } else if (int rc = conv_gemm_grouped(a.v, u_packed + (size_t)c0 * d->k_pad, a.m, a.rows, 36, d->cin, a.cn, d->k_pad,
                                               d->cout_pad, d->k_order, tile, st)) return rc;
-        hipLaunchKernelGGL(wino4_output_kernel, dim3(cdiv(tiles * (a.cn / 4), kTB)), dim3(kTB), 0, st, a);
+        if (d->dil > 1) hipLaunchKernelGGL(wino4_output_kernel<true>, dim3(cdiv(tiles * (a.cn / 4), kTB)), dim3(kTB), 0, st, a);
+        else hipLaunchKernelGGL(wino4_output_kernel<false>, dim3(cdiv(tiles * (a.cn / 4), kTB)), dim3(kTB), 0, st, a);
     }
     return check_launch("conv2d_winograd4_forward");
 }
+
+namespace {
+
+int wino4_multi_check(const sgv3d_conv_desc *d, const sgv3d_conv_desc *d0, const void *u, const float *scale, const float *bias, const float *y) {
+    SGV3D_REQUIRE(u && y, "conv2d_winograd4_forward_multi: null pointer");
+    SGV3D_REQUIRE(d->kh == 3 && d->kw == 3 && d->stride == 1 && d->dil >= 1 && d->pad == d->dil,
+                  "conv2d_winograd4_forward_multi: only 3x3 / stride 1 / pad == dilation");
+    SGV3D_REQUIRE(d->batch > 0 && d->in_h > 0 && d->in_w > 0 && d->cin > 0 && d->cout > 0 && d->out_h == d->in_h && d->out_w == d->in_w,
+                  "conv2d_winograd4_forward_multi: bad sizes");
+    SGV3D_REQUIRE(d->batch == d0->batch && d->in_h == d0->in_h && d->in_w == d0->in_w && d->cin == d0->cin && d->x_ld == d0->x_ld &&
+                      d->x_coff == d0->x_coff,
+                  "conv2d_winograd4_forward_multi: the layers must read the same input (batch, map, cin, x_ld, x_coff)");
+    SGV3D_REQUIRE(d->mode == SGV3D_CONV_NORMAL && d->split_k <= 1, "conv2d_winograd4_forward_multi: NHWC output, no split-K");
+    SGV3D_REQUIRE((d->tile & SGV3D_TILE_X3) && (d->tile & 15) < 10, "conv2d_winograd4_forward_multi: SGV3D_TILE_X3 | variant tiles only");
+    SGV3D_REQUIRE(d->cin % 32 == 0 && d->cout % 4 == 0 && d->cout_pad % 32 == 0 && d->cout_pad >= d->cout && (d->x_ld & 3) == 0 &&
+                      (d->x_coff & 3) == 0 && (d->y_ld & 3) == 0 && (d->y_coff & 3) == 0,
+                  "conv2d_winograd4_forward_multi: cin %% 32, cout %% 4, cout_pad %% 32, leading dimensions and offsets %% 4");
+    SGV3D_REQUIRE(((reinterpret_cast<uintptr_t>(u) | reinterpret_cast<uintptr_t>(y) | reinterpret_cast<uintptr_t>(scale) |
+                    reinterpret_cast<uintptr_t>(bias)) & 15) == 0, "conv2d_winograd4_forward_multi: pointers must be 16-B aligned");
+    SGV3D_REQUIRE(d->x_ld >= d->x_coff + d->cin && d->y_ld >= d->y_coff + d->cout, "conv2d_winograd4_forward_multi: leading dimension too small");
+    return SGV3D_OK;
+}
+
+}
+
+extern "C" size_t sgv3d_conv2d_winograd4_multi_workspace_bytes(int n, const sgv3d_conv_desc *descs) {
+    if (!descs || n < 1 || n > kWino4Multi) return 0;
+    size_t total = 0;
+    for (int l = 0; l < n; ++l) {
+        const size_t b = sgv3d_conv2d_winograd4_workspace_bytes(descs + l);
+        if (b == 0) return 0;
+        total += (b + 255) / 256 * 256;
+    }
+    return total;
+}
+
+extern "C" int sgv3d_conv2d_winograd4_forward_multi(int n, const sgv3d_conv_desc *descs, const float *x, const void *const *u_packed,
+                                                    const float *const *scale, const float *const *bias, float *const *y,
+                                                    void *workspace, size_t workspace_bytes, void *stream) {
+    SGV3D_REQUIRE(n >= 1 && n <= kWino4Multi, "conv2d_winograd4_forward_multi: 1 to %d layers, not %d", kWino4Multi, n);
+    SGV3D_REQUIRE(descs && x && u_packed && scale && bias && y && workspace, "conv2d_winograd4_forward_multi: null pointer");
+    SGV3D_REQUIRE(((reinterpret_cast<uintptr_t>(x) | reinterpret_cast<uintptr_t>(workspace)) & 15) == 0,
+                  "conv2d_winograd4_forward_multi: pointers must be 16-B aligned");
+    for (int l = 0; l < n; ++l)
+        if (int rc = wino4_multi_check(descs + l, descs, u_packed[l], scale[l], bias[l], y[l])) return rc;
+    const size_t need = sgv3d_conv2d_winograd4_multi_workspace_bytes(n, descs);
+    if (workspace_bytes < need)
+        return fail(SGV3D_ENOSPACE, "conv2d_winograd4_forward_multi: workspace has %zu bytes, needs %zu", workspace_bytes, need);
+    Wino4MultiArgs in, out;
+    in.n = out.n = n;
+    in.first[0] = out.first[0] = 0;
+    unsigned char *ws = static_cast<unsigned char *>(workspace);
+    for (int l = 0; l < n; ++l) {
+        const sgv3d_conv_desc *d = descs + l;
+        Wino4Args &a = in.a[l];
+        a.x = x; a.scale = scale[l]; a.bias = bias[l]; a.res = nullptr; a.y = y[l];
+        a.batch = d->batch; a.h = d->in_h; a.w = d->in_w; a.cin = d->cin; a.cout = d->cout;
+        a.x_ld = d->x_ld; a.x_coff = d->x_coff; a.y_ld = d->y_ld; a.y_coff = d->y_coff; a.res_ld = 0; a.relu = d->relu;
+        long long tiles;
+        wino4_geom(d, a.ay, a.ax, tiles, a.rows);
+        SGV3D_REQUIRE(tiles < 0x7fffffffLL / 64, "conv2d_winograd4_forward_multi: too many tiles");
+        SGV3D_REQUIRE(wino4_chunk(d, a.rows) == d->cout, "conv2d_winograd4_forward_multi: a layer whose M needs more than one channel pass");
+        a.v = reinterpret_cast<float *>(ws);
+        a.m = reinterpret_cast<float *>(ws + (size_t)36 * a.rows * d->cin * 6);
+        ws += (sgv3d_conv2d_winograd4_workspace_bytes(d) + 255) / 256 * 256;
+        a.gw = 0; a.c0 = 0; a.cn = d->cout;
+        out.a[l] = a;
+        in.first[l + 1] = in.first[l] + cdiv(tiles * (d->cin / 4), kTB);
+        out.first[l + 1] = out.first[l] + cdiv(tiles * (d->cout / 4), kTB);
+    }
+    for (int l = n; l < kWino4Multi; ++l) {
+        in.a[l] = in.a[0]; out.a[l] = out.a[0];
+        in.first[l + 1] = in.first[n]; out.first[l + 1] = out.first[n];
+    }
+    hipStream_t st = as_stream(stream);
+    hipLaunchKernelGGL(wino4_input_x3_multi_kernel, dim3(in.first[n]), dim3(kTB), 0, st, in);
+    for (int l = 0; l < n; ++l) {
+        const sgv3d_conv_desc *d = descs + l;
+        const Wino4Args &a = in.a[l];
+        if (int rc = conv_gemm_grouped_x3(a.v, static_cast<const unsigned char *>(u_packed[l]), a.m, a.rows, d->cin, d->cout, d->cout_pad,
+                                          d->tile & 15, st, (size_t)d->cout_pad * d->cin * 6)) return rc;
+    }
+    hipLaunchKernelGGL(wino4_output_multi_kernel, dim3(out.first[n]), dim3(kTB), 0, st, out);
+    return check_launch("conv2d_winograd4_forward_multi");
+}
diff --git a/sgv3d_amd/csrc/misc_layers.hip b/sgv3d_amd/csrc/misc_layers.hip
--- a/sgv3d_amd/csrc/misc_layers.hip
+++ b/sgv3d_amd/csrc/misc_layers.hip
@@ -1,4 +1,5 @@
 #include "common.hpp"
+#include "avgpool.hpp"
 
 using namespace sgv3d;
 
@@ -99,36 +100,43 @@
     }
 }
 
-constexpr int kAvgChunks = 32;
-
-__global__ __launch_bounds__(kBlock) void global_avgpool_partial_kernel(int P, int C, int ld,
-                                                                        const float *__restrict__ x,
-                                                                        float *__restrict__ part) {
-    __shared__ float red[4][64];
+__global__ __launch_bounds__(kAvgBlock) void global_avgpool_partial_kernel(int P, int C, int ld,
+                                                                           const float *__restrict__ x,
+                                                                           float *__restrict__ part) {
+    __shared__ float4 red[4][64];
     const int b = blockIdx.z, chunk = blockIdx.y;
-    const int c = blockIdx.x * 64 + (threadIdx.x & 63);
-    const int g = threadIdx.x >> 6;
-    const int per = (P + kAvgChunks - 1) / kAvgChunks;
-    const int p0 = chunk * per, p1 = min(P, p0 + per);
-    float s = 0.f;
-    if (c < C)
-        for (int p = p0 + g; p < p1; p += 4) s += x[((long long)b * P + p) * ld + c];
-    red[g][threadIdx.x & 63] = s;
+    const int q = threadIdx.x & 63, g = threadIdx.x >> 6;
+    const int c = (blockIdx.x * 64 + q) * 4;
+    int p0, p1;
+    avgpool_chunk(P, chunk, p0, p1);
+    float4 s = make_float4(0.f, 0.f, 0.f, 0.f);
+    if (c < C) {
+        const float *xb = x + ((long long)b * P) * ld + c;
+#pragma unroll 4
+        for (int p = p0 + g; p < p1; p += 4) {
+            const float4 v = *reinterpret_cast<const float4 *>(xb + (long long)p * ld);
+            s.x += v.x; s.y += v.y; s.z += v.z; s.w += v.w;
+        }
+    }
+    red[g][q] = s;
     __syncthreads();
-    if (g == 0 && c < C)
-        part[((long long)b * kAvgChunks + chunk) * C + c] =
-            (red[0][threadIdx.x] + red[1][threadIdx.x]) + (red[2][threadIdx.x] + red[3][threadIdx.x]);
-}
-
-__global__ __launch_bounds__(kBlock) void global_avgpool_final_kernel(int B, int P, int C,
-                                                                      const float *__restrict__ part,
-                                                                      float *__restrict__ y) {
-    const long long i = (long long)blockIdx.x * kBlock + threadIdx.x;
-    if (i >= (long long)B * C) return;
-    const int b = (int)(i / C), c = (int)(i - (long long)b * C);
-    float s = 0.f;
-    for (int k = 0; k < kAvgChunks; ++k) s += part[((long long)b * kAvgChunks + k) * C + c];
-    y[i] = s / (float)P;
+    if (g == 0 && c < C) {
+        const float4 r0 = red[0][q], r1 = red[1][q], r2 = red[2][q], r3 = red[3][q];
+        *reinterpret_cast<float4 *>(part + ((long long)b * kAvgChunks + chunk) * C + c) =
+            make_float4((r0.x + r1.x) + (r2.x + r3.x), (r0.y + r1.y) + (r2.y + r3.y), (r0.z + r1.z) + (r2.z + r3.z),
+                        (r0.w + r1.w) + (r2.w + r3.w));
+    }
+}
+
+__global__ __launch_bounds__(kAvgBlock) void global_avgpool_partial_scalar_kernel(int P, int C, int ld,
+                                                                                  const float *__restrict__ x,
+                                                                                  float *__restrict__ part) {
+    avgpool_partial_scalar(P, C, ld, x, part);
+}
+
+__global__ __launch_bounds__(kAvgBlock) void global_avgpool_final_kernel(int P, int C, const float *__restrict__ part,
+                                                                         float *__restrict__ y) {
+    avgpool_final(P, C, part, y);
 }
 
 __global__ __launch_bounds__(kBlock) void dense_kernel(int B, int K, int N, const float *__restrict__ x,
@@ -472,10 +480,15 @@
     if (workspace_bytes < sgv3d_global_avgpool_workspace_bytes(batch, channels))
         return fail(SGV3D_ENOSPACE, "global_avgpool: workspace too small");
     float *part = static_cast<float *>(workspace);
-    hipLaunchKernelGGL(global_avgpool_partial_kernel, dim3(cdiv(channels, 64), kAvgChunks, batch), dim3(kBlock), 0,
-                       as_stream(stream), pixels, channels, x_ld, x, part);
-    hipLaunchKernelGGL(global_avgpool_final_kernel, dim3(cdiv((long long)batch * channels, kBlock)), dim3(kBlock), 0,
-                       as_stream(stream), batch, pixels, channels, part, y);
+    const bool quads = channels % 4 == 0 && x_ld % 4 == 0 && ((reinterpret_cast<uintptr_t>(x) | reinterpret_cast<uintptr_t>(part)) & 15) == 0;
+    if (quads)
+        hipLaunchKernelGGL(global_avgpool_partial_kernel, dim3(cdiv(channels, 256), kAvgChunks, batch), dim3(kAvgBlock), 0,
+                           as_stream(stream), pixels, channels, x_ld, x, part);
+    else
+        hipLaunchKernelGGL(global_avgpool_partial_scalar_kernel, dim3(cdiv(channels, 64), kAvgChunks, batch), dim3(kAvgBlock), 0,
+                           as_stream(stream), pixels, channels, x_ld, x, part);
+    hipLaunchKernelGGL(global_avgpool_final_kernel, dim3(cdiv(channels, 32), batch), dim3(kAvgBlock), 0, as_stream(stream), pixels,
+                       channels, part, y);
     return check_launch("global_avgpool_kernel");
 }
 
diff --git a/sgv3d_amd/hip_ops.py b/sgv3d_amd/hip_ops.py
--- a/sgv3d_amd/hip_ops.py
+++ b/sgv3d_amd/hip_ops.py
@@ -136,6 +136,22 @@
 X3_TILE_ROWS = {t: TILES[t].bm for t in WINO4_X3_TILES}
 X3_TILE_COLS = {t: TILES[t].bn for t in WINO4_X3_TILES}
 WINO4_TILES = conv_tiles.family("wino4", "wino4_x3")
+
+
+def wino4_axis_tiles(n, dil):
+    dil = max(1, int(dil))
+    return min(dil * -(-(-(-n // dil)) // 4), -(-(n + dil - 1) // 4))
+
+
+def wino4_tiles(batch, oh, ow, dil):
+    return batch * wino4_axis_tiles(oh, dil) * wino4_axis_tiles(ow, dil)
+
+
+def _wino4_tiles_per_phase(batch, oh, ow, dil):
+    dil = max(1, int(dil))
+    return batch * dil * dil * -(-(-(-oh // dil)) // 4) * -(-(-(-ow // dil)) // 4)
+
+
 WINO4_G48 = _os.environ.get("SGV3D_WINO4_G48", "1") != "0"
 WINO4_X3 = _os.environ.get("SGV3D_WINO4_X3", "1") != "0"
 PW_X3 = _os.environ.get("SGV3D_PW_X3", "1") != "0"
@@ -607,8 +623,7 @@
                                      kmode=2 if self.k_order == 0 else 0 if pw1 else 1)
             if T.flops == "wino4":
                 oh, ow = self.out_hw(H, W)
-                dil = max(1, self.dil)
-                tiles = B * dil * dil * -(-(-(-oh // dil)) // 4) * -(-(-(-ow // dil)) // 4)
+                tiles = _wino4_tiles_per_phase(B, oh, ow, self.dil)
                 mfma = 2.0 * 36 * (-(-tiles // T.bm) * T.bm) * self.cin * self.cout
             elif T.flops == "direct_k32":
                 mfma = 2.0 * gemm_m * self.cout * _up32(self.cin * self.kh * self.kw)
@@ -804,8 +819,7 @@
         return cands
 
     def _x3_tiles(self, d):
-        dil = max(1, int(d.dil))
-        tiles = d.batch * dil * dil * -(-(-(-d.out_h // dil)) // 4) * -(-(-(-d.out_w // dil)) // 4)
+        tiles = _wino4_tiles_per_phase(d.batch, d.out_h, d.out_w, d.dil)
         waste = {r: (-(-tiles // r) * r - tiles) / tiles for r in sorted(set(X3_TILE_ROWS.values()))}
         best = min(waste.values())
         ms = [r for r in waste if waste[r] <= max(best, 0.10) and (r <= 64 or tiles >= r)]
@@ -923,7 +937,7 @@
     g = globals()
     return tuple(g.get(k) for k in ("AUTOTUNE", "SPLIT_K", "WINOGRAD", "FUSED_HEAD", "HEAD_PATH", "MFMA_BF16", "BF16_ACTIVATIONS",
                                     "MFMA_F32X3", "MFIRST", "WINO4", "WINO_HALF", "PATCH_BF16", "DW_BF16", "DW_DEEP", "DW_NARROW",
-                                    "DW_SPLIT_K", "DW_DEEP_MAX_WGS", "PAIR_BF16", "TUNE_STREAMS", "PARALLEL_BRANCHES", "F4RES", "OCC5", "WINO4_G48", "DCN_FUSED", "WINO4_X3", "PW_X3",
+                                    "DW_SPLIT_K", "DW_DEEP_MAX_WGS", "PAIR_BF16", "TUNE_STREAMS", "PARALLEL_BRANCHES", "F4RES", "OCC5", "WINO4_G48", "DCN_FUSED", "WINO4_X3", "WINO4_MULTI", "PW_X3",
                                     "DCN_FUSED_BF16", "DCN_FUSED_TRAIN", "TRAIN_BF16_STORAGE", "SHORTCUT_X3", "DECONV_X3", "VIT_BF16", "STEM_FUSED"))
 
 
@@ -1068,6 +1082,97 @@
     on = t1 < t2
     tune_record(sig, [1, best] if on else [0, 0])
     return best if on else 0
+
+WINO4_MULTI = _os.environ.get("SGV3D_WINO4_MULTI", "1") != "0"
+WINO4_MULTI_MAX = 4
+
+
+def _wino4_sibling_choice(conv, x):
+    B, H, W, _ = (int(v) for v in x.shape)
+    t = int(conv.tile)
+    if t in WINO4_X3_TILES:
+        return t, 1
+    return conv._tile_cache.get((B, H, W, t, 0, MFMA_BF16, MFMA_F32X3, CONV_NORMAL, False, False, 0), (0, 0))
+
+
+def wino4_multi_eligible(convs, x, out=None, y_coffs=None, training=False):
+    if not (WINO4_MULTI and WINO4_X3 and WINO4 and WINOGRAD and not MFMA_BF16 and not MFMA_F32X3 and not PARALLEL_BRANCHES and not training):
+        return False
+    if not 2 <= len(convs) <= WINO4_MULTI_MAX or x.dtype != torch.float32 or x.dim() != 4 or not x.is_contiguous():
+        return False
+    if int(x.shape[0]) < 1 or int(x.shape[-1]) % 4:
+        return False
+    if any((not c.wino4_ok()) or c.cin != convs[0].cin or c.cin > int(x.shape[-1]) for c in convs):
+        return False
+    if out is not None:
+        ld = int(out.shape[-1])
+        if (out.dtype != torch.float32 or out.dim() != 4 or not out.is_contiguous() or tuple(out.shape[:3]) != tuple(x.shape[:3]) or ld % 4
+                or y_coffs is None or len(y_coffs) != len(convs)
+                or any(int(o) % 4 or int(o) < 0 or int(o) + c.cout > ld for o, c in zip(y_coffs, convs))):
+            return False
+    return True
+
+
+def wino4_multi_signature(convs, x):
+    B, H, W, _ = (int(v) for v in x.shape)
+    return (f"pair|wino4multi|{'+'.join(f'{c.cout}x{c.cin}d{c.dil}' for c in convs)}|{B}x{H}x{W}|ts{TUNE_STREAMS}")
+
+
+def wino4_multi(convs, x, out, y_coffs, tiles):
+    n = len(convs)
+    if not wino4_multi_eligible(convs, x, out, y_coffs) or len(tiles) != n or any(int(t) not in WINO4_X3_TILES for t in tiles):
+        raise _lib.SGV3DError("wino4_multi covers 2..4 F(4x4) layers with f32x3 tiles on one f32 NHWC input in the fp32 mode")
+    B, H, W, x_ld = (int(v) for v in x.shape)
+    lib = _lib.load()
+    descs = (ConvDesc * n)()
+    us, flops, nbytes = [], 0.0, 4.0 * B * H * W * convs[0].cin_real
+    for l, (c, t) in enumerate(zip(convs, tiles)):
+        d = descs[l]
+        d.batch, d.in_h, d.in_w, d.cin = B, H, W, c.cin
+        d.out_h, d.out_w, d.cout = H, W, c.cout
+        d.kh, d.kw, d.stride, d.pad, d.dil = 3, 3, 1, c.pad, c.dil
+        d.x_ld, d.x_coff, d.y_ld, d.y_coff = x_ld, 0, int(out.shape[-1]), int(y_coffs[l])
+        d.res_ld, d.relu, d.mode, d.deconv_ks = 0, 1 if c.relu else 0, CONV_NORMAL, c.ks
+        T = TILES[int(t)]
+        us.append(c._form(T.form))
+        d.k_pad, d.cout_pad, d.tile, d.x_nchw, d.k_order, d.split_k = c.cin, c.wino4_x3_cout_pad, T.abi, 0, c.k_order, 1
+        flops += 2.0 * B * H * W * c.cout_real * c.cin_real * 9
+        nbytes += 4.0 * c.cout_real * c.cin_real * 9 + 4.0 * B * H * W * c.cout_real
+    arr = lambda ps: (ctypes.c_void_p * n)(*[p or None for p in ps])
+    pu, psc, psh, py = (arr([u.data_ptr() for u in us]), arr([_lib.ptr(c.scale) for c in convs]), arr([_lib.ptr(c.shift) for c in convs]),
+                        arr([out.data_ptr()] * n))
+    nws = lib.sgv3d_conv2d_winograd4_multi_workspace_bytes(n, ctypes.addressof(descs))
+    ws = torch.empty(max(nws, 16), dtype=torch.uint8, device=x.device)
+    with torch.cuda.device(x.device), prof("conv_wino4_x3_multi", flops, nbytes):
+        rc = lib.sgv3d_conv2d_winograd4_forward_multi(n, ctypes.addressof(descs), x.data_ptr(), ctypes.addressof(pu), ctypes.addressof(psc),
+                                                      ctypes.addressof(psh), ctypes.addressof(py), ws.data_ptr(), nws, _st(x))
+    _lib.check(rc, "sgv3d_conv2d_winograd4_forward_multi")
+    return out
+
+
+def wino4_multi_choice(convs, x, out, y_coffs, training=False):
+    if not wino4_multi_eligible(convs, x, out, y_coffs, training):
+        return None
+    picks = [_wino4_sibling_choice(c, x) for c in convs]
+    if any(t not in WINO4_X3_TILES or sk != 1 for t, sk in picks):
+        return None
+    tiles = tuple(t for t, _ in picks)
+    sig = wino4_multi_signature(convs, x)
+    hit = tune_lookup(sig, x.device)
+    if hit is not None:
+        return tiles if int(hit[0]) else None
+    if not tune_may_measure():
+        return tiles
+    TUNE_STATS["measured"] += 1
+
+    def separate():
+        for c, o, t in zip(convs, y_coffs, tiles):
+            c(x, out, y_coff=o, tile=t, split_k=1)
+    t0, _, t1 = tune_best_of(sig, x.device, separate, [(1, lambda: wino4_multi(convs, x, out, y_coffs, tiles))])
+    on = t1 < t0
+    tune_record(sig, [1 if on else 0, 0])
+    return tiles if on else None
+
 
 DECONV_X3 = _os.environ.get("SGV3D_DECONV_X3", "1") != "0"
 
diff --git a/sgv3d_amd/layers/backbones/lss_fpn.py b/sgv3d_amd/layers/backbones/lss_fpn.py
--- a/sgv3d_amd/layers/backbones/lss_fpn.py
+++ b/sgv3d_amd/layers/backbones/lss_fpn.py
@@ -88,8 +88,15 @@
                 hip_ops.broadcast_channels(x5, cat, y_coff=4 * mid)
 
         def conv_branches():
-            for i, m in enumerate((self.aspp1, self.aspp2, self.aspp3, self.aspp4)):
-                m.hip_state(x.device)(x, cat, y_coff=i * mid)
+            convs = [m.hip_state(x.device) for m in (self.aspp1, self.aspp2, self.aspp3, self.aspp4)]
+            convs[0](x, cat, y_coff=0)
+            offs = [mid, 2 * mid, 3 * mid]
+            tiles = hip_ops.wino4_multi_choice(convs[1:], x, cat, offs, training=self.training)
+            if tiles is not None:
+                hip_ops.wino4_multi(convs[1:], x, cat, offs, tiles)
+            else:
+                for c, o in zip(convs[1:], offs):
+                    c(x, cat, y_coff=o)
         hip_ops.run_parallel(x.device, (conv_branches, pooled_branch))
         if fold:
             return s['conv1_head'](cat, shift=folded[0].view(-1), out_dtype=x.dtype)
```

After: 297.8 (median of 6 runs). 1.6% higher.
